# wreuven/h264-scroll-encoder

Measured on AMD Instinct MI355X. Metric: composed frames/sec (1280x720, 360x360 dyn) at 1/2/4/8 GPU; bit-exact vs CPU, higher is better.
Workload: dtype u8; 1 GPU; BASELINE config 3: 256 concurrent 1280x720 streams + 360x360 synthetic dynamic rect (4x4 int transform + quant + CAVLC), composer_write_scroll_frame semantics; resolution=1280x720, streams_per_gpu=256, parallelism=static stream shard x1, no RCCL

## Files before the change

### h264-scroll-encoder_amd/csrc/dyn_engine.h

```cpp
#ifndef SCROLL_DYN_ENGINE_H
#define SCROLL_DYN_ENGINE_H

#include <hip/hip_runtime.h>
#include "engine.h"

typedef struct {
    uint32_t *rows;
    uint16_t *meta;
    uint2 *body_lo, *body_hi;
    uint4 *body_w;
    uint4 *heads;
    unsigned long long *tcx;
    uint32_t *rowstage;
    uint32_t *gbits;
    uint32_t *spill;
    uint32_t *ctr;
    uint32_t ctr_frames;
    uint32_t epoch;
} DynScratch;
#define DYN_HEAD_VECS 16
#define DYN_CTR_LIST 4

typedef struct {
    hipStream_t side;
    hipEvent_t e0, e1;
} DynFork;
int dyn_launch_code(hipStream_t hs, int nframes, int S, DevStream *st, const NalDesc *nal,
                    int ld_nal, const PlanPending *pend, DynFrame *dfr, int ld_fr,
                    const DynGeom *g, const uint8_t *src, const uint8_t *refs, const DynScratch *x,
                    uint32_t epoch, int mbw, uint64_t *stamps, const DynFork *fk, hipEvent_t ev0 = nullptr,
                    hipEvent_t ev1 = nullptr);
int dyn_launch_static(hipStream_t hs, int nframes, int S, DevStream *st, const NalDesc *nal, int ld_nal,
                      const PlanPending *pend, DynFrame *dfr, int ld_fr, const DynGeom *g, const DynScratch *x);
int dyn_launch_pack(hipStream_t hs, int nframes, int S, DevStream *st, const NalDesc *nal,
                    int ld_nal, const PlanPending *pend, DynFrame *dfr, int ld_fr,
                    const DynGeom *g, const DynScratch *x, uint8_t *eps, uint64_t *stamps, const DynFork *fk);
int dyn_launch_emit(hipStream_t hs, int nframes, int S, const DevStream *st, const NalDesc *nal,
                    int ld_nal, const DynFrame *dfr, int ld_fr, const DynGeom *g,
                    const uint8_t *stage, const DynScratch *x, uint8_t *arena, uint64_t ld_arena,
                    uint64_t *stamps);
int dyn_launch_synth(hipStream_t hs, int nframes, int S, uint8_t *src, const DynGeom *g,
                     int stream_base, int t0);

void dyn_rowstage_geom(DynGeom *g, int mbw, int mbh);
size_t dyn_slot_bound(int mbw, int mbh, int rw, int rh);
uint32_t dyn_ep_cap(int rw, int rh, int debug);

#endif
```

### h264-scroll-encoder_amd/csrc/dyn_kernels.hip

```cpp
#include <hip/hip_runtime.h>

#include <stdint.h>
#include <mutex>

#include "dyn_device.h"
#include "dyn_engine.h"
#include "row_mfma.h"
#include "stage_util.h"

using namespace scroll;
using namespace scroll::dyn;
using namespace scroll::stage;

namespace {

__constant__ Tabs g_tabs = SCROLL_DYN_TABS;
constexpr Tabs k_tabs = SCROLL_DYN_TABS;
__constant__ PTabs g_ptabs = make_ptabs(k_tabs);
__device__ uint32_t g_tzrb[TZRB_N];
__constant__ LvTab g_lvt = make_lvt();

struct QpPair {
    QParams l, c;
};
// ... 452 lines not shown
    Regions rg;
    int a_end, mbw, nrefs;
    __device__ inline int sel(int row, int col) const
    {
        const bool curA = row < a_end, abvA = (row - 1) < a_end;
        return 3 * (row == 0 ? 0 : (curA ? 1 : (abvA ? 2 : 3))) + (col == 0 ? 0 : (col == mbw - 1 ? 2 : 1));
    }
    template <class S>
    __device__ inline void put_class(S &sk, int cls) const
    {
        const int ty = cls / 3, pos = cls - 3 * ty;
        const int x = pos == 0 ? 0 : (pos == 1 ? min(1, mbw - 1) : mbw - 1);
        const bool cur = ty == 0 ? 0 < a_end : ty == 1;
        const bool abv = ty == 1 || ty == 2;
        const int ref = cur ? rg.ra : rg.rb, mv4 = 4 * (cur ? rg.mva : rg.mvb);
        const int aref = abv ? rg.ra : rg.rb, amv4 = 4 * (abv ? rg.mva : rg.mvb);
        int px, py;
        predict(x, ty == 0 ? 0 : 1, mbw, ref, mv4, aref, amv4, px, py);
        put_mb_head(sk, ref, 0 - px, mv4 - py, nrefs);
    }
    template <class S>
    __device__ inline void put_slow(S &sk, int row, int col) const
    {
        const bool curA = row < a_end, abvA = (row - 1) < a_end;
        const int ref = curA ? rg.ra : rg.rb, mv4 = 4 * (curA ? rg.mva : rg.mvb);
        const int aref = abvA ? rg.ra : rg.rb, amv4 = 4 * (abvA ? rg.mva : rg.mvb);
        int px, py;
        predict(col, row, mbw, ref, mv4, aref, amv4, px, py);
        put_mb_head(sk, ref, 0 - px, mv4 - py, nrefs);
    }
};

__device__ inline HeadCtx head_ctx(const NalCtx &c)
{
    HeadCtx H;
    H.rg = regions(c);
    H.a_end = (c.h - c.off) / 16;
    H.mbw = c.w / 16;
    H.nrefs = 2 + c.nwp;
    return H;
}

__device__ inline uint32_t row_static_bits(const HeadCtx &H, const uint32_t *hlen, int row, const Rect &R)
{
    const int mbw = H.mbw;
    const bool in = row >= R.y0 && row < R.y0 + R.h;
    auto isdyn = [&](int col) { return in && col >= R.x0 && col < R.x0 + R.w; };
    const int base = H.sel(row, 0) - 0;
    uint32_t bits = isdyn(0) ? 0u : hlen[base] + 1u;
    if (mbw >= 2) {
        if (!isdyn(mbw - 1)) bits += hlen[base + 2] + 1u;
        int nmid = mbw - 2;
        if (in) nmid -= max(0, min(R.x0 + R.w, mbw - 1) - max(R.x0, 1));
        bits += (uint32_t)nmid * (hlen[base + 1] + 1u);
    }
    return bits;
}

__device__ inline void lb_store(unsigned long long *p, uint64_t v)
{
    __hip_atomic_store(p, v, __ATOMIC_RELAXED, __HIP_MEMORY_SCOPE_AGENT);
}

__host__ __device__ inline uint64_t rs_group_words(const DynGeom &g, int nA, int gi)
{
    if (gi < nA) return (uint64_t)gi * g.rs_static_words;
    if (gi < nA + g.h) return (uint64_t)nA * g.rs_static_words + (uint64_t)(gi - nA) * g.rs_row_words;
    return (uint64_t)(gi - g.h) * g.rs_static_words + (uint64_t)g.h * g.rs_row_words;
}

__host__ __device__ inline uint64_t rs_runs_words(const DynGeom &g, int nA, int gi)
{
    const bool row = gi >= nA && gi < nA + g.h;
    return rs_group_words(g, nA, gi) + (row ? g.rs_row_words - EPC_ROW : g.rs_static_words - EPC_STATIC);
}

constexpr uint32_t LO_LEN = 0x7ffu;

__device__ inline void piece_token(const uint16_t (*ct)[68], uint32_t mv, int nC, uint32_t &tv, uint32_t &tl)
{
    const int tc = tc_of(mv), t1 = (int)((mv >> 13) & 3u);
    if (nC >= 8) {
        tv = tc ? (uint32_t)(((tc - 1) << 2) | t1) : 3u;
        tl = 6;
    } else {
        const uint32_t e = ct[nC < 2 ? 0 : (nC < 4 ? 1 : 2)][4 * tc + t1];
        tv = e & 255u;
        tl = e >> 8;
    }
}

__device__ inline void wave_sync()
{
    __builtin_amdgcn_fence(__ATOMIC_RELEASE, "wavefront");
    __builtin_amdgcn_wave_barrier();
    __builtin_amdgcn_fence(__ATOMIC_ACQUIRE, "wavefront");
}

template <class S>
__device__ inline void ovf_code(S &sk, const PTabs &PT, const Tabs &TB, uint4 bd, const uint4 *bw, int pc, int nC)
{
    if (nC == -1) {
        const int dq[4] = {(int)(int16_t)(bd.x & 0xffffu), (int)(int16_t)(bd.x >> 16),
                           (int)(int16_t)(bd.y & 0xffffu), (int)(int16_t)(bd.y >> 16)};
        cavlc_dc4(sk, PT, dq);
    } else if (bw) {
        const uint4 hi = *bw;
        const uint32_t w8[8] = {bd.x, bd.y, bd.z, bd.w, hi.x, hi.y, hi.z, hi.w};
        int16_t l16[16];
#pragma unroll
        for (int i = 0; i < 8; ++i) {
            l16[2 * i] = (int16_t)(w8[i] & 0xffffu);
            l16[2 * i + 1] = (int16_t)(w8[i] >> 16);
        }
        cavlc_block(sk, TB, l16, pc < 16 ? 16 : 15, nC);
    } else {
        const int8_t *lvp = reinterpret_cast<const int8_t *>(&bd);
        cavlc_block(sk, TB, lvp, pc < 16 ? 16 : 15, nC);
    }
}

__device__ __attribute__((noinline)) uint32_t ovf_bits(const PTabs &PT, const Tabs &TB, uint4 bd, const uint4 *bw,
                                                       int pc, int nC)
{
    CountSink cn{0};
    ovf_code(cn, PT, TB, bd, bw, pc, nC);
    return cn.n;
}

__device__ __attribute__((noinline)) void ovf_put(uint32_t *buf, uint32_t lo, uint32_t n, uint32_t pos,
                                                  const PTabs &PT, const Tabs &TB, uint4 bd, const uint4 *bw, int pc,
                                                  int nC)
{
    WSink sk{LdsOrWin{buf, lo, n}, 0, 0, 0};
    sk.start(pos);
    ovf_code(sk, PT, TB, bd, bw, pc, nC);
    sk.finish();
}

__device__ inline uint4 body_msb(uint64_t hi, uint64_t lo, uint32_t n)
{
    const uint32_t k = 128u - n;
    uint64_t H, Lw;
    if (k >= 64u) {
        H = k >= 128u ? 0ull : lo << (k - 64u);
        Lw = 0ull;
    } else {
        H = k ? (hi << k) | (lo >> (64u - k)) : hi;
        Lw = lo << k;
    }
    return make_uint4((uint32_t)(H >> 32), (uint32_t)H, (uint32_t)(Lw >> 32), (uint32_t)Lw);
}

__global__ __launch_bounds__(256) void k_dyn_rows(const DevStream *__restrict__ st,
                                                  const NalDesc *__restrict__ nal, int ld_nal,
                                                  const PlanPending *__restrict__ pend,
                                                  DynFrame *__restrict__ dfr, int ld_fr, DynGeom g,
                                                  uint32_t *__restrict__ rows, uint32_t *__restrict__ ctr,
                                                  uint4 *__restrict__ heads)
{
    __shared__ int32_t wo[8], wl[8], wv[8];
    __shared__ int32_t gen;
    const int s = blockIdx.y, f = blockIdx.x, t = threadIdx.x;
    DynFrame *DF = dfr + (size_t)s * ld_fr + f;
    const int j = DF->nal;
    if (j < 0) return;
    if (t < 8) {
        wo[t] = pend[s].wo[t];
        wl[t] = pend[s].wl[t];
        wv[t] = pend[s].wv[t];
    }
    if (t == 0) gen = 0;
    __syncthreads();
    const DevStream *S = st + s;
    const NalDesc d = nal[(size_t)s * ld_nal + j];
    const NalCtx c = nal_ctx(S, d, wo, wl, wv);
    if (t < 12) {
        const HeadCtx H = head_ctx(c);
        CapSink hc{0, 0, 0};
        H.put_class(hc, t);
        uint4 *hv = heads + ((size_t)s * ld_fr + f) * DYN_HEAD_VECS;
        hv[t] = body_msb(hc.hi, hc.lo, min(hc.n, 128u));
        reinterpret_cast<uint32_t *>(hv + 12)[t] = hc.n | (hc.over() ? 0x80000000u : 0u);
    }
    const Regions rg = regions(c);
    const int w = c.w, h = c.h, a_end = (h - c.off) / 16;
    const uint32_t ysz = (uint32_t)w * (uint32_t)h, pic = ysz + ysz / 2;
    const WpTab T{wo, wv, h};
    uint32_t *rw = rows + ((size_t)s * ld_fr + f) * (size_t)(32 * g.h);
    bool my_gen = false;
    for (int i = t; i < 32 * g.h; i += 256) {
        uint32_t e;
        if (i < 16 * g.h) {
            const int Y = 16 * g.y0 + i, row = Y >> 4;
            const bool cA = row < a_end;
            int yo;
            const int b = luma_row(T, cA ? rg.ra : rg.rb, Y + (cA ? rg.mva : rg.mvb), yo);
            e = (uint32_t)b * pic + (uint32_t)yo * (uint32_t)w;
        } else {
            const int i2 = i - 16 * g.h, bot = i2 >= 8 * g.h;
            const int Y = 8 * g.y0 + (bot ? i2 - 8 * g.h : i2), row = Y >> 3;
            const bool cA = row < a_end;
            const int q = 4 * (cA ? rg.mva : rg.mvb), o = q >> 3, fr = q & 7;
            int yo;
            const int b = chroma_row(T, cA ? rg.ra : rg.rb, Y + o + bot, yo);
            if (b < 0) {
                e = ROW_GEN;
                if (!bot || fr) my_gen = true;
            } else {
                e = ((uint32_t)b * pic + ysz + (uint32_t)yo * (uint32_t)(w / 2)) | (uint32_t)fr << 28;
            }
        }
        rw[i] = e;
    }
    if (my_gen || S->dyn_qp < QP_MIN) gen = 1;
    __syncthreads();
    if (t == 0) {
        uint32_t e = 0u;
        if (gen) {
            const uint32_t k = atomicAdd(&ctr[1], 1u);
            if (k < g.gen_cap) {
                DF->rbsp_bytes = k;
                ctr[DYN_CTR_LIST + k] = (uint32_t)((size_t)s * ld_fr + f);
                e = DF_GENERAL;
            } else {
                e = DF_OVER;
            }
        }
        DF->err = e;
        DF->ep = 0u;
    }
}

constexpr int GW = 64;
#ifndef SCROLL_GBUF_WORDS
#define SCROLL_GBUF_WORDS 256
#endif
constexpr int GBUF_WORDS = SCROLL_GBUF_WORDS;

#ifndef SCROLL_STATIC_WORDS
#define SCROLL_STATIC_WORDS 1
#endif

struct StaticFixed {
    uint32_t ncand;
    uint32_t buf[GBUF_WORDS];
    uint64_t hhi[12], hlo[12];
    uint4 pat[12];
    uint32_t hlen[12];
    int32_t head_over;
    int32_t wo[8], wl[8], wv[8];
    uint32_t moff[DYN_STATIC_ROWS + 1];
};

__global__ __launch_bounds__(GW) void k_dyn_static(const DevStream *__restrict__ st,
                                                   const NalDesc *__restrict__ nal, int ld_nal,
                                                   const PlanPending *__restrict__ pend,
                                                   const DynFrame *__restrict__ dfr, int ld_fr, DynGeom g,
                                                   uint32_t *__restrict__ rowstage, uint32_t *__restrict__ gbits)
{
    __shared__ StaticFixed L;
    constexpr int SR = DYN_STATIC_ROWS;
    const Rect R{g.x0, g.y0, g.w, g.h};
    const int nA = max(1, (R.y0 + SR - 1) / SR);
    const int gi = (int)blockIdx.x >= nA ? (int)blockIdx.x + R.h : (int)blockIdx.x;
    const int ng = g.ngroups, f = blockIdx.y, s = blockIdx.z, t = threadIdx.x;
    const size_t nb = (size_t)s * ld_fr + f;
    const int j = dfr[nb].nal;
    if (j < 0) return;
    const bool first = gi == 0, last = gi == ng - 1;
    if (t < 8) {
        L.wo[t] = pend[s].wo[t];
        L.wl[t] = pend[s].wl[t];
        L.wv[t] = pend[s].wv[t];
    }
    if (t == 0) {
        L.head_over = 0;
        L.ncand = 0;
    }
    const DevStream *S = st + s;
    const NalDesc d = nal[(size_t)s * ld_nal + j];
    wave_sync();
    NalCtx c = nal_ctx(S, d, L.wo, L.wl, L.wv);
    c.qpd = S->dyn_qp - QP_DEFAULT;
    const HeadCtx H = head_ctx(c);
    const int mbw = H.mbw, mbh = c.h / 16;
    int ra, rb;
    if (gi < nA) {
        ra = gi * SR;
        rb = min(ra + SR, R.y0);
    } else {
        ra = R.y0 + R.h + (gi - nA - R.h) * SR;
        rb = min(ra + SR, mbh);
    }
    uint32_t F = 0;
    if (first) {
        CountSink hc{0};
        emit_slice_header(hc, c);
        F = hc.n;
    }
    if (t < 12) {
        CapSink hc{0, 0, 0};
        H.put_class(hc, t);
        L.hhi[t] = hc.hi;
        L.hlo[t] = hc.lo;
        L.hlen[t] = hc.n;
        if (hc.over()) L.head_over = 1;
        if (hc.n < 128u) {
            const uint64_t hi = (hc.hi << 1) | (hc.lo >> 63), lo = (hc.lo << 1) | 1u;
            L.pat[t] = body_msb(hi, lo, hc.n + 1u);
        } else {
            L.head_over = 1;
        }
    }
    wave_sync();
    const bool head_over = L.head_over;
    auto head_bits = [&](int r, int col) -> uint32_t {
        if (!head_over) return L.hlen[H.sel(r, col)];
        CountSink cn{0};
        H.put_slow(cn, r, col);
        return cn.n;
    };
    uint32_t len = 0;
    const int r = ra + t;
    if (r < rb) {
        if (!head_over) {
            len = row_static_bits(H, L.hlen, r, R);
        } else {
            for (int col = 0; col < mbw; ++col) len += head_bits(r, col) + 1u;
        }
    }
    const uint32_t incl = wave_incl_sum(len, t);
    if (r < rb) L.moff[r - ra] = F + incl - len;
    const uint32_t rows_end = F + __shfl(incl, GW - 1, GW);
    if (t == 0) L.moff[rb - ra] = rows_end;
    const uint32_t bits = rows_end + (last ? 1u : 0u);
    if (t == 0) gbits[nb * (size_t)ng + gi] = bits;
    wave_sync();

    uint32_t *out = rowstage + nb * g.rs_frame_words + rs_group_words(g, nA, gi);
    const uint32_t nw = min((bits + 31u) >> 5, g.rs_static_words - EPC_STATIC);
    const int ne = rb - ra;
    auto cnt_le = [&](uint32_t x) -> int {
        int lo = 0, hi = ne + 1;
        while (lo < hi) {
            const int mid = (lo + hi) >> 1;
            if (L.moff[mid] <= x) lo = mid + 1;
            else hi = mid;
        }
        return lo;
    };
    const uint32_t m_mbw = magic32((uint32_t)mbw);
    for (uint32_t p0 = 0; p0 < nw; p0 += GBUF_WORDS) {
        const uint32_t n = min((uint32_t)GBUF_WORDS, nw - p0);
        for (uint32_t i = (uint32_t)t; i < n; i += GW) L.buf[i] = 0u;
        wave_sync();
        const LdsOrWin win{L.buf, p0, n};
        if (!(SCROLL_STATIC_WORDS && !head_over) && first && t == 0 && p0 * 32u < F) {
            WSink hs{win, 0, 0, 0};
            hs.start(0);
            emit_slice_header(hs, c);
            hs.finish();
        }
        if (SCROLL_STATIC_WORDS && !head_over) {
            const uint32_t rbeg = L.moff[0], rend = L.moff[ne];
            for (uint32_t i = (uint32_t)t; i < n; i += GW) {
                const uint32_t W0 = 32u * (p0 + i), W1 = W0 + 32u;
                uint32_t acc = 0, b = max(W0, rbeg), R0 = 0, R1 = 0, L0 = 0, Lm = 1;
                int b3 = 0;
                float inv = 1.0f;
                while (b < W1 && b < rend) {
                    if (b >= R1 || b < R0) {
                        const int e = cnt_le(b) - 1;
                        R0 = L.moff[e];
                        R1 = L.moff[e + 1];
                        b3 = H.sel(ra + e, 0);
                        L0 = L.hlen[b3] + 1u;
                        Lm = L.hlen[b3 + 1] + 1u;
                        inv = 1.0f / (float)Lm;
                    }
                    const uint32_t o = b - R0;
                    uint32_t cl = (uint32_t)b3, off = o;
                    if (o >= L0) {
                        const uint32_t o2 = o - L0;
                        uint32_t q = (uint32_t)((float)o2 * inv);
                        if (q * Lm > o2) --q;
                        else if ((q + 1u) * Lm <= o2) ++q;
                        if (q < (uint32_t)(mbw - 2)) {
                            cl = (uint32_t)b3 + 1u;
                            off = o2 - q * Lm;
                        } else {
                            cl = (uint32_t)b3 + 2u;
                            off = o2 - (uint32_t)(mbw - 2) * Lm;
                        }
                    }
                    const uint32_t k = min(L.hlen[cl] + 1u - off, W1 - b);
                    const uint4 P = L.pat[cl];
                    const uint32_t wi = off >> 5, sh = off & 31u;
                    const uint32_t w0 = wi == 0 ? P.x : (wi == 1 ? P.y : (wi == 2 ? P.z : P.w));
                    const uint32_t w1 = wi == 0 ? P.y : (wi == 1 ? P.z : (wi == 2 ? P.w : 0u));
                    uint32_t v = sh ? __builtin_amdgcn_alignbit(w0, w1, 32u - sh) : w0;
                    v &= k >= 32u ? 0xffffffffu : ~(0xffffffffu >> k);
                    acc |= v >> (b - W0);
                    b += k;
                }
                L.buf[i] = acc;
            }
            wave_sync();
            if (first && t == 0 && p0 * 32u < F) {
                WSink hs{win, 0, 0, 0};
                hs.start(0);
                emit_slice_header(hs, c);
                hs.finish();
            }
            if (last && t == 0) {
                WSink sk{win, 0, 0, 0};
                sk.start(bits - 1u);
                sk.put(1, 1);
                sk.finish();
            }
            wave_sync();
            flush_window(L.buf, n, p0, p0 + n >= nw, out, &L.ncand,
                         rowstage + nb * g.rs_frame_words + rs_runs_words(g, nA, gi), EPC_STATIC - 1, t, GW);
            wave_sync();
            continue;
        }
        const int ea = max(cnt_le(32u * p0) - 1, 0), eb = min(cnt_le(32u * (p0 + n) - 1u), ne);
        const int nm = eb * mbw;
        for (int m = ea * mbw + t; m < nm; m += GW) {
            const int rr = (int)div_m((uint32_t)m, m_mbw), col = m - rr * mbw, rw = ra + rr;
            uint32_t off = L.moff[rr];
            WSink sk{win, 0, 0, 0};
            if (!head_over) {
                const int b3 = H.sel(rw, 0);
                off += col == 0 ? 0u : L.hlen[b3] + 1u + (uint32_t)(col - 1) * (L.hlen[b3 + 1] + 1u);
                if (off >= 32u * (p0 + n)) continue;
                const int cls = b3 + (col == 0 ? 0 : (col == mbw - 1 ? 2 : 1));
                if (off + L.hlen[cls] + 1u <= 32u * p0) continue;
                sk.start(off);
                sk.put_cap(CapSink{L.hhi[cls], L.hlo[cls], L.hlen[cls]});
            } else {
                for (int c2 = 0; c2 < col; ++c2) off += head_bits(rw, c2) + 1u;
                sk.start(off);
                H.put_slow(sk, rw, col);
            }
            sk.put(1, 1);
            sk.finish();
        }
        if (last && t == 0) {
            WSink sk{win, 0, 0, 0};
            sk.start(bits - 1u);
            sk.put(1, 1);
            sk.finish();
        }
        wave_sync();
        flush_window(L.buf, n, p0, p0 + n >= nw, out, &L.ncand,
                     rowstage + nb * g.rs_frame_words + rs_runs_words(g, nA, gi), EPC_STATIC - 1, t, GW);
        wave_sync();
    }
    if (t == 0) rowstage[nb * g.rs_frame_words + rs_runs_words(g, nA, gi)] = L.ncand;
}


__device__ inline CapSink cap_of_msb(uint64_t a, uint64_t b, uint32_t n)
{
    if (n == 0u) return CapSink{0, 0, 0};
    const uint32_t sh = 128u - n;
    if (sh >= 64u) return CapSink{0, a >> (sh - 64u), n};
    if (sh == 0u) return CapSink{a, b, n};
    return CapSink{a >> sh, (b >> sh) | (a << (64u - sh)), n};
}

__device__ inline void put_piece(uint32_t *buf, uint32_t p0, uint32_t n, uint32_t pos, uint32_t tv, uint32_t tl,
                                 uint4 b, uint32_t bl)
{
    const uint32_t tw = tv & low_mask((int)tl);
    const uint32_t c0 = __builtin_amdgcn_alignbit(tw, b.x, tl), c1 = __builtin_amdgcn_alignbit(b.x, b.y, tl);
    const uint32_t c2 = __builtin_amdgcn_alignbit(b.y, b.z, tl), c3 = __builtin_amdgcn_alignbit(b.z, b.w, tl);
    const uint32_t c4 = __builtin_amdgcn_alignbit(b.w, 0u, tl);
    const uint32_t sh = pos & 31u;
    const uint32_t o[6] = {c0 >> sh, __builtin_amdgcn_alignbit(c0, c1, sh), __builtin_amdgcn_alignbit(c1, c2, sh),
                           __builtin_amdgcn_alignbit(c2, c3, sh), __builtin_amdgcn_alignbit(c3, c4, sh),
                           __builtin_amdgcn_alignbit(c4, 0u, sh)};
    const uint32_t nw = (sh + tl + bl + 31u) >> 5, w0 = (pos >> 5) - p0;
#pragma unroll
    for (uint32_t j = 0; j < 6; ++j)
        if (j < nw && w0 + j < n && o[j]) atomicOr(&buf[w0 + j], o[j]);
}

constexpr uint32_t ROW_PAD = 4;

#ifndef SCROLL_LV_SWZ
#define SCROLL_LV_SWZ 0
#endif
__device__ inline uint32_t lv_key(int slot) { return ((uint32_t)slot >> 4) & 3u; }
__device__ inline uint4 lv_swz(uint4 v, uint32_t key)
{
    if (key & 1u) v = make_uint4(v.y, v.x, v.w, v.z);
    if (key & 2u) v = make_uint4(v.z, v.w, v.x, v.y);
    return v;
}
__device__ inline void put_piece1(uint32_t *buf, uint32_t pos, uint32_t tv, uint32_t tl, uint4 b, uint32_t bl)
{
    const uint32_t tw = tv & low_mask((int)tl);
    const uint32_t c0 = __builtin_amdgcn_alignbit(tw, b.x, tl), c1 = __builtin_amdgcn_alignbit(b.x, b.y, tl);
    const uint32_t c2 = __builtin_amdgcn_alignbit(b.y, b.z, tl), c3 = __builtin_amdgcn_alignbit(b.z, b.w, tl);
    const uint32_t c4 = __builtin_amdgcn_alignbit(b.w, 0u, tl);
    const uint32_t sh = pos & 31u, nw = (sh + tl + bl + 31u) >> 5;
    uint32_t *d = buf + (pos >> 5);
#ifndef SCROLL_PUT_FIRST
#define SCROLL_PUT_FIRST 1
#endif
    atomicOr(d, c0 >> sh);
    if (SCROLL_PUT_FIRST >= 2 || nw > 1u) atomicOr(d + 1, __builtin_amdgcn_alignbit(c0, c1, sh));
    if (SCROLL_PUT_FIRST >= 3 || nw > 2u) atomicOr(d + 2, __builtin_amdgcn_alignbit(c1, c2, sh));
    if (nw > 3u) {
        atomicOr(d + 3, __builtin_amdgcn_alignbit(c2, c3, sh));
        if (nw > 4u) {
            atomicOr(d + 4, __builtin_amdgcn_alignbit(c3, c4, sh));
            if (nw > 5u) atomicOr(d + 5, __builtin_amdgcn_alignbit(c4, 0u, sh));
        }
    }
}

constexpr int ROW_MAXT = 1024;
#ifndef SCROLL_ROW_WAVES
#define SCROLL_ROW_WAVES 8
#endif
#ifndef SCROLL_ROW_NP
#define SCROLL_ROW_NP 3
#endif
#ifndef SCROLL_ROW_NP_WIDE
#define SCROLL_ROW_NP_WIDE 4
#endif
#ifndef SCROLL_ROW_WIDE
#define SCROLL_ROW_WIDE 40
#endif
constexpr int ROW_NPMAX = 8;
#ifndef SCROLL_ROW_GB
#define SCROLL_ROW_GB 896
#endif
constexpr int ROW_GB = SCROLL_ROW_GB;

struct RowFixed {
    RowTabs ptabs;
    union {
        uint32_t buf[ROW_GB + 4];
        struct {
            uint32_t kc[2][SORT_KEYS];
            uint32_t kc_pad[32 - 2 * SORT_KEYS];
            uint32_t lvt[LVT_N];
        };
    };
    uint64_t hhi[12], hlo[12];
    uint32_t hlen[12];
    int32_t wo[8], wl[8], wv[8];
    int32_t head_over;
    uint32_t rt[32];
    uint32_t ncand;
    uint32_t spill;
    uint32_t pcd[NPC];
};

static_assert(2 * SORT_KEYS <= 32 && 32 + LVT_N <= ROW_GB, "the sort counts and the level table share the bit window");
static_assert(ROW_PAD == 4, "RowFixed::buf holds ROW_PAD spare words");
static_assert(offsetof(RowFixed, lvt) % 8 == 0, "the level table is copied in 8-byte words");

__host__ __device__ inline size_t row_lds_base(int w)
{
    return (size_t)16 * NPC * w + (size_t)4 * (w + 1) + (size_t)2 * (3 * NPC * w) + (size_t)10 * w + 16;
}
#ifndef SCROLL_ROW_GB_WIDE
#define SCROLL_ROW_GB_WIDE 1248
#endif
constexpr int ROW_GB_WIDE = SCROLL_ROW_GB_WIDE;
__host__ __device__ inline size_t row_wide_off(int w) { return (row_lds_base(w) + 15) & ~(size_t)15; }
__host__ __device__ inline bool row_wide_win(int w)
{
    return w > SCROLL_ROW_WIDE && row_wide_off(w) + 4 * (size_t)(ROW_GB_WIDE + ROW_PAD) + sizeof(RowFixed) <= 163840;
}
__host__ __device__ inline size_t row_lds_bytes(int w)
{
    return row_wide_win(w) ? row_wide_off(w) + 4 * (size_t)(ROW_GB_WIDE + ROW_PAD) : row_lds_base(w);
}

__host__ __device__ constexpr uint32_t pc_desc(int pc)
{
    if (pc == 16 || pc == 17) return 1u << 17;
    int da = 0, db = 0, e = 0;
    bool al = false, bt = false;
    if (pc < 16) {
        const int bx = pc & 3, by = pc >> 2;
        al = bx == 0;
        da = al ? 3 - NPC : -1;
        bt = by == 0;
        db = bt ? 0 : -4;
        e = bt ? pc : 0;
    } else {
        const int b = (pc - 18) & 3, bx = b & 1, by = b >> 1;
        al = bx == 0;
        da = al ? 1 - NPC : -1;
        bt = by == 0;
        db = bt ? 0 : -2;
        e = bt ? (pc < 22 ? pc - 14 : pc - 16) : 0;
    }
    return (uint32_t)(da + 32) | (al ? 1u : 0u) << 6 | (uint32_t)(db + 32) << 7 | (bt ? 1u : 0u) << 13 |
           (uint32_t)e << 14;
}

struct EpfLds {
    uint32_t *goff, *gb, *gw, *cw, *cbase, *lst, *cnt;
    uint32_t *ws;
};
// ... 2060 lines not shown
        S.fast = false;
        S.two = false;
        S.yv = false;
        S.lp = S.rem = 0u;
        if (c < wend && u0 >= 0 && u0 + 16 <= nebsp) {
            while ((int32_t)(sp[K] + K) < u0) K++;
            const uint32_t i0 = (uint32_t)u0 - K - kb, P = 8u * i0;
            while (gg + 1 < ng && goff[gg + 1] <= P) ++gg;
            const uint32_t lp = P - goff[gg], rem = gb[gg] - lp;
            const bool two = rem < 128u;
            if (!two || gg + 1 >= ng || gb[gg + 1] >= 128u - rem) {
                S.fast = true;
                S.two = two;
                S.lp = lp;
                S.rem = rem;
                S.yv = two && gg + 1 < ng;
                wo = 4u * (gw[gg] + (lp >> 5));
                yo = S.yv ? 4u * gw[gg + 1] : wo;
            }
        }
        S.K = K;
        const auto xa = __builtin_amdgcn_raw_buffer_load_b128(rr, wo, 0, 0);
        const uint32_t x4 = __builtin_amdgcn_raw_buffer_load_b32(rr, wo + 16u, 0, 0);
        const auto y = __builtin_amdgcn_raw_buffer_load_b128(rr, yo, 0, 0);
        S.x[0] = (uint32_t)xa[0]; S.x[1] = (uint32_t)xa[1]; S.x[2] = (uint32_t)xa[2]; S.x[3] = (uint32_t)xa[3];
        S.x[4] = x4;
        S.y[0] = (uint32_t)y[0]; S.y[1] = (uint32_t)y[1]; S.y[2] = (uint32_t)y[2]; S.y[3] = (uint32_t)y[3];
    };
    auto finish = [&](GSet &S) {
        if (S.fast) {
            const uint32_t yb[4] = {S.yv ? S.y[0] : 0u, S.yv ? S.y[1] : 0u, S.yv ? S.y[2] : 0u, S.yv ? S.y[3] : 0u};
            fast_chunk(S.c, S.u0, S.K, S.lp, S.rem, S.two, S.x, yb);
        } else {
            slow_chunk(S.c, S.K);
        }
    };
    for (uint32_t cb = cbeg; cb < cend; cb = wend) {
        uint32_t m = n;
        if (whole) {
            kb = 0;
            wend = cend;
        } else {
            __syncthreads();
            if (t == 0) {
                const int32_t ulo = 16 * (int32_t)cb - d0;
                uint32_t lo = 0, hi = n;
                while (lo < hi) {
                    const uint32_t mid = (lo + hi) >> 1;
                    if ((int32_t)(el[mid] + mid) < ulo) lo = mid + 1;
                    else hi = mid;
                }
                const uint32_t mm = min(n - lo, wcap);
                uint32_t ce = cend;
                if (lo + mm < n) ce = min(cend, max(cb + 1u, (uint32_t)((int32_t)(el[lo + mm] + lo + mm) + d0) >> 4));
                win[0] = lo;
                win[1] = mm;
                win[2] = ce;
            }
            __syncthreads();
            kb = win[0];
            m = win[1];
            wend = win[2];
        }
        for (uint32_t i = t; i < m; i += DT) (sorted ? sp : raw)[i] = el[kb + i] + kb;
        if (t == 0) sp[m] = 0x3fffffffu;
        __syncthreads();
        for (uint32_t i = t; i < (sorted ? 0u : m); i += DT) {
            const uint32_t v = raw[i];
            uint32_t r = 0;
            for (uint32_t k = 0; k < m; ++k) r += raw[k] < v ? 1u : 0u;
            sp[r] = v;
        }
        __syncthreads();
        T = goff[ng];
        ub = whole ? 0 : max(0, 16 * (int32_t)cb - d0);
        const uint32_t span = whole ? d.size : (uint32_t)(16 * (int32_t)wend - d0 - ub + 16);
        int lg = 0;
        while ((1u << lg) <= m) lg++;
        cs = 8;
        while ((span >> cs) >= (uint32_t)EPLIST_MAX) cs++;
        nblk = (int)(span >> cs) + 1;
        for (int bi = t; bi < nblk; bi += DT) {
            const uint32_t e0 = (uint32_t)ub + ((uint32_t)bi << cs);
            uint32_t K = 0;
            for (int b = lg - 1; b >= 0; --b) {
                const uint32_t k2 = K + (1u << b);
                K = k2 <= m && sp[k2 - 1] + (k2 - 1) < e0 ? k2 : K;
            }
            raw[bi] = K;
        }
        __syncthreads();
        if (stp && cb == cbeg) stp[1] = __builtin_amdgcn_s_memrealtime();
        GSet sa, sb;
        uint32_t c = cb + (uint32_t)t;
        if (c < wend) prep(c, sa);
        while (c < wend) {
            prep(c + DT, sb);
            finish(sa);
            c += DT;
            if (c >= wend) break;
            prep(c + DT, sa);
            finish(sb);
            c += DT;
        }
    }
    if (stamps) {
        __syncthreads();
        if (stp) stp[2] = __builtin_amdgcn_s_memrealtime();
    }
}

__device__ inline uint32_t mix32(uint32_t x)
{
    x ^= x >> 16;
    x *= 0x7feb352du;
    x ^= x >> 15;
    x *= 0x846ca68bu;
    x ^= x >> 16;
    return x;
}

__global__ __launch_bounds__(256) void k_dyn_synth(uint8_t *__restrict__ src, DynGeom g,
                                                   int stream_base, int t0)
{
    const uint32_t i = blockIdx.x * 256u + threadIdx.x;
    const int f = blockIdx.y, s = blockIdx.z;
    const uint32_t npx = 384u * (uint32_t)g.w * (uint32_t)g.h;
    if (i >= npx) return;
    const uint32_t tt = (uint32_t)(t0 + f);
    const uint32_t seed = (0x9E3779B9u * (uint32_t)(stream_base + s)) ^ (0x85EBCA6Bu * tt);
    const uint32_t hv = mix32(seed + i * 0x9E3779B9u);
    const uint32_t ly = 256u * (uint32_t)g.w * (uint32_t)g.h;
    int v;
    if (i < ly) {
        const int lw = 16 * g.w;
        const int y = (int)(i / (uint32_t)lw), x = (int)(i - (uint32_t)(y * lw));
        const int X = 16 * g.x0 + x, Y = 16 * g.y0 + y;
        v = 128 + ((X + 2 * Y + 3 * (int)tt) & 63) - 32 + (int)(hv >> 28) - 8;
    } else {
        const uint32_t r = (i - ly) % (64u * (uint32_t)g.w * (uint32_t)g.h);
        const int cw = 8 * g.w;
        const int y = (int)(r / (uint32_t)cw), x = (int)(r - (uint32_t)(y * cw));
        const int X = 8 * g.x0 + x, Y = 8 * g.y0 + y;
        v = 128 + ((X + Y + (int)tt) & 15) - 8 + (int)(hv >> 30);
    }
    src[(size_t)s * g.src_ld + (size_t)f * g.src_fr + i] = (uint8_t)clampi(v, 0, 255);
}

}

int dyn_launch_code(hipStream_t hs, int nframes, int S, DevStream *st, const NalDesc *nal,
                    int ld_nal, const PlanPending *pend, DynFrame *dfr, int ld_fr,
                    const DynGeom *g, const uint8_t *src, const uint8_t *refs, const DynScratch *x,
                    uint32_t epoch, int mbw, uint64_t *stamps, const DynFork *fk, hipEvent_t ev0, hipEvent_t ev1)
{
    if (nframes <= 0 || S <= 0) return 0;
    {
        static std::mutex mu;
        static uint64_t ready = 0;
        int dev = 0;
        if (hipGetDevice(&dev) != hipSuccess || dev >= 64) return -1;
        std::lock_guard<std::mutex> lk(mu);
        if (!(ready >> dev & 1u)) {
            hipLaunchKernelGGL(k_tzrb_init, dim3((TZRB_N + 255) / 256), dim3(256), 0, hs);
            if (hipGetLastError() != hipSuccess || hipStreamSynchronize(hs) != hipSuccess) return -1;
            ready |= 1ull << dev;
        }
    }
    hipLaunchKernelGGL(k_dyn_rows, dim3(nframes, S), dim3(256), 0, hs, st, nal, ld_nal, pend, dfr, ld_fr,
                       *g, x->rows, x->ctr, x->heads);
    if (hipGetLastError() != hipSuccess) return -1;
    hipStream_t hg = hs;
    if (fk) {
        if (hipEventRecord(fk->e0, hs) != hipSuccess || hipStreamWaitEvent(fk->side, fk->e0, 0) != hipSuccess)
            return -1;
        hg = fk->side;
    }
    const int nchunk = (24 * g->w * g->h + CODE_T - 1) / CODE_T;
    hipLaunchKernelGGL(k_dyn_code_general, dim3(nchunk, CODE_GEN_Y), dim3(CODE_T), 0, hg, st, dfr, ld_fr,
                       pend, nal, ld_nal, *g, x->rows, src, refs, x->meta, x->body_lo, x->body_hi, x->body_w,
                       x->ctr);
    if (hipGetLastError() != hipSuccess) return -1;
    if (row_lds_bytes(g->w) > 65536) {
        const int rl = (int)row_lds_bytes(g->w);
        if (hipFuncSetAttribute(reinterpret_cast<const void *>(&k_dyn_row<false>),
                                hipFuncAttributeMaxDynamicSharedMemorySize, rl) != hipSuccess ||
            hipFuncSetAttribute(reinterpret_cast<const void *>(&k_dyn_row<true>),
                                hipFuncAttributeMaxDynamicSharedMemorySize, rl) != hipSuccess)
            return -1;
    }
    if (ev0 && hipEventRecord(ev0, hs) != hipSuccess) return -1;
    hipLaunchKernelGGL(k_dyn_row<false>, dim3(g->h, nframes, S), dim3(row_threads(g->w)),
                       row_lds_bytes(g->w), hs, st, nal, ld_nal, pend, dfr, ld_fr, *g, x->rows, src, refs,
                       x->meta, x->body_lo, x->body_hi, x->body_w, x->tcx, epoch, x->rowstage, x->gbits, x->spill,
                       x->ctr, x->heads, stamps);
    if (hipGetLastError() != hipSuccess) return -1;
    if (ev1 && hipEventRecord(ev1, hs) != hipSuccess) return -1;
    hipLaunchKernelGGL(k_dyn_row<true>, dim3(g->h, std::min<uint32_t>(g->gen_cap, (uint32_t)(nframes * S)), 1),
                       dim3(row_threads(g->w)),
                       row_lds_bytes(g->w), hg, st, nal, ld_nal, pend, dfr, ld_fr, *g, x->rows, src, refs,
                       x->meta, x->body_lo, x->body_hi, x->body_w, x->tcx, epoch, x->rowstage, x->gbits, x->spill,
                       x->ctr, x->heads, stamps);
    if (hipGetLastError() != hipSuccess) return -1;
    if (fk) {
        if (dyn_launch_static(hg, nframes, S, st, nal, ld_nal, pend, dfr, ld_fr, g, x) ||
            hipEventRecord(fk->e1, hg) != hipSuccess)
            return -1;
    }
    return 0;
}

int dyn_launch_static(hipStream_t hs, int nframes, int S, DevStream *st, const NalDesc *nal, int ld_nal,
                      const PlanPending *pend, DynFrame *dfr, int ld_fr, const DynGeom *g, const DynScratch *x)
{
    if (nframes <= 0 || S <= 0) return 0;
    hipLaunchKernelGGL(k_dyn_static, dim3(g->ngroups - g->h, nframes, S), dim3(GW), 0, hs, st, nal, ld_nal,
                       pend, dfr, ld_fr, *g, x->rowstage, x->gbits);
    return hipGetLastError() == hipSuccess ? 0 : -1;
}

int dyn_launch_pack(hipStream_t hs, int nframes, int S, DevStream *st, const NalDesc *nal,
                    int ld_nal, const PlanPending *pend, DynFrame *dfr, int ld_fr,
                    const DynGeom *g, const DynScratch *x, uint8_t *eps, uint64_t *stamps, const DynFork *fk)
{
    if (nframes <= 0 || S <= 0) return 0;
    if (fk) {
        if (hipStreamWaitEvent(hs, fk->e1, 0) != hipSuccess) return -1;
    } else if (dyn_launch_static(hs, nframes, S, st, nal, ld_nal, pend, dfr, ld_fr, g, x)) {
        return -1;
    }
    if (g->ep_cap >= (uint32_t)EPF_BIG_LIST)
        hipLaunchKernelGGL((k_dyn_epfix<EPF_T, EPF_BIG_LIST>), dim3(nframes, S), dim3(EPF_T), gtab_bytes(g->ngroups, true),
                           hs, st, dfr, ld_fr, nframes, *g, x->rowstage, x->gbits, eps, stamps);
    else
        hipLaunchKernelGGL((k_dyn_epfix<EPF_T, EPF_LIST>), dim3(nframes, S), dim3(EPF_T), gtab_bytes(g->ngroups, true),
                           hs, st, dfr, ld_fr, nframes, *g, x->rowstage, x->gbits, eps, stamps);
    return hipGetLastError() == hipSuccess ? 0 : -1;
}

int dyn_launch_emit(hipStream_t hs, int nframes, int S, const DevStream *st, const NalDesc *nal,
                    int ld_nal, const DynFrame *dfr, int ld_fr, const DynGeom *g,
                    const uint8_t *stage, const DynScratch *x, uint8_t *arena, uint64_t ld_arena,
                    uint64_t *stamps)
{
    if (nframes <= 0 || S <= 0) return 0;
    const bool big = (int64_t)g->w * g->h > 1024;
    const uint32_t *rs = x ? x->rowstage : nullptr, *gbits = x ? x->gbits : nullptr;
    const dim3 grid(nframes, S, GATHER_Z);
    const size_t gl = x ? gtab_bytes(g->ngroups, false) : 0;
    if (x && !(g->debug & SCROLL_DEBUG_DYN_GATHER1))
        hipLaunchKernelGGL(k_dyn_gather, dim3(nframes, S, gather_z(*g, (int64_t)nframes * S)), dim3(DT), gl, hs, st, nal, ld_nal, dfr,
                           ld_fr, *g, stage, rs, gbits, arena, ld_arena, stamps);
    else if (x && big)
        hipLaunchKernelGGL((k_dyn_emit_gather<4, true>), grid, dim3(DT), gl, hs, st, nal, ld_nal, dfr, ld_fr, *g,
                           stage, rs, gbits, arena, ld_arena, stamps);
    else if (x)
        hipLaunchKernelGGL((k_dyn_emit_gather<1, true>), grid, dim3(DT), gl, hs, st, nal, ld_nal, dfr, ld_fr, *g,
                           stage, rs, gbits, arena, ld_arena, stamps);
    else if (big)
        hipLaunchKernelGGL((k_dyn_emit_gather<4, false>), grid, dim3(DT), 0, hs, st, nal, ld_nal, dfr, ld_fr,
                           *g, stage, rs, gbits, arena, ld_arena, stamps);
    else
        hipLaunchKernelGGL((k_dyn_emit_gather<1, false>), grid, dim3(DT), 0, hs, st, nal, ld_nal, dfr, ld_fr,
                           *g, stage, rs, gbits, arena, ld_arena, stamps);
    return hipGetLastError() == hipSuccess ? 0 : -1;
}

int dyn_launch_synth(hipStream_t hs, int nframes, int S, uint8_t *src, const DynGeom *g,
                     int stream_base, int t0)
{
    if (nframes <= 0 || S <= 0) return 0;
    const uint32_t npx = 384u * (uint32_t)g->w * (uint32_t)g->h;
    hipLaunchKernelGGL(k_dyn_synth, dim3((npx + 255) / 256, nframes, S), dim3(256), 0, hs, src, *g,
                       stream_base, t0);
    return hipGetLastError() == hipSuccess ? 0 : -1;
}

void dyn_rowstage_geom(DynGeom *g, int mbw, int mbh)
{
    const int SR = DYN_STATIC_ROWS;
    const int above = g->y0 < SR ? g->y0 : SR, below0 = mbh - g->y0 - g->h;
    const int below = below0 < SR ? below0 : SR;
    const int maxrows = above > below ? above : below;
    auto words = [](uint64_t bits) { return (uint32_t)((((bits + 31) / 32) + 63) & ~(uint64_t)63); };
    g->rs_static_words = words((uint64_t)HDR_MAX + (uint64_t)maxrows * mbw * (HEAD_MAX + 1) + 64) + EPC_STATIC;
    g->rs_spill_words = words((uint64_t)mbw * (HEAD_MAX + 1) + (uint64_t)g->w * MB_BITS_MAX + 64) + EPC_ROW;
    g->rs_row_words = words((uint64_t)mbw * (HEAD_MAX + 1) + (uint64_t)g->w * SCROLL_DYN_ROW_KBITS + 64) + EPC_ROW;
    if (g->rs_row_words > g->rs_spill_words) g->rs_row_words = g->rs_spill_words;
    g->rs_frame_words = (uint64_t)(g->ngroups - g->h) * g->rs_static_words + (uint64_t)g->h * g->rs_row_words;
}

uint32_t dyn_ep_cap(int rw, int rh, int debug)
{
    return (debug & SCROLL_DEBUG_DYN_EPWIN) || epf_big_rect((int64_t)rw * rh) ? (uint32_t)EPF_BIG_LIST
                                                                            : (uint32_t)EPLIST_MAX;
}

size_t dyn_slot_bound(int mbw, int mbh, int rw, int rh)
{
    const size_t bits = (size_t)HDR_MAX + (size_t)mbw * mbh * (HEAD_MAX + 1) +
                        (size_t)rw * rh * MB_BITS_MAX + 64;
    return ((bits / 8 + 32 + DYN_OVF_BYTES) + 255) & ~(size_t)255;
}

extern "C" int scroll_debug_row_occupancy(int w, int mbw, int extra_lds)
{
    int n = -1;
    (void)mbw;
    const size_t lds = (size_t)((long)row_lds_bytes(w) + extra_lds);
    if (hipOccupancyMaxActiveBlocksPerMultiprocessor(&n, reinterpret_cast<const void *>(&k_dyn_row<false>),
                                                     row_threads(w), lds) != hipSuccess)
        return -1;
    return n;
}
```

### h264-scroll-encoder_amd/csrc/scroll_kernels.hip

```cpp
#include <hip/hip_runtime.h>

#include <stdarg.h>
#include <stdint.h>
#include <stdio.h>
#include <stdlib.h>
#include <string.h>

#include <algorithm>
#include <mutex>
#include <vector>

#include "dyn_engine.h"
#include "hint_engine.h"
#include "splice_engine.h"
#include "hdyn_engine.h"
#include "ingest_engine.h"
#include "ipcm_engine.h"
#include "engine.h"
#include "scroll_device.h"

#include "dyn_device.h"

using namespace scroll;

// ... 661 lines not shown
                A[B0 + rel] = (uint8_t)tile_byte(Lo, no, cnt, jj, rel);
            }
        }
    }
    mark(4);
    if (stamps && lane == 0) {
        uint64_t hw = (uint32_t)__builtin_amdgcn_s_getreg((31 << 11) | 4);
        uint64_t xcc = (uint32_t)__builtin_amdgcn_s_getreg((15 << 11) | 20);
        stamp[7] = (__builtin_amdgcn_s_memrealtime() & 0xffffffffull) | (hw << 32);
        stamp[6] = (stamp[6] & 0x00ffffffffffffffull) | ((xcc & 0xff) << 56);
    }
    if (own && d.slow == 1) serial_write(my_ctx, A + d.out_off);
}

thread_local char g_err[512];

void set_err(const char *fmt, ...)
{
    va_list ap;
    va_start(ap, fmt);
    vsnprintf(g_err, sizeof(g_err), fmt, ap);
    va_end(ap);
}

#define HIPCHK(x)                                                                  \
    do {                                                                           \
        hipError_t e_ = (x);                                                       \
        if (e_ != hipSuccess) {                                                    \
            set_err("%s failed: %s", #x, hipGetErrorString(e_));                   \
            return SCROLL_ERR_HIP;                                                 \
        }                                                                          \
    } while (0)

int usable_devices(std::vector<int> *ids)
{
    int n = 0;
    if (hipGetDeviceCount(&n) != hipSuccess || n <= 0) {
        set_err("no HIP device visible (libh264scroll needs an MI355X / gfx950)");
        return 0;
    }
    int ok = 0;
    for (int i = 0; i < n; ++i) {
        hipDeviceProp_t p;
        if (hipGetDeviceProperties(&p, i) != hipSuccess) continue;
        if (strncmp(p.gcnArchName, "gfx950", 6) == 0) {
            ok++;
            if (ids) ids->push_back(i);
        }
    }
    if (!ok) set_err("no gfx950 device among %d HIP devices", n);
    return ok;
}

int check_cfg(const ComposerConfig *c)
{
    if (c->log2_max_frame_num < 1 || c->log2_max_frame_num > 16 ||
        (c->pic_order_cnt_type == 0 &&
         (c->log2_max_pic_order_cnt_lsb < 1 || c->log2_max_pic_order_cnt_lsb > 16)) ||
        c->num_waypoints < 0 || c->num_waypoints > MAX_WAYPOINTS || c->width < 0 ||
        c->height < 0) {
        set_err("unsupported ComposerConfig (log2 fields must be 1..16, num_waypoints 0..8)");
        return SCROLL_ERR_CONFIG;
    }
    return SCROLL_OK;
}

void cfg_to_dev(const ComposerConfig *c, DevStream *d)
{
    d->w = c->width;
    d->h = c->height;
    d->log2_mfn = c->log2_max_frame_num;
    d->poc_type = c->pic_order_cnt_type;
    d->log2_poc = c->log2_max_pic_order_cnt_lsb;
    d->deblock = c->deblocking_filter_control_present_flag;
    d->frame_num = c->frame_num;
    d->nwp = c->num_waypoints;
    for (int i = 0; i < 8; ++i) {
        d->wp_off[i] = c->waypoints[i].offset_px;
        d->wp_lt[i] = c->waypoints[i].long_term_idx;
        d->wp_valid[i] = c->waypoints[i].valid;
    }
}

void dev_to_cfg(const DevStream *d, ComposerConfig *c)
{
    c->frame_num = d->frame_num;
    c->num_waypoints = d->nwp;
    for (int i = 0; i < 8; ++i) {
        c->waypoints[i].offset_px = d->wp_off[i];
        c->waypoints[i].long_term_idx = d->wp_lt[i];
        c->waypoints[i].valid = d->wp_valid[i];
    }
}

}

constexpr int NEV = 7;
struct ScrollBatch {
    int device = 0;
    int mode = SCROLL_MODE_COMPOSER;
    int max_streams = 0, max_frames = 0, nstreams = 0;
    int debug = 0;
    size_t arena_bytes = 0, ld_arena = 0;
    int ld_nal = 0;
    DevStream *d_st = nullptr;
    DevStream *h_st = nullptr;
    int32_t *d_off = nullptr;
    NalDesc *d_nal = nullptr;
    uint8_t *d_arena = nullptr;
    hipStream_t own = nullptr;
    hipStream_t last = nullptr;
    hipEvent_t ev[NEV] = {};
    int timing = 0;
    int timed_pending = 0;
    float ms[6] = {0, 0, 0, 0, 0, 0};
    std::vector<hipEvent_t> ring;
    std::vector<uint8_t> ring_dyn;
    int ev_dyn = 0;
    int ring_used = 0;
    double acc_ms[6] = {0, 0, 0, 0, 0, 0};
    int acc_n = 0;
    int host_valid = 1;
    int last_plan_mode = SCROLL_PLAN_COMPOSER;
    int last_nframes = 0;
    std::vector<NalDesc> nal_cache;
    int nal_cache_valid = 0;
    uint64_t *d_dbg = nullptr;
    size_t dbg_slots = 0;
    PlanPending *d_pend = nullptr;
    int dyn_on = 0;
    int dyn_pw = 0, dyn_ph = 0;
    int dyn_refs = 0;
    DynGeom geo{};
    DynFrame *d_dfr = nullptr;
    uint8_t *d_src = nullptr, *d_refs = nullptr, *d_stage = nullptr;
    DynScratch dx{};
    int hint_on = 0;
    int hint_dirty = 0;
    int hint_max_mb = 0;
    std::vector<std::vector<ScrollHintRect>> h_hint;
    std::vector<int16_t> h_hint_mode;
    HintFrame *d_hf = nullptr;
    ScrollHintRect *d_pool = nullptr;
    size_t pool_cap = 0;
    struct SpliceHost {
        int x0 = 0, y0 = 0, w = 0, h = 0;
        std::vector<uint8_t> nal;
        const uint8_t *dnal = nullptr;
        size_t n = 0;
    };
    std::vector<SpliceHost> h_sp;
    std::vector<int32_t> h_dyn_pos;
    int fallback = 0;
    DynFork fork{};
    std::vector<int32_t> h_dyn_qp;
    int dyn_pos_custom = 0;
    int dyn_qp = 26;
    int hd_dirty = 0;
    uint32_t hd_mb_words = 0;
    size_t dyn_cap = 0;
    int sp_n = 0;
    int sp_dirty = 0;
    int sp_parse = 0;
    SpliceFrame *d_spf = nullptr;
    uint8_t *d_sp_nal = nullptr;
    uint32_t *d_sp_rbsp = nullptr;
    SpliceMbRec *d_sp_rec = nullptr;
    int32_t *d_sp_list = nullptr;
    SpliceUnit *d_sp_units = nullptr;
    int32_t *d_sp_lanes = nullptr;
    size_t sp_lanes_cap = 0, sp_nslots = 0;
    int sp_ymax = 1;
    size_t sp_nal_cap = 0, sp_rbsp_cap = 0, sp_rec_cap = 0, sp_list_cap = 0, sp_units_cap = 0;
    uint8_t *d_ing_in = nullptr;
    size_t ing_in_cap = 0;
    IngestFile *d_ing_files = nullptr;
    IngestScan *d_ing_scan = nullptr;
    IngestOut *d_ing_out = nullptr;
    int ing_cap = 0;
    void *d_ing_work = nullptr;
    size_t ing_work_bytes = 0;
    hipEvent_t ing_ev[2] = {};
    uint32_t *d_ipcm_cnt = nullptr;
    size_t ipcm_cap = 0;
    uint8_t *d_ipcm_stg = nullptr;
    size_t ipcm_stg_cap = 0;
    unsigned long long *d_ipcm_hw = nullptr;
    size_t ipcm_hw_cap = 0;
    uint32_t ipcm_epoch = 0;
    double ipcm_ms = 0.0;
    int ipcm_n = 0;
    uint32_t *ipcm_over = nullptr;
    uint32_t *d_ipcm_sticky = nullptr;
    size_t ipcm_over_stride = 0;
    std::vector<hipEvent_t> ipcm_ev;
    size_t ipcm_ev_used = 0;
    double ing_ms = 0.0;
    int ing_n = 0;
    int dyn_grow = 0;
    int32_t *d_upd = nullptr;
    size_t upd_cap = 0;
    uint64_t *d_out_tab = nullptr;
    size_t out_tab_cap = 0;
    hipEvent_t out_ev = nullptr;
};

static void event_ms(const hipEvent_t *e, bool dyn, bool lite, float out[6])
{
    auto el = [&](int a, int b) {
        float v = 0.0f;
        return hipEventElapsedTime(&v, e[a], e[b]) == hipSuccess ? v : 0.0f;
    };
    if (lite) {
        for (int k = 0; k < 6; ++k) out[k] = 0.0f;
        if (dyn) out[2] = out[4] = el(1, 6);
        else out[1] = el(1, 4);
        return;
    }
    if (dyn) {
        out[0] = el(0, 1) + el(2, 3);
        out[1] = el(3, 4);
        out[2] = el(1, 2);
        out[3] = el(4, 5);
        out[4] = el(1, 6);
        out[5] = el(6, 2);
    } else {
        out[0] = el(0, 1);
        out[1] = el(1, 4);
        out[2] = out[3] = out[4] = out[5] = 0.0f;
    }
}

static hipError_t timing_event(hipEvent_t *e)
{
    return hipEventCreateWithFlags(e, hipEventDisableSystemFence);
}

extern "C" {

const char *scroll_last_error(void) { return g_err; }

const char *scroll_version(void) { return "h264scroll-amd 0.1 (gfx950)"; }

int scroll_device_count(void) { return usable_devices(nullptr); }

int scroll_batch_create(ScrollBatch **out, const ScrollBatchDesc *desc)
{
    if (!out || !desc || desc->max_streams <= 0 || desc->max_frames <= 0 ||
        desc->arena_bytes == 0 ||
        (desc->mode != SCROLL_MODE_COMPOSER && desc->mode != SCROLL_MODE_EXPERIMENT)) {
        set_err("scroll_batch_create: bad descriptor");
        return SCROLL_ERR_ARG;
    }
    *out = nullptr;
    std::vector<int> ids;
    if (!usable_devices(&ids)) return SCROLL_ERR_NO_DEVICE;
    int n = 0;
    (void)hipGetDeviceCount(&n);
    if (desc->device < 0 || desc->device >= n) {
        set_err("scroll_batch_create: device %d out of range (%d visible)", desc->device, n);
        return SCROLL_ERR_ARG;
    }
    bool ok = false;
    for (int i : ids) ok |= (i == desc->device);
    if (!ok) {
        set_err("scroll_batch_create: device %d is not gfx950", desc->device);
        return SCROLL_ERR_NO_DEVICE;
    }
    HIPCHK(hipSetDevice(desc->device));
    ScrollBatch *b = new ScrollBatch();
    b->device = desc->device;
    b->mode = desc->mode;
    b->max_streams = desc->max_streams;
    b->max_frames = desc->max_frames;
    b->arena_bytes = desc->arena_bytes;
    b->ld_arena = (desc->arena_bytes + 128 + 255) & ~(size_t)255;
    b->ld_nal = 2 * desc->max_frames;
    size_t S = (size_t)desc->max_streams;
    hipError_t e = hipSuccess;
    if (e == hipSuccess) e = hipMalloc(&b->d_st, S * sizeof(DevStream));
    if (e == hipSuccess) e = hipHostMalloc(&b->h_st, S * sizeof(DevStream), hipHostMallocDefault);
    if (e == hipSuccess) e = hipMalloc(&b->d_off, S * (size_t)desc->max_frames * sizeof(int32_t));
    if (e == hipSuccess) e = hipMalloc(&b->d_nal, S * (size_t)b->ld_nal * sizeof(NalDesc));
    if (e == hipSuccess) e = hipMalloc(&b->d_arena, S * b->ld_arena);
    if (e == hipSuccess) e = hipMalloc(&b->d_pend, S * sizeof(PlanPending));
    if (e == hipSuccess) e = hipStreamCreateWithFlags(&b->own, hipStreamNonBlocking);
    for (int i = 0; i < NEV && e == hipSuccess; ++i) e = timing_event(&b->ev[i]);
    if (e == hipSuccess) e = hipMemset(b->d_st, 0, S * sizeof(DevStream));
    if (e == hipSuccess) e = hipMemset(b->d_off, 0, S * (size_t)desc->max_frames * sizeof(int32_t));
    if (e != hipSuccess) {
        set_err("scroll_batch_create: %s", hipGetErrorString(e));
        scroll_batch_destroy(b);
        return e == hipErrorOutOfMemory ? SCROLL_ERR_OOM : SCROLL_ERR_HIP;
    }
    memset(b->h_st, 0, S * sizeof(DevStream));
    b->last = b->own;
    *out = b;
    return SCROLL_OK;
}

void scroll_batch_destroy(ScrollBatch *b)
{
    if (!b) return;
    (void)hipSetDevice(b->device);
    if (b->own) (void)hipStreamSynchronize(b->own);
    for (int i = 0; i < NEV; ++i)
        if (b->ev[i]) (void)hipEventDestroy(b->ev[i]);
    for (hipEvent_t e : b->ring) (void)hipEventDestroy(e);
    if (b->fork.side) {
        (void)hipStreamSynchronize(b->fork.side);
        (void)hipStreamDestroy(b->fork.side);
        (void)hipEventDestroy(b->fork.e0);
        (void)hipEventDestroy(b->fork.e1);
    }
    if (b->own) (void)hipStreamDestroy(b->own);
    (void)hipFree(b->d_st);
    (void)hipHostFree(b->h_st);
    (void)hipFree(b->d_off);
    (void)hipFree(b->d_nal);
    (void)hipFree(b->d_arena);
    (void)hipFree(b->d_out_tab);
    (void)hipFree(b->d_upd);
    if (b->out_ev) (void)hipEventDestroy(b->out_ev);
    (void)hipFree(b->d_pend);
    (void)hipFree(b->d_dfr);
    (void)hipFree(b->d_src);
    (void)hipFree(b->d_refs);
    (void)hipFree(b->d_stage);
    (void)hipFree(b->d_hf);
    (void)hipFree(b->d_pool);
    (void)hipFree(b->d_spf);
    (void)hipFree(b->d_sp_nal);
    (void)hipFree(b->d_sp_rbsp);
    (void)hipFree(b->d_sp_rec);
    (void)hipFree(b->d_sp_list);
    (void)hipFree(b->d_sp_units);
    (void)hipFree(b->d_sp_lanes);
    (void)hipFree(b->d_ing_in);
    (void)hipFree(b->d_ipcm_cnt);
    (void)hipFree(b->d_ipcm_stg);
    (void)hipFree(b->d_ipcm_hw);
    (void)hipFree(b->d_ing_files);
    (void)hipFree(b->d_ing_scan);
    (void)hipFree(b->d_ing_out);
    (void)hipFree(b->d_ing_work);
    for (hipEvent_t e : b->ing_ev)
        if (e) (void)hipEventDestroy(e);
    for (hipEvent_t e : b->ipcm_ev)
        if (e) (void)hipEventDestroy(e);
    (void)hipFree(b->d_ipcm_sticky);
    if (b->d_dbg) (void)hipFree(b->d_dbg);
    delete b;
}

int scroll_batch_num_streams(const ScrollBatch *b) { return b ? b->nstreams : 0; }

int scroll_batch_set_debug(ScrollBatch *b, int flags)
{
    if (!b) return SCROLL_ERR_ARG;
    b->debug = flags;
    return SCROLL_OK;
}

static int dyn_grow_pools(ScrollBatch *b);

static int ipcm_async_check(ScrollBatch *b);

static int batch_host_sync(ScrollBatch *b)
{
    if (b->host_valid) return SCROLL_OK;
    HIPCHK(hipSetDevice(b->device));
    HIPCHK(hipStreamSynchronize(b->last));
    HIPCHK(hipMemcpy(b->h_st, b->d_st, (size_t)b->nstreams * sizeof(DevStream),
                     hipMemcpyDeviceToHost));
    b->host_valid = 1;
    return SCROLL_OK;
}

int scroll_batch_add_stream(ScrollBatch *b, const ComposerConfig *cfg)
{
    if (!b || !cfg) return SCROLL_ERR_ARG;
    if (b->nstreams >= b->max_streams) {
        set_err("scroll_batch_add_stream: batch full (%d streams)", b->max_streams);
        return SCROLL_ERR_ARG;
    }
    int rc = check_cfg(cfg);
    if (rc) return rc;
    if (b->dyn_on && (cfg->width != b->dyn_pw || cfg->height != b->dyn_ph)) {
        set_err("scroll_batch_add_stream: the dynamic rect needs %dx%d streams", b->dyn_pw,
                b->dyn_ph);
        return SCROLL_ERR_CONFIG;
    }
    if (b->hint_on && ((cfg->width / 16) * (cfg->height / 16) > b->hint_max_mb ||
                       cfg->width / 16 > HINT_MAX_MBW)) {
        set_err("scroll_batch_add_stream: hint staging slots hold %d MBs per picture, %d per row",
                b->hint_max_mb, HINT_MAX_MBW);
        return SCROLL_ERR_CONFIG;
    }
    rc = batch_host_sync(b);
    if (rc) return rc;
    int s = b->nstreams;
    DevStream *d = &b->h_st[s];
    if (b->dyn_qp != 26 && !cfg->deblocking_filter_control_present_flag) {
        set_err("scroll_batch_add_stream: a stream with the deblocking filter on (no "
                "deblocking_filter_control_present_flag) needs the rect at QP 26, the batch's is %d",
                b->dyn_qp);
        return SCROLL_ERR_CONFIG;
    }
    memset(d, 0, sizeof(*d));
    cfg_to_dev(cfg, d);
    d->dyn_qp = b->dyn_qp;
    d->out_pos = 0;
    d->out_cap = b->arena_bytes;
    HIPCHK(hipSetDevice(b->device));
    HIPCHK(hipMemcpy(b->d_st + s, d, sizeof(DevStream), hipMemcpyHostToDevice));
    b->nstreams++;
    return s;
}

int scroll_batch_get_config(ScrollBatch *b, int s, ComposerConfig *cfg)
{
    if (!b || !cfg || s < 0 || s >= b->nstreams) return SCROLL_ERR_ARG;
    int rc = batch_host_sync(b);
    if (rc) return rc;
    const DevStream *d = &b->h_st[s];
    composer_config_init(cfg, d->w, d->h);
    cfg->log2_max_frame_num = d->log2_mfn;
    cfg->pic_order_cnt_type = d->poc_type;
    cfg->log2_max_pic_order_cnt_lsb = d->log2_poc;
    cfg->deblocking_filter_control_present_flag = d->deblock;
    dev_to_cfg(d, cfg);
    return SCROLL_OK;
}

int scroll_batch_set_config(ScrollBatch *b, int s, const ComposerConfig *cfg)
{
    if (!b || !cfg || s < 0 || s >= b->nstreams) return SCROLL_ERR_ARG;
    int rc = check_cfg(cfg);
    if (rc) return rc;
    rc = batch_host_sync(b);
    if (rc) return rc;
    DevStream *d = &b->h_st[s];
    if (!cfg->deblocking_filter_control_present_flag) {
        bool bad = d->dyn_qp != 26;
        const size_t F = (size_t)b->max_frames, i0 = (size_t)s * F;
        for (size_t f = 0; !bad && f < F && i0 + f < b->h_dyn_qp.size(); ++f) {
            const int q = b->h_dyn_qp[i0 + f];
            bad = q >= 0 && q != 26;
        }
        if (bad) {
            set_err("scroll_batch_set_config: stream %d's rect QP is not 26: it cannot turn the deblocking "
                    "filter on (no deblocking_filter_control_present_flag)", s);
            return SCROLL_ERR_CONFIG;
        }
    }
    cfg_to_dev(cfg, d);
    HIPCHK(hipSetDevice(b->device));
    HIPCHK(hipMemcpy(b->d_st + s, d, sizeof(DevStream), hipMemcpyHostToDevice));
    return SCROLL_OK;
}

int scroll_batch_set_offsets(ScrollBatch *b, const int32_t *offsets, int nframes)
{
    if (!b || !offsets || nframes < 0 || nframes > b->max_frames) return SCROLL_ERR_ARG;
    if (nframes == 0 || b->nstreams == 0) return SCROLL_OK;
    HIPCHK(hipSetDevice(b->device));
    HIPCHK(hipMemcpy2D(b->d_off, (size_t)b->max_frames * sizeof(int32_t), offsets,
                       (size_t)nframes * sizeof(int32_t), (size_t)nframes * sizeof(int32_t),
                       (size_t)b->nstreams, hipMemcpyHostToDevice));
    return SCROLL_OK;
}

int32_t *scroll_batch_offsets_device(ScrollBatch *b) { return b ? b->d_off : nullptr; }

static void fold_ring(ScrollBatch *b)
{
    for (int i = 0; i + NEV <= b->ring_used; i += NEV) {
        float m[6];
        event_ms(&b->ring[i], (b->ring_dyn[i / NEV] & 1) != 0, (b->ring_dyn[i / NEV] & 2) != 0, m);
        for (int k = 0; k < 6; ++k) b->acc_ms[k] += m[k];
        b->acc_n++;
    }
    b->ring_used = 0;
}

static int ring_events(ScrollBatch *b, hipEvent_t **evs)
{
    if ((size_t)b->ring_used + NEV > b->ring.size()) {
        if (b->ring.size() >= (size_t)NEV * 256) {
            HIPCHK(hipStreamSynchronize(b->last));
            fold_ring(b);
        } else {
            for (int i = 0; i < NEV; ++i) {
                hipEvent_t e;
                HIPCHK(timing_event(&e));
                b->ring.push_back(e);
            }
            b->ring_dyn.push_back(0);
        }
    }
    *evs = &b->ring[b->ring_used];
    b->ring_used += NEV;
    return SCROLL_OK;
}

static int launch(ScrollBatch *b, int nframes, int plan_mode, int nal_max, hipStream_t hs,
                  int plan_flags = 0)
{
    int S = b->nstreams;
    if (S == 0) return SCROLL_OK;
    hipEvent_t *rev = nullptr;
    if (b->timing) {
        int rc = ring_events(b, &rev);
        if (rc) return rc;
    }
    const bool hint = b->hint_on && plan_mode != SCROLL_PLAN_EXPLICIT;
    const bool dyn = (b->dyn_on || hint) && plan_mode != SCROLL_PLAN_EXPLICIT;
    const bool lite = b->timing == 2;
    const bool lite_row = lite && dyn && !hint;
    auto mark = [&](int k) -> int {
        if (!b->timing || (!dyn && k != 0 && k != 1 && k != 4)) return SCROLL_OK;
        if (lite) {
            if ((k == 1 || k == (dyn ? 6 : 4)) && !lite_row) HIPCHK(hipEventRecord(rev[k], hs));
            return SCROLL_OK;
        }
        HIPCHK(hipEventRecord(b->ev[k], hs));
        HIPCHK(hipEventRecord(rev[k], hs));
        return SCROLL_OK;
    };
    if (b->timing) {
        b->ring_dyn[(b->ring_used - NEV) / NEV] = (uint8_t)((dyn ? 1 : 0) | (lite ? 2 : 0));
        if (!lite) b->ev_dyn = dyn ? 1 : 0;
    }
    const int ld_fr = b->max_frames;
    int rc = mark(0);
    if (rc) return rc;
    if (!dyn) {
        hipLaunchKernelGGL(k_plan, dim3(S), dim3(PLAN_THREADS), 0, hs, b->d_st, b->d_off,
                           b->max_frames, b->d_nal, b->ld_nal, nframes, plan_mode,
                           b->debug | plan_flags, b->d_pend, b->d_dfr, ld_fr);
        HIPCHK(hipGetLastError());
        if ((rc = mark(1)) || (rc = mark(2)) || (rc = mark(3))) return rc;
    } else {
        const bool dyn_rect = b->dyn_on && !hint;
        hipLaunchKernelGGL(k_plan, dim3(S), dim3(PLAN_THREADS), 0, hs, b->d_st, b->d_off,
                           b->max_frames, b->d_nal, b->ld_nal, nframes, plan_mode,
                           b->debug | plan_flags | PLAN_STATE | PLAN_DYN, b->d_pend, b->d_dfr,
                           ld_fr, nullptr, 0u, 0u, dyn_rect ? b->dx.ctr : nullptr);
        HIPCHK(hipGetLastError());
        if ((rc = mark(1))) return rc;
        uint64_t *stamps = nullptr;
        if (b->debug & SCROLL_DEBUG_DYN_STAMPS) {
            const size_t slots = (2 + (size_t)b->geo.ngroups) * (size_t)nframes * S;
            if (slots > b->dbg_slots) {
                if (b->d_dbg) (void)hipFree(b->d_dbg);
                HIPCHK(hipMalloc(&b->d_dbg, slots * 8 * sizeof(uint64_t)));
                b->dbg_slots = slots;
            }
            HIPCHK(hipMemsetAsync(b->d_dbg, 0, slots * 8 * sizeof(uint64_t), hs));
            stamps = b->d_dbg + 2 * (size_t)nframes * S * 8;
        }
        b->geo.debug = b->debug;
        if (hint) {
            if (b->sp_parse) {
                if (splice_launch_parse(hs, b->sp_n, b->sp_ymax, b->d_sp_list, b->d_spf, b->d_sp_units,
                                        b->d_sp_lanes, b->sp_nslots, b->d_st, ld_fr, b->d_sp_rbsp, b->d_sp_rec)) {
                    set_err("k_splice_parse launch: %s", hipGetErrorString(hipGetLastError()));
                    return SCROLL_ERR_HIP;
                }
                b->sp_parse = 0;
            }
            if (b->fallback && b->dyn_on &&
                hint_launch_fb(hs, nframes, S, b->d_st, b->d_nal, b->ld_nal, b->d_pend, b->d_dfr, ld_fr,
                               b->d_hf, b->d_pool)) {
                set_err("k_hint_fb launch: %s", hipGetErrorString(hipGetLastError()));
                return SCROLL_ERR_HIP;
            }
            if (hint_launch_stage(hs, nframes, S, b->d_st, b->d_nal, b->ld_nal, b->d_pend,
                                  b->d_dfr, ld_fr, b->d_hf, b->d_pool, b->d_stage,
                                  b->geo.slot_bytes)) {
                set_err("k_hint_stage launch: %s", hipGetErrorString(hipGetLastError()));
                return SCROLL_ERR_HIP;
            }
            const bool combined = b->dyn_on;
            if (combined &&
                hdyn_launch_code(hs, nframes, S, b->d_st, b->d_nal, b->ld_nal, b->d_pend, b->d_dfr, ld_fr,
                                 b->d_hf, b->d_pool, b->d_spf, &b->geo, b->d_src, b->d_refs,
                                 b->d_sp_rec, b->d_sp_rbsp, b->hd_mb_words)) {
                set_err("k_hdyn_code launch: %s", hipGetErrorString(hipGetLastError()));
                return SCROLL_ERR_HIP;
            }
            if ((b->sp_n > 0 || combined) &&
                splice_launch_stage(hs, nframes, S, b->d_st, b->d_nal, b->ld_nal, b->d_pend,
                                    b->d_dfr, ld_fr, b->d_hf, b->d_pool, b->d_spf, b->d_sp_rec,
                                    b->d_sp_rbsp, b->d_stage, b->geo.slot_bytes)) {
                set_err("k_splice_stage launch: %s", hipGetErrorString(hipGetLastError()));
                return SCROLL_ERR_HIP;
            }
            if ((rc = mark(6))) return rc;
        } else {
            b->dx.epoch = b->dx.epoch % 0xffffffu + 1u;
            const DynGeom &G = b->geo;
            const DynFork *fk = nullptr;
            static const bool fork_on = [] {
                const char *e = getenv("SCROLL_DYN_FORK");
                return e && e[0] == '1';
            }();
            if (fork_on) {
                if (!b->fork.side) {
                    HIPCHK(hipStreamCreateWithFlags(&b->fork.side, hipStreamNonBlocking));
                    HIPCHK(hipEventCreateWithFlags(&b->fork.e0, hipEventDisableTiming));
                    HIPCHK(hipEventCreateWithFlags(&b->fork.e1, hipEventDisableTiming));
                }
                fk = &b->fork;
            }
            if (dyn_launch_code(hs, nframes, S, b->d_st, b->d_nal, b->ld_nal, b->d_pend, b->d_dfr, ld_fr, &G,
                                b->d_src, b->d_refs, &b->dx, b->dx.epoch, b->dyn_pw / 16, stamps, fk,
                                lite_row ? rev[1] : nullptr, lite_row ? rev[6] : nullptr)) {
                set_err("k_dyn_code launch: %s", hipGetErrorString(hipGetLastError()));
                return SCROLL_ERR_HIP;
            }
            if ((rc = mark(6))) return rc;
            if (dyn_launch_pack(hs, nframes, S, b->d_st, b->d_nal, b->ld_nal, b->d_pend, b->d_dfr, ld_fr, &G,
                                &b->dx, b->d_stage, stamps ? b->d_dbg : nullptr, fk)) {
                set_err("k_dyn_static / k_dyn_epfix launch: %s", hipGetErrorString(hipGetLastError()));
                return SCROLL_ERR_HIP;
            }
        }
        if ((rc = mark(2))) return rc;
        hipLaunchKernelGGL(k_plan, dim3(S), dim3(PLAN_THREADS), 0, hs, b->d_st, b->d_off,
                           b->max_frames, b->d_nal, b->ld_nal, nframes, plan_mode,
                           b->debug | plan_flags | PLAN_SIZE | PLAN_DYN, b->d_pend, b->d_dfr,
                           ld_fr, (b->dyn_on && !b->hint_on) ? (const uint32_t *)b->dx.ctr : nullptr,
                           b->geo.rs_spill_cap, b->geo.gen_cap);
        HIPCHK(hipGetLastError());
        if ((rc = mark(3))) return rc;
    }
    int per_wg = EMIT_WAVES * TILE;
    int gx = (nal_max + per_wg - 1) / per_wg;
    if (gx > 0 && (b->debug & SCROLL_DEBUG_EMIT_STAMPS)) {
        size_t slots = (size_t)gx * S * EMIT_WAVES;
        if (slots > b->dbg_slots) {
            if (b->d_dbg) (void)hipFree(b->d_dbg);
            HIPCHK(hipMalloc(&b->d_dbg, slots * 8 * sizeof(uint64_t)));
            b->dbg_slots = slots;
        }
        HIPCHK(hipMemsetAsync(b->d_dbg, 0, slots * 8 * sizeof(uint64_t), hs));
    }
    if (gx > 0) {
        hipLaunchKernelGGL(k_emit, dim3(gx, S), dim3(EMIT_WAVES * 64), 0, hs, b->d_st, b->d_nal,
                           b->ld_nal, b->d_arena, (uint64_t)b->ld_arena, b->debug, b->d_dbg);
        HIPCHK(hipGetLastError());
    }
    if ((rc = mark(4))) return rc;
    if (dyn && dyn_launch_emit(hs, nframes, S, b->d_st, b->d_nal, b->ld_nal, b->d_dfr, ld_fr,
                               &b->geo, b->d_stage, hint ? nullptr : &b->dx, b->d_arena,
                               (uint64_t)b->ld_arena,
                               (b->debug & SCROLL_DEBUG_DYN_STAMPS) && b->d_dbg
                                   ? b->d_dbg + (size_t)nframes * S * 8 : nullptr)) {
        set_err("k_dyn_gather launch: %s", hipGetErrorString(hipGetLastError()));
        return SCROLL_ERR_HIP;
    }
    if ((rc = mark(5))) return rc;
    if (b->timing == 1) b->timed_pending = 1;
    b->host_valid = 0;
    b->nal_cache_valid = 0;
    b->last = hs;
    return SCROLL_OK;
}

static int hint_upload(ScrollBatch *b);
static int splice_upload(ScrollBatch *b);
static int hd_upload(ScrollBatch *b);
static int splice_frame_status(ScrollBatch *b, size_t i, int *status);
static const char *splice_msg(int e);

int scroll_batch_compose(ScrollBatch *b, int nframes, void *hip_stream)
{
    return scroll_batch_compose_ex(b, nframes, hip_stream, 0);
}

int scroll_batch_compose_ex(ScrollBatch *b, int nframes, void *hip_stream, int flags)
{
    if (!b || nframes < 0 || nframes > b->max_frames) {
        set_err("scroll_batch_compose: nframes %d out of range", nframes);
        return SCROLL_ERR_ARG;
    }
    if (b->dyn_on && !b->dyn_refs) {
        set_err("scroll_batch_compose: dynamic rect without reference pictures");
        return SCROLL_ERR_CONFIG;
    }
    HIPCHK(hipSetDevice(b->device));
    const bool combined = b->hint_on && b->dyn_on;
    if (b->dyn_pos_custom && !b->hint_on) {
        set_err("scroll_batch_compose: per-frame dynamic rect positions need UI hints "
                "(scroll_batch_set_hints)");
        return SCROLL_ERR_CONFIG;
    }
    if (b->hint_on && b->sp_dirty) {
        int rc = splice_upload(b);
        if (rc) return rc;
        if (combined) b->hd_dirty = 1;
    }
    if (combined && b->hd_dirty) {
        int rc = hd_upload(b);
        if (rc) return rc;
    }
    if (b->hint_on && b->hint_dirty) {
        int rc = hint_upload(b);
        if (rc) return rc;
    }
    hipStream_t hs = hip_stream ? (hipStream_t)hip_stream : b->own;
    int plan = b->mode == SCROLL_MODE_EXPERIMENT ? SCROLL_PLAN_EXPERIMENT : SCROLL_PLAN_COMPOSER;
    int nal_max = plan == SCROLL_PLAN_COMPOSER ? 2 * nframes : nframes;
    b->last_plan_mode = plan;
    b->last_nframes = nframes;
    return launch(b, nframes, plan, nal_max, hs,
                  (flags & SCROLL_COMPOSE_REWIND) ? PLAN_REWIND : 0);
}

int scroll_batch_sync(ScrollBatch *b)
{
    if (!b) return SCROLL_ERR_ARG;
    {
        int rc0 = batch_host_sync(b);
        if (rc0) return rc0;
        if ((rc0 = ipcm_async_check(b))) return rc0;
    }
    if (b->timed_pending) {
        event_ms(b->ev, b->ev_dyn != 0, false, b->ms);
        b->timed_pending = 0;
    }
    int rc = SCROLL_OK;
    for (int s = 0; s < b->nstreams; ++s) {
        if (!b->h_st[s].err) continue;
        if (rc == SCROLL_OK && (b->h_st[s].err & SCROLL_DEVERR_HANDOFF)) {
            set_err("stream %d: a dynamic-rect row waited past its bound for the row above's "
                    "TotalCoeffs (k_dyn_row hand-off); the stream committed nothing", s);
            rc = SCROLL_ERR_DEVICE;
        } else if (rc == SCROLL_OK && (b->h_st[s].err & SCROLL_DEVERR_SPLICE)) {
            int st = 0, ff = 0;
            for (; ff < b->max_frames && !st; ++ff)
                if (splice_frame_status(b, (size_t)s * b->max_frames + ff, &st)) break;
            if (st == HDYN_STATUS_OVERFLOW) {
                set_err("stream %d frame %d: a dynamic-rect MB under hints outgrew its %u-byte "
                        "region (raise slot_bytes of scroll_batch_set_dyn_rect)", s, ff - 1,
                        4u * b->hd_mb_words);
                rc = SCROLL_ERR_OVERFLOW;
            } else {
                set_err("stream %d frame %d: %s: %s", s, ff - 1,
                        b->dyn_on ? "dynamic rect under hints" : "spliced slice", splice_msg(st));
                rc = SCROLL_ERR_CONFIG;
            }
        } else if (rc == SCROLL_OK && (b->h_st[s].err & SCROLL_DEVERR_HINT)) {
            set_err("stream %d: a hint rect names a reference that is not valid in its frame "
                    "(ref 2 + i needs waypoint i)", s);
            rc = SCROLL_ERR_CONFIG;
        } else if (rc == SCROLL_OK && (b->h_st[s].err & SCROLL_DEVERR_DYN)) {
            uint32_t used[2] = {0, 0};
            if (b->dyn_on && !b->hint_on && b->dx.ctr)
                HIPCHK(hipMemcpy(used, b->dx.ctr, sizeof(used), hipMemcpyDeviceToHost));
            if (used[0] > b->geo.rs_spill_cap || used[1] > b->geo.gen_cap) {
                const int grc = dyn_grow_pools(b);
                set_err("stream %d: the dynamic rect's %s pool ran out (%u of %u); %s", s,
                        used[0] > b->geo.rs_spill_cap ? "row-stage spill" : "general-path record",
                        used[0] > b->geo.rs_spill_cap ? used[0] : used[1],
                        used[0] > b->geo.rs_spill_cap ? b->geo.rs_spill_cap : b->geo.gen_cap,
                        grc ? "growing it failed" : "grown: compose again");
            } else {
                set_err("stream %d: a staged NAL outgrew its staging slot (%llu bytes)", s,
                        (unsigned long long)b->geo.slot_bytes);
            }
            rc = SCROLL_ERR_OVERFLOW;
        } else if (rc == SCROLL_OK) {
            set_err("stream %d: output arena overflow (%llu bytes used, capacity %llu)", s,
                    (unsigned long long)b->h_st[s].out_pos,
                    (unsigned long long)b->h_st[s].out_cap);
            rc = SCROLL_ERR_OVERFLOW;
        }
        b->h_st[s].err = 0;
        HIPCHK(hipMemcpy(&b->d_st[s].err, &b->h_st[s].err, sizeof(int32_t),
                         hipMemcpyHostToDevice));
    }
    if (rc) return rc;
    return SCROLL_OK;
}

size_t scroll_batch_output_size(ScrollBatch *b, int s)
{
    if (!b || s < 0 || s >= b->nstreams || batch_host_sync(b)) return 0;
    return (size_t)b->h_st[s].out_pos;
}

int scroll_batch_copy_output(ScrollBatch *b, int s, size_t from, uint8_t *dst, size_t n)
{
    if (!b || s < 0 || s >= b->nstreams || (!dst && n)) return SCROLL_ERR_ARG;
    int rc = batch_host_sync(b);
    if (rc) return rc;
    if (from + n > b->h_st[s].out_pos) {
        set_err("scroll_batch_copy_output: range beyond stream output");
        return SCROLL_ERR_ARG;
    }
    if (n == 0) return SCROLL_OK;
    HIPCHK(hipSetDevice(b->device));
    HIPCHK(hipMemcpy(dst, b->d_arena + (size_t)s * b->ld_arena + from, n, hipMemcpyDeviceToHost));
    return SCROLL_OK;
}

namespace {
constexpr int OUT_Z = 8;
__global__ __launch_bounds__(1024) void k_out_table(DevStream *__restrict__ st, int S, uint64_t cap,
                                                    uint64_t *__restrict__ dtab, uint64_t *__restrict__ htab)
{
    __shared__ uint64_t s_w[16], s_carry;
    const int t = threadIdx.x, lane = t & 63, wave = t >> 6;
    if (t == 0) s_carry = 0;
    __syncthreads();
    for (int s0 = 0; s0 < S; s0 += 1024) {
        const int s = s0 + t;
        const uint64_t n = s < S ? st[s].undelivered : 0, a = (n + 15) & ~(uint64_t)15;
        const uint64_t inc = wave_incl_scan(a, lane);
        if (lane == 63) s_w[wave] = inc;
        __syncthreads();
        uint64_t before = s_carry;
        for (int w = 0; w < wave; ++w) before += s_w[w];
        if (s < S) {
            dtab[1 + 2 * (size_t)s] = htab[1 + 2 * (size_t)s] = before + inc - a;
            dtab[2 + 2 * (size_t)s] = htab[2 + 2 * (size_t)s] = n;
        }
        __syncthreads();
        if (t == 0)
            for (int w = 0; w < 16; ++w) s_carry += s_w[w];
        __syncthreads();
    }
    if (t == 0) {
        const uint64_t tot = s_carry <= cap ? s_carry : ~(uint64_t)0;
        dtab[0] = htab[0] = tot;
    }
    if (s_carry <= cap)
        for (int s = t; s < S; s += 1024) st[s].undelivered = 0;
}

__global__ __launch_bounds__(256) void k_out_copy(const DevStream *__restrict__ st, const uint8_t *__restrict__ arena,
                                                  uint64_t ld_arena, uint64_t arena_end,
                                                  const uint64_t *__restrict__ dtab, uint8_t *__restrict__ dst)
{
    const int s = blockIdx.y;
    if (dtab[0] == ~(uint64_t)0) return;
    const uint64_t n = dtab[2 + 2 * (size_t)s], o = dtab[1 + 2 * (size_t)s];
    const uint64_t from = (uint64_t)s * ld_arena + st[s].out_pos - n;
    uint4 *d = reinterpret_cast<uint4 *>(dst + o);
    const uint32_t q = (uint32_t)(from & 15u) >> 2, rb = (uint32_t)from & 3u;
    const uint64_t base = from & ~(uint64_t)15;
    const uint4 *a = reinterpret_cast<const uint4 *>(arena + base);
    const uint64_t nch = (n + 15) / 16;
    for (uint64_t j = (uint64_t)blockIdx.x * 256 + threadIdx.x; j < nch; j += (uint64_t)OUT_Z * 256) {
        const uint4 x = a[j];
        const uint4 y = (q | rb) && base + 16 * (j + 2) <= arena_end ? a[j + 1] : x;
        const uint32_t w0 = x.x, w1 = x.y, w2 = x.z, w3 = x.w, w4 = y.x, w5 = y.y, w6 = y.z, w7 = y.w;
        auto pick = [&](uint32_t i) -> uint32_t {
            const uint32_t lo = i & 1u ? (i & 2u ? w3 : w1) : (i & 2u ? w2 : w0);
            const uint32_t hi = i & 1u ? (i & 2u ? w7 : w5) : (i & 2u ? w6 : w4);
            return i & 4u ? hi : lo;
        };
        uint32_t o4[4];
#pragma unroll
        for (uint32_t k = 0; k < 4; ++k) {
            const uint32_t lo = pick(q + k), hi = pick(q + k + 1u);
            o4[k] = rb ? __builtin_amdgcn_alignbyte(hi, lo, rb) : lo;
        }
        d[j] = make_uint4(o4[0], o4[1], o4[2], o4[3]);
    }
}
}

int scroll_host_alloc(void **p, size_t n)
{
    if (!p) return SCROLL_ERR_ARG;
    *p = nullptr;
    hipError_t e = hipHostMalloc(p, n ? n : 1, hipHostMallocDefault);
    if (e != hipSuccess) {
        (void)hipGetLastError();
        set_err("scroll_host_alloc(%zu): %s", n, hipGetErrorString(e));
        return e == hipErrorOutOfMemory ? SCROLL_ERR_OOM : SCROLL_ERR_HIP;
    }
    return SCROLL_OK;
}

void scroll_host_free(void *p)
{
    if (p) (void)hipHostFree(p);
}

int scroll_batch_output_to_host_async(ScrollBatch *b, uint8_t *dst, size_t cap, uint64_t *table, void *hip_stream)
{
    if (!b || !dst || !table || (cap & 15) || (reinterpret_cast<uintptr_t>(dst) & 15)) {
        set_err("scroll_batch_output_to_host_async: bad arguments (dst / cap must be 16-byte aligned)");
        return SCROLL_ERR_ARG;
    }
    HIPCHK(hipSetDevice(b->device));
    hipStream_t hs = hip_stream ? (hipStream_t)hip_stream : (b->last ? b->last : b->own);
    if (b->last && hs != b->last) {
        if (!b->out_ev) HIPCHK(hipEventCreateWithFlags(&b->out_ev, hipEventDisableTiming));
        HIPCHK(hipEventRecord(b->out_ev, b->last));
        HIPCHK(hipStreamWaitEvent(hs, b->out_ev, 0));
    }
    const size_t S = (size_t)b->nstreams;
    if (b->out_tab_cap < 1 + 2 * S) {
        (void)hipFree(b->d_out_tab);
        b->d_out_tab = nullptr;
        b->out_tab_cap = 0;
        HIPCHK(hipMalloc(&b->d_out_tab, (1 + 2 * S) * sizeof(uint64_t)));
        b->out_tab_cap = 1 + 2 * S;
    }
    hipLaunchKernelGGL(k_out_table, dim3(1), dim3(1024), 0, hs, b->d_st, (int)S, (uint64_t)cap, b->d_out_tab,
                       table);
    HIPCHK(hipGetLastError());
    if (S) {
        hipLaunchKernelGGL(k_out_copy, dim3(OUT_Z, (unsigned)S), dim3(256), 0, hs, b->d_st, b->d_arena,
                           (uint64_t)b->ld_arena, (uint64_t)b->max_streams * b->ld_arena, b->d_out_tab, dst);
        HIPCHK(hipGetLastError());
    }
    b->last = hs;
    b->host_valid = 0;
    return SCROLL_OK;
}

const uint8_t *scroll_batch_output_device(ScrollBatch *b, int s)
{
    if (!b || s < 0 || s >= b->nstreams) return nullptr;
    return b->d_arena + (size_t)s * b->ld_arena;
}

int scroll_batch_reset_output(ScrollBatch *b)
{
    if (!b) return SCROLL_ERR_ARG;
    int rc = batch_host_sync(b);
    if (rc) return rc;
    for (int s = 0; s < b->nstreams; ++s) b->h_st[s].out_pos = b->h_st[s].undelivered = 0;
    HIPCHK(hipSetDevice(b->device));
    HIPCHK(hipMemcpy(b->d_st, b->h_st, (size_t)b->nstreams * sizeof(DevStream),
                     hipMemcpyHostToDevice));
    return SCROLL_OK;
}

static int load_nals(ScrollBatch *b)
{
    if (b->nal_cache_valid) return SCROLL_OK;
    int rc = batch_host_sync(b);
    if (rc) return rc;
    b->nal_cache.resize((size_t)b->nstreams * b->ld_nal);
    HIPCHK(hipMemcpy(b->nal_cache.data(), b->d_nal, b->nal_cache.size() * sizeof(NalDesc),
                     hipMemcpyDeviceToHost));
    b->nal_cache_valid = 1;
    return SCROLL_OK;
}

int scroll_batch_nal_count(ScrollBatch *b, int s)
{
    if (!b || s < 0 || s >= b->nstreams) return SCROLL_ERR_ARG;
    int rc = batch_host_sync(b);
    if (rc) return rc;
    return b->h_st[s].nnal;
}

int scroll_batch_nal_info(ScrollBatch *b, int s, int i, int *kind, int *offset_px,
                          uint32_t *size, int *slow)
{
    if (!b || s < 0 || s >= b->nstreams) return SCROLL_ERR_ARG;
    int rc = load_nals(b);
    if (rc) return rc;
    if (i < 0 || i >= b->h_st[s].nnal) return SCROLL_ERR_ARG;
    const NalDesc &d = b->nal_cache[(size_t)s * b->ld_nal + i];
    if (kind) *kind = d.kind;
    if (offset_px) *offset_px = d.off;
    if (size) *size = d.size;
    if (slow) *slow = d.slow;
    return SCROLL_OK;
}

int scroll_batch_kernel_stats(ScrollBatch *b, double *plan_ms, double *emit_ms, int *count)
{
    if (!b) return SCROLL_ERR_ARG;
    int rc = batch_host_sync(b);
    if (rc) return rc;
    HIPCHK(hipStreamSynchronize(b->last));
    fold_ring(b);
    if (plan_ms) *plan_ms = b->acc_ms[0];
    if (emit_ms) *emit_ms = b->acc_ms[1];
    if (count) *count = b->acc_n;
    for (int k = 0; k < 6; ++k) b->acc_ms[k] = 0;
    b->acc_n = 0;
    return SCROLL_OK;
}

int scroll_batch_kernel_stats_ex(ScrollBatch *b, double ms[6], int *count)
{
    if (!b || !ms) return SCROLL_ERR_ARG;
    int rc = batch_host_sync(b);
    if (rc) return rc;
    HIPCHK(hipStreamSynchronize(b->last));
    fold_ring(b);
    for (int k = 0; k < 6; ++k) {
        ms[k] = b->acc_ms[k];
        b->acc_ms[k] = 0;
    }
    if (count) *count = b->acc_n;
    b->acc_n = 0;
    return SCROLL_OK;
}

long long scroll_batch_debug_stamps(ScrollBatch *b, uint64_t *dst, long long max_slots)
{
    if (!b || batch_host_sync(b) || !b->d_dbg) return 0;
    long long n = (long long)b->dbg_slots < max_slots ? (long long)b->dbg_slots : max_slots;
    if (hipMemcpy(dst, b->d_dbg, (size_t)n * 8 * sizeof(uint64_t), hipMemcpyDeviceToHost) !=
        hipSuccess)
        return 0;
    return n;
}

unsigned long long scroll_batch_last_bytes(ScrollBatch *b)
{
    if (!b || batch_host_sync(b)) return 0;
    unsigned long long t = 0;
    for (int s = 0; s < b->nstreams; ++s) t += b->h_st[s].batch_bytes;
    return t;
}

long long scroll_batch_last_nals(ScrollBatch *b)
{
    if (!b || batch_host_sync(b)) return -1;
    long long t = 0;
    for (int s = 0; s < b->nstreams; ++s) t += b->h_st[s].nnal;
    return t;
}

static void dyn_release(ScrollBatch *b)
{
    if (!b->hint_on) {
        (void)hipFree(b->d_dfr);
        (void)hipFree(b->d_stage);
        b->d_dfr = nullptr;
        b->d_stage = nullptr;
    }
    (void)hipFree(b->d_src);
    (void)hipFree(b->d_refs);
    (void)hipFree(b->dx.rows);
    (void)hipFree(b->dx.meta);
    (void)hipFree(b->dx.body_lo);
    (void)hipFree(b->dx.body_hi);
    (void)hipFree(b->dx.body_w);
    (void)hipFree(b->dx.heads);
    (void)hipFree(b->dx.tcx);
    (void)hipFree(b->dx.rowstage);
    (void)hipFree(b->dx.ctr);
    (void)hipFree(b->dx.gbits);
    b->d_src = b->d_refs = nullptr;
    b->dx = DynScratch{};
    b->dyn_on = 0;
    b->dyn_refs = 0;
    b->h_dyn_pos.clear();
    b->h_dyn_qp.clear();
    b->dyn_pos_custom = 0;
    if (b->hint_on) {
        b->geo.x0 = b->geo.y0 = b->geo.w = b->geo.h = 0;
        b->sp_dirty = 1;
        b->hint_dirty = 1;
    }
}

static int hd_setup(ScrollBatch *b);
static int sp_grow(void **p, size_t *cap, size_t n, size_t size);

static size_t round256(size_t n) { return (n + 255) & ~(size_t)255; }

static size_t dyn_pair_bytes(const ScrollBatch *b)
{
    return round256((size_t)3 * b->dyn_pw * b->dyn_ph);
}

int scroll_batch_set_dyn_rect(ScrollBatch *b, int x0, int y0, int w, int h, size_t slot_bytes)
{
    if (!b || x0 < 0 || y0 < 0 || w < 0 || h < 0) return SCROLL_ERR_ARG;
    if (b->hint_on && b->sp_n > 0 && w > 0 && h > 0) {
        set_err("scroll_batch_set_dyn_rect: not combinable with spliced slices (clear them first)");
        return SCROLL_ERR_CONFIG;
    }
    int rc = batch_host_sync(b);
    if (rc) return rc;
    HIPCHK(hipSetDevice(b->device));
    dyn_release(b);
    if (w == 0 || h == 0) return SCROLL_OK;
    if (b->nstreams == 0) {
        set_err("scroll_batch_set_dyn_rect: add the streams first");
        return SCROLL_ERR_ARG;
    }
    const int pw = b->h_st[0].w, ph = b->h_st[0].h;
    for (int s = 1; s < b->nstreams; ++s)
        if (b->h_st[s].w != pw || b->h_st[s].h != ph) {
            set_err("scroll_batch_set_dyn_rect: streams of one batch must share the picture size");
            return SCROLL_ERR_CONFIG;
        }
    const int mbw = pw / 16, mbh = ph / 16;
    if ((pw & 15) || (ph & 15) || x0 + w > mbw || y0 + h > mbh || w > DYN_MAX_W || h > DYN_MAX_H ||
        mbw > DYN_MAX_MBW || mbh > DYN_MAX_MBH ||
        (size_t)3 * pw * ph >= ((size_t)1 << 28)) {
        set_err("scroll_batch_set_dyn_rect: rect (%d,%d %dx%d MBs) not supported in %dx%d", x0, y0,
                w, h, pw, ph);
        return SCROLL_ERR_CONFIG;
    }
    DynGeom g{};
    g.x0 = x0;
    g.y0 = y0;
    g.pw = pw;
    g.ph = ph;
    g.w = w;
    g.h = h;
    g.qp = b->dyn_qp;
    g.ql = scroll::dyn::qparams(g.qp);
    g.qc = scroll::dyn::qparams(scroll::dyn::qp_chroma(g.qp));
    {
        const int sr = DYN_STATIC_ROWS;
        const int na = (y0 + sr - 1) / sr, nbl = (mbh - y0 - h + sr - 1) / sr;
        g.ngroups = (na > 1 ? na : 1) + h + (nbl > 1 ? nbl : 1);
    }
    g.src_fr = (uint64_t)384 * w * h;
    g.src_ld = round256((size_t)b->max_frames * g.src_fr);
    g.ref_ld = 0;
    g.slot_bytes = slot_bytes ? round256(slot_bytes + DYN_OVF_BYTES) : dyn_slot_bound(mbw, mbh, w, h);
    g.ep_cap = dyn_ep_cap(w, h, b->debug);
    dyn_rowstage_geom(&g, mbw, mbh);
    b->dyn_pw = pw;
    b->dyn_ph = ph;
    const size_t S = (size_t)b->max_streams, F = (size_t)b->max_frames;
    hipError_t e = hipSuccess;
    if (!b->hint_on) {
        e = hipMalloc(&b->d_dfr, S * F * sizeof(DynFrame));
        if (e == hipSuccess) e = hipMalloc(&b->d_stage, S * F * (size_t)4 * g.ep_cap);
        if (e == hipSuccess) e = hipMemset(b->d_dfr, 0, S * F * sizeof(DynFrame));
    }
    if (e == hipSuccess) e = hipMalloc(&b->d_src, S * g.src_ld);
    if (e == hipSuccess) e = hipMalloc(&b->d_refs, S * dyn_pair_bytes(b));
    if (e == hipSuccess) e = hipMalloc(&b->dx.rows, S * F * 32 * h * sizeof(uint32_t));
    g.gen_cap = (uint32_t)std::min(S * F, std::max<size_t>(32, S * F / 64));
    g.rs_spill_cap = g.rs_row_words < g.rs_spill_words
                         ? (uint32_t)std::min(S * F * (size_t)h, std::max<size_t>(2048, S * F * (size_t)h / 32))
                         : 0u;
    g.rs_frames = (uint32_t)(S * F);
    if (b->dyn_grow) {
        g.gen_cap = (uint32_t)(S * F);
        if (g.rs_spill_cap) g.rs_spill_cap = (uint32_t)(S * F * (size_t)h);
    }
    const size_t nrec = (size_t)g.gen_cap * DYN_PIECES * w * h;
    if (e == hipSuccess) e = hipMalloc(&b->dx.meta, nrec * sizeof(uint16_t));
    if (e == hipSuccess) e = hipMalloc(&b->dx.body_lo, nrec * sizeof(uint2));
    if (e == hipSuccess) e = hipMalloc(&b->dx.body_hi, nrec * sizeof(uint2));
    if (e == hipSuccess) e = hipMalloc(&b->dx.body_w, nrec * sizeof(uint4));
    const size_t ng = (size_t)g.ngroups;
    if (e == hipSuccess) e = hipMalloc(&b->dx.heads, S * F * DYN_HEAD_VECS * sizeof(uint4));
    if (e == hipSuccess) e = hipMalloc(&b->dx.tcx, S * F * w * h * sizeof(unsigned long long));
    if (e == hipSuccess) e = hipMemset(b->dx.tcx, 0, S * F * w * h * sizeof(unsigned long long));
    const size_t rs_words = S * F * g.rs_frame_words + (size_t)g.rs_spill_cap * g.rs_spill_words;
// ... 215 lines not shown
            n++;
        }
    if (rbsp_bytes) *rbsp_bytes = r;
    if (ep_bytes) *ep_bytes = e;
    if (dyn_nals) *dyn_nals = n;
    return SCROLL_OK;
}

static void hint_release(ScrollBatch *b)
{
    (void)hipFree(b->d_dfr);
    (void)hipFree(b->d_stage);
    (void)hipFree(b->d_hf);
    (void)hipFree(b->d_pool);
    b->d_dfr = nullptr;
    b->d_stage = nullptr;
    b->d_hf = nullptr;
    b->d_pool = nullptr;
    b->pool_cap = 0;
    b->hint_on = 0;
    b->hint_dirty = 0;
    b->h_hint.clear();
    b->h_hint_mode.clear();
    (void)hipFree(b->d_spf);
    (void)hipFree(b->d_sp_nal);
    (void)hipFree(b->d_sp_rbsp);
    (void)hipFree(b->d_sp_rec);
    (void)hipFree(b->d_sp_list);
    (void)hipFree(b->d_sp_units);
    (void)hipFree(b->d_sp_lanes);
    b->d_spf = nullptr;
    b->d_sp_nal = nullptr;
    b->d_sp_rbsp = nullptr;
    b->d_sp_rec = nullptr;
    b->d_sp_list = nullptr;
    b->d_sp_units = nullptr;
    b->d_sp_lanes = nullptr;
    b->sp_nal_cap = b->sp_rbsp_cap = b->sp_rec_cap = b->sp_list_cap = b->sp_units_cap = b->sp_lanes_cap = 0;
    b->sp_nslots = 0;
    b->h_sp.clear();
    b->sp_n = 0;
    b->sp_dirty = 0;
    b->sp_parse = 0;
}

static int hint_upload(ScrollBatch *b)
{
    const size_t n = b->h_hint.size();
    std::vector<HintFrame> hf(n);
    std::vector<ScrollHintRect> pool;
    for (size_t i = 0; i < n; ++i) {
        hf[i].first = (int32_t)pool.size();
        hf[i].n = (int16_t)b->h_hint[i].size();
        hf[i].mode = b->h_hint_mode[i];
        if (i < b->h_sp.size() && b->h_sp[i].w > 0) hf[i].mode |= HINT_MODE_SPLICED;
        if (b->dyn_on && 2 * i < b->h_dyn_pos.size() && b->h_dyn_pos[2 * i] >= 0)
            hf[i].mode |= HINT_MODE_SPLICED;
        pool.insert(pool.end(), b->h_hint[i].begin(), b->h_hint[i].end());
    }
    if (pool.size() > b->pool_cap) {
        (void)hipFree(b->d_pool);
        b->d_pool = nullptr;
        b->pool_cap = 0;
        hipError_t e = hipMalloc(&b->d_pool, pool.size() * sizeof(ScrollHintRect));
        if (e != hipSuccess) {
            set_err("scroll_batch_compose: hint rects: %s", hipGetErrorString(e));
            return e == hipErrorOutOfMemory ? SCROLL_ERR_OOM : SCROLL_ERR_HIP;
        }
        b->pool_cap = pool.size();
    }
    HIPCHK(hipMemcpy(b->d_hf, hf.data(), n * sizeof(HintFrame), hipMemcpyHostToDevice));
    if (!pool.empty())
        HIPCHK(hipMemcpy(b->d_pool, pool.data(), pool.size() * sizeof(ScrollHintRect),
                         hipMemcpyHostToDevice));
    b->hint_dirty = 0;
    return SCROLL_OK;
}

static int hd_setup(ScrollBatch *b)
{
    const size_t S = (size_t)b->max_streams, F = (size_t)b->max_frames;
    const size_t nmb = (size_t)b->geo.w * b->geo.h;
    const size_t words = S * F * nmb * b->hd_mb_words + 2 + RWIN_SLACK_WORDS;
    int rc;
    if (!b->d_spf) {
        HIPCHK(hipMalloc(&b->d_spf, S * F * sizeof(SpliceFrame)));
        HIPCHK(hipMemset(b->d_spf, 0, S * F * sizeof(SpliceFrame)));
    }
    if ((rc = sp_grow((void **)&b->d_sp_rbsp, &b->sp_rbsp_cap, words, sizeof(uint32_t))) ||
        (rc = sp_grow((void **)&b->d_sp_rec, &b->sp_rec_cap, S * F * nmb, sizeof(SpliceMbRec))))
        return rc;
    const size_t slot = splice_slot_bound(b->dyn_pw / 16, b->dyn_ph / 16, b->geo.w, b->geo.h,
                                          nmb * 4 * b->hd_mb_words);
    if (slot > b->geo.slot_bytes) {
        void *ns = nullptr;
        hipError_t e = hipMalloc(&ns, S * F * slot);
        if (e != hipSuccess) {
            (void)hipGetLastError();
            set_err("dynamic rect under hints: staging (%zu bytes per frame): %s", slot,
                    hipGetErrorString(e));
            return e == hipErrorOutOfMemory ? SCROLL_ERR_OOM : SCROLL_ERR_HIP;
        }
        (void)hipFree(b->d_stage);
        b->d_stage = (uint8_t *)ns;
        b->geo.slot_bytes = slot;
    }
    b->hd_dirty = 1;
    b->hint_dirty = 1;
    return SCROLL_OK;
}

static int hd_upload(ScrollBatch *b)
{
    const size_t S = (size_t)b->max_streams, F = (size_t)b->max_frames;
    const size_t nmb = (size_t)b->geo.w * b->geo.h;
    std::vector<SpliceFrame> spf(S * F);
    for (size_t i = 0; i < S * F; ++i) {
        SpliceFrame &o = spf[i];
        o = SpliceFrame{};
        const bool dormant = b->h_dyn_pos[2 * i] < 0;
        if (dormant && !b->fallback) continue;
        o.x0 = dormant ? 0 : b->h_dyn_pos[2 * i];
        o.y0 = dormant ? 0 : b->h_dyn_pos[2 * i + 1];
        o.pad = dormant ? 1 : 0;
        o.w = b->geo.w;
        o.h = b->geo.h;
        o.rbsp_word = i * nmb * b->hd_mb_words;
        o.rec_first = (uint32_t)(i * nmb);
        const int fq = i < b->h_dyn_qp.size() ? b->h_dyn_qp[i] : -1;
        const size_t st = i / F;
        o.hd_qp = fq >= 0 ? fq : (st < (size_t)b->nstreams ? b->h_st[st].dyn_qp : b->dyn_qp);
    }
    HIPCHK(hipMemcpy(b->d_spf, spf.data(), S * F * sizeof(SpliceFrame), hipMemcpyHostToDevice));
    b->hd_dirty = 0;
    return SCROLL_OK;
}

static int set_stream_qp(ScrollBatch *b, int s, int qp, const char *who)
{
    if (!b || qp < SCROLL_DYN_QP_MIN || qp > SCROLL_DYN_QP_MAX || s >= b->nstreams) {
        set_err("%s: QP %d outside %d..%d or stream %d out of range", who, qp, SCROLL_DYN_QP_MIN,
                SCROLL_DYN_QP_MAX, s);
        return SCROLL_ERR_ARG;
    }
    const int s0 = s < 0 ? 0 : s, s1 = s < 0 ? b->nstreams : s + 1;
    for (int k = s0; k < s1; ++k)
        if (qp != 26 && !b->h_st[k].deblock) {
            set_err("%s: stream %d has the deblocking filter on (no "
                    "deblocking_filter_control_present_flag): its rect codes at QP 26", who, k);
            return SCROLL_ERR_CONFIG;
        }
    int rc = batch_host_sync(b);
    if (rc) return rc;
    HIPCHK(hipSetDevice(b->device));
    for (int k = s0; k < s1; ++k) {
        b->h_st[k].dyn_qp = qp;
        HIPCHK(hipMemcpy(&b->d_st[k].dyn_qp, &qp, sizeof(int32_t), hipMemcpyHostToDevice));
    }
    if (s < 0) b->dyn_qp = qp;
    b->hd_dirty = 1;
    return SCROLL_OK;
}

int scroll_batch_set_dyn_qp(ScrollBatch *b, int qp)
{
    return set_stream_qp(b, -1, qp, "scroll_batch_set_dyn_qp");
}

int scroll_batch_set_dyn_qp_stream(ScrollBatch *b, int s, int qp)
{
    if (!b || s < 0) {
        set_err("scroll_batch_set_dyn_qp_stream: bad stream");
        return SCROLL_ERR_ARG;
    }
    return set_stream_qp(b, s, qp, "scroll_batch_set_dyn_qp_stream");
}

int scroll_batch_set_dyn_qp_at(ScrollBatch *b, int s, int f, int qp)
{
    if (!b || !b->hint_on || !b->dyn_on || s < 0 || s >= b->nstreams || f < 0 || f >= b->max_frames ||
        qp < -1 || qp > SCROLL_DYN_QP_MAX) {
        set_err("scroll_batch_set_dyn_qp_at: needs UI hints and the dynamic rect; stream / frame / QP "
                "(-1, 0..%d) out of range", SCROLL_DYN_QP_MAX);
        return SCROLL_ERR_ARG;
    }
    if (qp >= 0 && qp != 26 && !b->h_st[s].deblock) {
        set_err("scroll_batch_set_dyn_qp_at: stream %d has the deblocking filter on: its rect codes at QP 26",
                s);
        return SCROLL_ERR_CONFIG;
    }
    int rc = batch_host_sync(b);
    if (rc) return rc;
    const size_t i = (size_t)s * b->max_frames + f;
    if (b->h_dyn_qp.size() < (size_t)b->max_streams * b->max_frames)
        b->h_dyn_qp.assign((size_t)b->max_streams * b->max_frames, -1);
    b->h_dyn_qp[i] = qp;
    b->hd_dirty = 1;
    return SCROLL_OK;
}

int scroll_batch_set_hints(ScrollBatch *b, int s, int f, const ScrollHintRect *rects, int n,
                           int mode)
{
    if (!b || s < 0 || s >= b->nstreams || f < 0 || f >= b->max_frames || n < 0 ||
        n > SCROLL_HINT_MAX_RECTS || (n > 0 && !rects) ||
        (mode != SCROLL_HINT_EXACT && mode != SCROLL_HINT_PSKIP && mode != SCROLL_HINT_SPEC)) {
        set_err("scroll_batch_set_hints: bad arguments");
        return SCROLL_ERR_ARG;
    }
    for (int i = 0; i < n; ++i) {
        const ScrollHintRect &r = rects[i];
        if (r.ref < 0 || r.ref >= 2 + 8 || r.mv_x < -SCROLL_HINT_MAX_MV ||
            r.mv_x > SCROLL_HINT_MAX_MV || r.mv_y < -SCROLL_HINT_MAX_MV ||
            r.mv_y > SCROLL_HINT_MAX_MV) {
            set_err("scroll_batch_set_hints: rect %d: ref %d / mv (%d, %d) out of range", i,
                    r.ref, r.mv_x, r.mv_y);
            return SCROLL_ERR_ARG;
        }
    }
    int rc = batch_host_sync(b);
    if (rc) return rc;
    HIPCHK(hipSetDevice(b->device));
    if (!b->hint_on) {
        int mb = 0;
        for (int k = 0; k < b->nstreams; ++k) {
            mb = std::max(mb, (b->h_st[k].w / 16) * (b->h_st[k].h / 16));
            if (b->h_st[k].w / 16 > HINT_MAX_MBW) {
                set_err("scroll_batch_set_hints: stream %d is wider than %d MBs", k, HINT_MAX_MBW);
                return SCROLL_ERR_CONFIG;
            }
        }
        const size_t slot = hint_slot_bound(1, mb);
        const size_t S = (size_t)b->max_streams, F = (size_t)b->max_frames;
        hipError_t e = hipSuccess;
        if (b->dyn_on) {
            void *ns = nullptr;
            e = hipMalloc(&ns, S * F * slot);
            if (e == hipSuccess) e = hipMalloc(&b->d_hf, S * F * sizeof(HintFrame));
            if (e != hipSuccess) {
                (void)hipFree(ns);
                (void)hipFree(b->d_hf);
                b->d_hf = nullptr;
                (void)hipGetLastError();
                set_err("scroll_batch_set_hints: %s", hipGetErrorString(e));
                return e == hipErrorOutOfMemory ? SCROLL_ERR_OOM : SCROLL_ERR_HIP;
            }
            (void)hipFree(b->d_stage);
            b->d_stage = (uint8_t *)ns;
        } else {
            e = hipMalloc(&b->d_dfr, S * F * sizeof(DynFrame));
            if (e == hipSuccess) e = hipMalloc(&b->d_stage, S * F * slot);
            if (e == hipSuccess) e = hipMalloc(&b->d_hf, S * F * sizeof(HintFrame));
            if (e == hipSuccess) e = hipMemset(b->d_dfr, 0, S * F * sizeof(DynFrame));
            if (e != hipSuccess) {
                set_err("scroll_batch_set_hints: %s", hipGetErrorString(e));
                hint_release(b);
                return e == hipErrorOutOfMemory ? SCROLL_ERR_OOM : SCROLL_ERR_HIP;
            }
            b->geo = DynGeom{};
        }
        b->geo.slot_bytes = slot;
        b->hint_max_mb = mb;
        b->h_hint.assign(S * F, {});
        b->h_hint_mode.assign(S * F, (int16_t)SCROLL_HINT_EXACT);
        b->hint_on = 1;
        if (b->dyn_on && (rc = hd_setup(b))) return rc;
    }
    const size_t i = (size_t)s * b->max_frames + f;
    b->h_hint[i].assign(rects, rects + n);
    b->h_hint_mode[i] = (int16_t)mode;
    b->hint_dirty = 1;
    return SCROLL_OK;
}

int scroll_batch_clear_hints(ScrollBatch *b)
{
    if (!b) return SCROLL_ERR_ARG;
    if (!b->hint_on) return SCROLL_OK;
    int rc = batch_host_sync(b);
    if (rc) return rc;
    HIPCHK(hipSetDevice(b->device));
    hint_release(b);
    if (b->dyn_on) {
        const size_t S = (size_t)b->max_streams, F = (size_t)b->max_frames;
        hipError_t e = hipMalloc(&b->d_dfr, S * F * sizeof(DynFrame));
        if (e == hipSuccess) e = hipMalloc(&b->d_stage, S * F * (size_t)4 * b->geo.ep_cap);
        if (e == hipSuccess) e = hipMemset(b->d_dfr, 0, S * F * sizeof(DynFrame));
        if (e != hipSuccess) {
            set_err("scroll_batch_clear_hints: %s", hipGetErrorString(e));
            dyn_release(b);
            return e == hipErrorOutOfMemory ? SCROLL_ERR_OOM : SCROLL_ERR_HIP;
        }
        b->geo.slot_bytes = b->dyn_cap;
        if (b->dyn_pos_custom) {
            for (size_t i = 0; i < S * F; ++i) {
                b->h_dyn_pos[2 * i] = b->geo.x0;
                b->h_dyn_pos[2 * i + 1] = b->geo.y0;
            }
            b->dyn_pos_custom = 0;
        }
    }
    return SCROLL_OK;
}

static int sp_grow(void **p, size_t *cap, size_t n, size_t size)
{
    if (n <= *cap) return SCROLL_OK;
    (void)hipFree(*p);
    *p = nullptr;
    *cap = 0;
    hipError_t e = hipMalloc(p, std::max<size_t>(n, 1) * size);
    if (e != hipSuccess) {
        set_err("splice: %s", hipGetErrorString(e));
        return e == hipErrorOutOfMemory ? SCROLL_ERR_OOM : SCROLL_ERR_HIP;
    }
    *cap = n;
    return SCROLL_OK;
}

static int splice_upload(ScrollBatch *b)
{
    const size_t S = (size_t)b->max_streams, F = (size_t)b->max_frames;
    std::vector<SpliceFrame> spf(S * F);
    for (SpliceFrame &o : spf) o.hd_qp = -1;
    std::vector<int32_t> list;
    std::vector<uint8_t> pool;
    size_t words = 0, recs = 0, nunits = 0, slot = b->geo.slot_bytes;
    int ymax = 1;
    std::vector<size_t> pool_off(b->h_sp.size(), 0);
    for (size_t i = 0; i < b->h_sp.size(); ++i) {
        const ScrollBatch::SpliceHost &h = b->h_sp[i];
        SpliceFrame &o = spf[i];
        o = SpliceFrame{};
        o.hd_qp = -1;
        if (h.w <= 0) continue;
        o.x0 = h.x0;
        o.y0 = h.y0;
        o.w = h.w;
        o.h = h.h;
        o.nal_len = (uint32_t)h.n;
        o.rbsp_word = words;
        o.rec_first = (uint32_t)recs;
        if (!h.dnal) {
            pool_off[i] = pool.size();
            pool.insert(pool.end(), h.nal.begin(), h.nal.end());
            pool.resize((pool.size() + 3) & ~(size_t)3);
        }
        words += (h.n + 3) / 4 + 2;
        recs += (size_t)h.w * h.h;
// ... 906 lines not shown
```

### h264-scroll-encoder_amd/h264scroll.py

```python
import ctypes
import os

HERE = os.path.dirname(os.path.abspath(__file__))
LIB_PATH = os.environ.get("H264SCROLL_LIB") or os.path.join(HERE, "lib", "libh264scroll.so")

SCROLL_OK = 0
SCROLL_ERR_NO_DEVICE = -1
SCROLL_ERR_ARG = -2
SCROLL_ERR_OOM = -3
SCROLL_ERR_OVERFLOW = -4
SCROLL_ERR_HIP = -5
SCROLL_ERR_CONFIG = -6
SCROLL_ERR_DEVICE = -7
SCROLL_MODE_COMPOSER = 0
SCROLL_MODE_EXPERIMENT = 1
SCROLL_DEBUG_FORCE_SERIAL = 1
SCROLL_DEBUG_EMIT_NOSTORE = 2
SCROLL_DEBUG_EMIT_ZEROS = 4
SCROLL_DEBUG_EMIT_BUILD = 8
SCROLL_DEBUG_EMIT_NOPURE = 16
SCROLL_DEBUG_EMIT_NOMIXED = 32
SCROLL_DEBUG_EMIT_STAMPS = 64
SCROLL_DEBUG_EMIT_NOBYTES = 128
SCROLL_DEBUG_DYN_STAMPS = 256
SCROLL_DEBUG_DYN_NOLOAD = 512
SCROLL_DEBUG_DYN_NOCAVLC = 1024
SCROLL_DEBUG_DYN_NOHEAD = 2048
SCROLL_DEBUG_DYN_NOWRITE = 4096
SCROLL_DEBUG_DYN_EPCAP4 = 8192
SCROLL_DEBUG_DYN_NOPUBLISH = 16384
SCROLL_DEBUG_DYN_GATHER1 = 32768
SCROLL_DEBUG_DYN_EPWIN = 65536
SCROLL_COMPOSE_REWIND = 1
MAX_WAYPOINTS = 8
MV_LIMIT_PX = 496


class WaypointInfo(ctypes.Structure):
    _fields_ = [("offset_px", ctypes.c_int), ("long_term_idx", ctypes.c_int),
                ("valid", ctypes.c_int)]


class ComposerConfig(ctypes.Structure):
    _fields_ = [("width", ctypes.c_int), ("height", ctypes.c_int),
                ("mb_width", ctypes.c_int), ("mb_height", ctypes.c_int),
                ("log2_max_frame_num", ctypes.c_int), ("pic_order_cnt_type", ctypes.c_int),
                ("log2_max_pic_order_cnt_lsb", ctypes.c_int),
                ("num_ref_idx_l0_default_minus1", ctypes.c_int),
                ("deblocking_filter_control_present_flag", ctypes.c_int),
                ("frame_num", ctypes.c_int), ("idr_pic_id", ctypes.c_int),
                ("waypoints", WaypointInfo * MAX_WAYPOINTS), ("num_waypoints", ctypes.c_int)]


class NALWriter(ctypes.Structure):
    _fields_ = [("output", ctypes.POINTER(ctypes.c_uint8)), ("output_capacity", ctypes.c_size_t),
                ("output_pos", ctypes.c_size_t), ("rbsp", ctypes.POINTER(ctypes.c_uint8)),
                ("rbsp_capacity", ctypes.c_size_t)]


class BitWriter(ctypes.Structure):
    _fields_ = [("buffer", ctypes.POINTER(ctypes.c_uint8)), ("capacity", ctypes.c_size_t),
                ("byte_pos", ctypes.c_size_t), ("bit_pos", ctypes.c_int),
                ("current_byte", ctypes.c_uint8)]


class BitReader(ctypes.Structure):
    _fields_ = [("buffer", ctypes.POINTER(ctypes.c_uint8)), ("size", ctypes.c_size_t),
                ("byte_pos", ctypes.c_size_t), ("bit_pos", ctypes.c_int)]


class NALUnit(ctypes.Structure):
    _fields_ = [("nal_ref_idc", ctypes.c_int), ("nal_unit_type", ctypes.c_int),
                ("data", ctypes.POINTER(ctypes.c_uint8)), ("size", ctypes.c_size_t),
                ("rbsp_size", ctypes.c_size_t)]


class NALParser(ctypes.Structure):
    _fields_ = [("data", ctypes.POINTER(ctypes.c_uint8)), ("size", ctypes.c_size_t),
                ("pos", ctypes.c_size_t)]


class Composer(ctypes.Structure):
    _fields_ = [("cfg", ComposerConfig), ("parse_cfg", ComposerConfig),
                ("ref_a_rbsp", ctypes.c_void_p), ("ref_a_size", ctypes.c_size_t),
                ("ref_b_rbsp", ctypes.c_void_p), ("ref_b_size", ctypes.c_size_t),
                ("orig_sps", ctypes.c_void_p), ("orig_sps_size", ctypes.c_size_t),
                ("orig_pps", ctypes.c_void_p), ("orig_pps_size", ctypes.c_size_t),
                ("nw", NALWriter), ("output_buffer", ctypes.c_void_p),
                ("output_capacity", ctypes.c_size_t), ("rbsp_temp", ctypes.c_void_p),
                ("rbsp_capacity", ctypes.c_size_t), ("frames_written", ctypes.c_int)]


class ScrollBatchDesc(ctypes.Structure):
    _fields_ = [("device", ctypes.c_int), ("max_streams", ctypes.c_int),
                ("max_frames", ctypes.c_int), ("arena_bytes", ctypes.c_size_t),
                ("mode", ctypes.c_int)]


class ScrollSpliceDesc(ctypes.Structure):
    _fields_ = [(n, ctypes.c_int32) for n in ("s", "f", "x0", "y0", "w", "h")] + [
        ("nal", ctypes.c_void_p), ("n", ctypes.c_uint64)]


class ScrollHintRect(ctypes.Structure):
    _fields_ = [(n, ctypes.c_int16) for n in ("x0", "y0", "x1", "y1", "ref", "reserved")] + [
        ("mv_x", ctypes.c_int32), ("mv_y", ctypes.c_int32)]


SCROLL_HINT_EXACT, SCROLL_HINT_PSKIP, SCROLL_HINT_SPEC, SCROLL_HINT_MAX_RECTS = 0, 1, 2, 64
(SCROLL_SPLICE_OK, SCROLL_SPLICE_ERR_NAL, SCROLL_SPLICE_ERR_HEADER, SCROLL_SPLICE_ERR_MBTYPE,
 SCROLL_SPLICE_ERR_SYNTAX, SCROLL_SPLICE_ERR_REF) = range(6)


def _load():
    if not os.path.exists(LIB_PATH):
        raise ImportError(f"{LIB_PATH} not built: run `make -C h264-scroll-encoder_amd` "
                          "(there is no fallback implementation)")
    lib = ctypes.CDLL(LIB_PATH)
    P = ctypes.POINTER
    u8p = P(ctypes.c_uint8)
    sig = {
        "scroll_last_error": (ctypes.c_char_p, []),
        "scroll_device_count": (ctypes.c_int, []),
        "scroll_version": (ctypes.c_char_p, []),
        "scroll_batch_create": (ctypes.c_int, [P(ctypes.c_void_p), P(ScrollBatchDesc)]),
        "scroll_batch_destroy": (None, [ctypes.c_void_p]),
        "scroll_batch_add_stream": (ctypes.c_int, [ctypes.c_void_p, P(ComposerConfig)]),
        "scroll_batch_num_streams": (ctypes.c_int, [ctypes.c_void_p]),
        "scroll_batch_set_debug": (ctypes.c_int, [ctypes.c_void_p, ctypes.c_int]),
        "scroll_batch_set_offsets": (ctypes.c_int, [ctypes.c_void_p, P(ctypes.c_int32),
                                                    ctypes.c_int]),
        "scroll_batch_offsets_device": (ctypes.c_void_p, [ctypes.c_void_p]),
        "scroll_batch_compose": (ctypes.c_int, [ctypes.c_void_p, ctypes.c_int, ctypes.c_void_p]),
        "scroll_batch_sync": (ctypes.c_int, [ctypes.c_void_p]),
        "scroll_batch_compose_ex": (ctypes.c_int, [ctypes.c_void_p, ctypes.c_int, ctypes.c_void_p,
                                                   ctypes.c_int]),
        "scroll_batch_kernel_stats": (ctypes.c_int, [ctypes.c_void_p, P(ctypes.c_double),
                                                     P(ctypes.c_double), P(ctypes.c_int)]),
        "scroll_batch_last_bytes": (ctypes.c_ulonglong, [ctypes.c_void_p]),
        "scroll_batch_debug_stamps": (ctypes.c_longlong, [ctypes.c_void_p, P(ctypes.c_uint64),
                                                          ctypes.c_longlong]),
        "scroll_batch_last_nals": (ctypes.c_longlong, [ctypes.c_void_p]),
        "scroll_batch_get_config": (ctypes.c_int, [ctypes.c_void_p, ctypes.c_int,
                                                   P(ComposerConfig)]),
        "scroll_batch_set_config": (ctypes.c_int, [ctypes.c_void_p, ctypes.c_int,
                                                   P(ComposerConfig)]),
        "scroll_batch_output_size": (ctypes.c_size_t, [ctypes.c_void_p, ctypes.c_int]),
        "scroll_batch_copy_output": (ctypes.c_int, [ctypes.c_void_p, ctypes.c_int,
                                                    ctypes.c_size_t, u8p, ctypes.c_size_t]),
        "scroll_batch_output_device": (ctypes.c_void_p, [ctypes.c_void_p, ctypes.c_int]),
        "scroll_host_alloc": (ctypes.c_int, [P(ctypes.c_void_p), ctypes.c_size_t]),
        "scroll_host_free": (None, [ctypes.c_void_p]),
        "scroll_batch_output_to_host_async": (ctypes.c_int, [ctypes.c_void_p, ctypes.c_void_p,
                                                             ctypes.c_size_t, ctypes.c_void_p,
                                                             ctypes.c_void_p]),
        "scroll_batch_reset_output": (ctypes.c_int, [ctypes.c_void_p]),
        "scroll_batch_nal_count": (ctypes.c_int, [ctypes.c_void_p, ctypes.c_int]),
        "scroll_batch_nal_info": (ctypes.c_int, [ctypes.c_void_p, ctypes.c_int, ctypes.c_int,
                                                 P(ctypes.c_int), P(ctypes.c_int),
                                                 P(ctypes.c_uint32), P(ctypes.c_int)]),
        "scroll_batch_enable_timing": (ctypes.c_int, [ctypes.c_void_p, ctypes.c_int]),
        "scroll_batch_kernel_ms": (ctypes.c_float, [ctypes.c_void_p, ctypes.c_int]),
        "scroll_batch_set_dyn_rect": (ctypes.c_int, [ctypes.c_void_p] + [ctypes.c_int] * 4 +
                                      [ctypes.c_size_t]),
        "scroll_batch_set_dyn_refs": (ctypes.c_int, [ctypes.c_void_p, ctypes.c_int, u8p, u8p]),
        "scroll_batch_set_dyn_qp": (ctypes.c_int, [ctypes.c_void_p, ctypes.c_int]),
        "scroll_batch_set_dyn_qp_stream": (ctypes.c_int, [ctypes.c_void_p, ctypes.c_int, ctypes.c_int]),
        "scroll_batch_set_dyn_qp_at": (ctypes.c_int, [ctypes.c_void_p, ctypes.c_int, ctypes.c_int,
                                                      ctypes.c_int]),
        "scroll_batch_set_dyn_source": (ctypes.c_int, [ctypes.c_void_p, u8p, ctypes.c_int]),
        "scroll_batch_set_dyn_rect_at": (ctypes.c_int, [ctypes.c_void_p] + [ctypes.c_int] * 4),
        "scroll_batch_set_fallback": (ctypes.c_int, [ctypes.c_void_p, ctypes.c_int]),
        "scroll_batch_fallback_frame": (ctypes.c_int, [ctypes.c_void_p, ctypes.c_int, ctypes.c_int,
                                                       ctypes.POINTER(ctypes.c_int)]),
        "scroll_batch_dyn_source_device": (ctypes.c_void_p, [ctypes.c_void_p, P(ctypes.c_size_t),
                                                             P(ctypes.c_size_t)]),
        "scroll_batch_dyn_source_synth": (ctypes.c_int, [ctypes.c_void_p, ctypes.c_int,
                                                         ctypes.c_int, ctypes.c_int]),
        "scroll_batch_dyn_frame_info": (ctypes.c_int, [ctypes.c_void_p, ctypes.c_int, ctypes.c_int,
                                                       P(ctypes.c_uint32), P(ctypes.c_uint32)]),
        "scroll_batch_dyn_totals": (ctypes.c_int, [ctypes.c_void_p, P(ctypes.c_ulonglong),
                                                   P(ctypes.c_ulonglong), P(ctypes.c_longlong)]),
        "scroll_batch_kernel_stats_ex": (ctypes.c_int, [ctypes.c_void_p, P(ctypes.c_double),
                                                        P(ctypes.c_int)]),
        "scroll_batch_set_hints": (ctypes.c_int, [ctypes.c_void_p, ctypes.c_int, ctypes.c_int,
                                                  P(ScrollHintRect), ctypes.c_int, ctypes.c_int]),
        "scroll_batch_clear_hints": (ctypes.c_int, [ctypes.c_void_p]),
        "scroll_batch_set_splice": (ctypes.c_int, [ctypes.c_void_p, ctypes.c_int, ctypes.c_int,
                                                   ctypes.c_int, ctypes.c_int, ctypes.c_int,
                                                   ctypes.c_int, ctypes.c_char_p, ctypes.c_size_t]),
        "scroll_batch_clear_splices": (ctypes.c_int, [ctypes.c_void_p]),
        "scroll_batch_set_splices_device": (ctypes.c_int, [ctypes.c_void_p, ctypes.c_int,
                                                           P(ScrollSpliceDesc)]),
        "scroll_batch_splice_status": (ctypes.c_int, [ctypes.c_void_p, ctypes.c_int, ctypes.c_int,
                                                      P(ctypes.c_int)]),
        "scroll_batch_splice_refusal": (ctypes.c_int, [ctypes.c_void_p, ctypes.c_int, ctypes.c_int,
                                                       P(ctypes.c_int), P(ctypes.c_int), P(ctypes.c_int),
                                                       P(ctypes.c_int)]),
        "scroll_batch_ingest": (ctypes.c_int, [ctypes.c_void_p, ctypes.c_int, P(u8p),
                                               P(ctypes.c_size_t), P(u8p), P(ctypes.c_size_t),
                                               P(ctypes.c_int)]),
        "scroll_batch_update_refs": (ctypes.c_int, [ctypes.c_void_p, ctypes.c_int, P(ctypes.c_int),
                                                    P(ctypes.c_int), P(u8p), P(ctypes.c_size_t),
                                                    P(ctypes.c_int)]),
        "scroll_batch_update_refs_device": (ctypes.c_int, [ctypes.c_void_p, ctypes.c_int, P(ctypes.c_int),
                                                           P(ctypes.c_int), ctypes.c_void_p,
                                                           P(ctypes.c_uint64), P(ctypes.c_int)]),
        "scroll_batch_ingest_stats": (ctypes.c_int, [ctypes.c_void_p, P(ctypes.c_double),
                                                     P(ctypes.c_int)]),
        "scroll_batch_ingest_device": (ctypes.c_int, [ctypes.c_void_p, ctypes.c_int,
                                                      ctypes.c_void_p, P(ctypes.c_uint64),
                                                      P(ctypes.c_int)]),
        "scroll_batch_ipcm_files_device": (ctypes.c_int, [ctypes.c_void_p, ctypes.c_int, ctypes.c_int,
                                                          ctypes.c_int, ctypes.c_void_p, ctypes.c_size_t,
                                                          ctypes.c_void_p, ctypes.c_size_t,
                                                          P(ctypes.c_uint64)]),
        "scroll_batch_ipcm_files_device_async": (ctypes.c_int, [ctypes.c_void_p, ctypes.c_int, ctypes.c_int,
                                                                ctypes.c_int, ctypes.c_void_p, ctypes.c_size_t,
                                                                ctypes.c_void_p, ctypes.c_size_t,
                                                                ctypes.c_void_p]),
        "scroll_batch_ipcm_stats": (ctypes.c_int, [ctypes.c_void_p, P(ctypes.c_double),
                                                   P(ctypes.c_int)]),
        "composer_batch_write_scroll_frames": (ctypes.c_int, [P(P(Composer)), P(ctypes.c_int),
                                                              ctypes.c_int, ctypes.c_int]),
        "composer_flush": (ctypes.c_int, [P(Composer)]),
        "composer_init": (ctypes.c_int, [P(Composer), ctypes.c_char_p, ctypes.c_char_p]),
        "composer_get_width": (ctypes.c_int, [P(Composer)]),
        "composer_get_height": (ctypes.c_int, [P(Composer)]),
        "composer_write_header": (None, [P(Composer)]),
        "composer_write_scroll_frame": (None, [P(Composer), ctypes.c_int]),
        "composer_get_output_size": (ctypes.c_size_t, [P(Composer)]),
        "composer_get_output": (u8p, [P(Composer)]),
        "composer_write_to_file": (ctypes.c_int, [P(Composer), ctypes.c_char_p]),
        "composer_finish": (None, [P(Composer)]),
        "composer_config_init": (None, [P(ComposerConfig), ctypes.c_int, ctypes.c_int]),
        "composer_config_set_sps_params": (None, [P(ComposerConfig), ctypes.c_int, ctypes.c_int,
                                                  ctypes.c_int]),
        "composer_config_set_pps_params": (None, [P(ComposerConfig), ctypes.c_int,
                                                  ctypes.c_int]),
        "h264_generate_sps": (ctypes.c_size_t, [u8p, ctypes.c_size_t, ctypes.c_int,
                                                ctypes.c_int]),
        "h264_generate_pps": (ctypes.c_size_t, [u8p, ctypes.c_size_t]),
        "h264_rewrite_idr_frame": (ctypes.c_size_t, [P(NALWriter), P(ComposerConfig),
                                                     P(ComposerConfig), u8p, ctypes.c_size_t]),
        "h264_rewrite_as_non_idr_i_frame": (ctypes.c_size_t, [P(NALWriter), P(ComposerConfig),
                                                              P(ComposerConfig), u8p,
                                                              ctypes.c_size_t, ctypes.c_int]),
        "h264_write_scroll_p_frame": (ctypes.c_size_t, [P(NALWriter), P(ComposerConfig),
                                                        ctypes.c_int]),
        "h264_needs_waypoint": (ctypes.c_int, [P(ComposerConfig), ctypes.c_int]),
        "h264_write_waypoint_p_frame": (ctypes.c_size_t, [P(NALWriter), P(ComposerConfig),
                                                          ctypes.c_int]),
        "nal_writer_init": (None, [P(NALWriter), u8p, ctypes.c_size_t, u8p, ctypes.c_size_t]),
        "nal_write_unit": (ctypes.c_size_t, [P(NALWriter), ctypes.c_int, ctypes.c_int, u8p,
                                             ctypes.c_size_t, ctypes.c_int]),
        "nal_writer_get_size": (ctypes.c_size_t, [P(NALWriter)]),
        "nal_writer_get_output": (u8p, [P(NALWriter)]),
        "rbsp_to_ebsp": (ctypes.c_size_t, [u8p, ctypes.c_size_t, u8p, ctypes.c_size_t]),
        "nal_parser_init": (None, [P(NALParser), u8p, ctypes.c_size_t]),
        "nal_parser_next": (ctypes.c_int, [P(NALParser), P(NALUnit)]),
        "ebsp_to_rbsp": (ctypes.c_size_t, [u8p, u8p, ctypes.c_size_t]),
        "parse_sps": (ctypes.c_int, [u8p, ctypes.c_size_t] + [P(ctypes.c_int)] * 5),
        "parse_pps": (ctypes.c_int, [u8p, ctypes.c_size_t] + [P(ctypes.c_int)] * 2),
        "bitwriter_init": (None, [P(BitWriter), u8p, ctypes.c_size_t]),
        "bitwriter_write_bits": (None, [P(BitWriter), ctypes.c_uint32, ctypes.c_int]),
        "bitwriter_write_bit": (None, [P(BitWriter), ctypes.c_int]),
        "bitwriter_write_ue": (None, [P(BitWriter), ctypes.c_uint32]),
        "bitwriter_write_se": (None, [P(BitWriter), ctypes.c_int32]),
        "bitwriter_write_trailing_bits": (None, [P(BitWriter)]),
        "bitwriter_flush": (None, [P(BitWriter)]),
        "bitwriter_get_size": (ctypes.c_size_t, [P(BitWriter)]),
        "bitwriter_get_bit_position": (ctypes.c_size_t, [P(BitWriter)]),
        "bitwriter_is_byte_aligned": (ctypes.c_int, [P(BitWriter)]),
        "bitreader_init": (None, [P(BitReader), u8p, ctypes.c_size_t]),
        "bitreader_read_bits": (ctypes.c_uint32, [P(BitReader), ctypes.c_int]),
        "bitreader_read_bit": (ctypes.c_int, [P(BitReader)]),
        "bitreader_read_ue": (ctypes.c_uint32, [P(BitReader)]),
        "bitreader_read_se": (ctypes.c_int32, [P(BitReader)]),
        "bitreader_get_bit_position": (ctypes.c_size_t, [P(BitReader)]),
        "bitreader_is_byte_aligned": (ctypes.c_int, [P(BitReader)]),
        "bitreader_get_remaining_bytes": (ctypes.c_size_t, [P(BitReader)]),
        "bitreader_get_pointer": (u8p, [P(BitReader)]),
    }
    variant = bool(os.environ.get("H264SCROLL_LIB"))
    for name, (res, args) in sig.items():
        try:
            f = getattr(lib, name)
        except AttributeError:
            if variant:
                continue
            raise
        f.restype = res
        f.argtypes = args
    return lib


lib = _load()


def last_error():
    return (lib.scroll_last_error() or b"").decode()


def device_count():
    return lib.scroll_device_count()


def u8buf(data_or_size):
    if isinstance(data_or_size, int):
        return (ctypes.c_uint8 * data_or_size)()
    b = (ctypes.c_uint8 * len(data_or_size)).from_buffer_copy(data_or_size)
    return b


class HostBuffer:

    def __init__(self, nbytes, nstreams):
        self.cap = (nbytes + 15) & ~15
        self.ns = nstreams
        self.p = ctypes.c_void_p()
        self.t = ctypes.c_void_p()
        if lib.scroll_host_alloc(ctypes.byref(self.p), self.cap) or \
                lib.scroll_host_alloc(ctypes.byref(self.t), 8 * (1 + 2 * nstreams)):
            raise RuntimeError("scroll_host_alloc: " + last_error())
        self.table = (ctypes.c_uint64 * (1 + 2 * nstreams)).from_address(self.t.value)
        self.data = (ctypes.c_uint8 * self.cap).from_address(self.p.value)

    def total(self):
        v = self.table[0]
        return None if v == (1 << 64) - 1 else v

    def stream(self, s):
        if self.total() is None:
            raise RuntimeError("the last delivery did not fit the host buffer: nothing was written")
        o, n = self.table[1 + 2 * s], self.table[2 + 2 * s]
        return ctypes.string_at(self.p.value + o, n)

    def close(self):
        if self.p:
            lib.scroll_host_free(self.p)
            lib.scroll_host_free(self.t)
            self.p = self.t = None

    def __del__(self):
        try:
            self.close()
        except Exception:
            pass


def make_config(w, h, frame_num=2, log2_mfn=4, poc_type=2, log2_poc=4, deblock=1,
                waypoints=()):
    c = ComposerConfig()
    lib.composer_config_init(ctypes.byref(c), w, h)
    lib.composer_config_set_sps_params(ctypes.byref(c), log2_mfn, poc_type, log2_poc)
    lib.composer_config_set_pps_params(ctypes.byref(c), 1, deblock)
    c.frame_num = frame_num
    for i, (off, lt, valid) in enumerate(waypoints):
        c.waypoints[i].offset_px, c.waypoints[i].long_term_idx, c.waypoints[i].valid = off, lt, valid
    c.num_waypoints = len(waypoints)
    return c


class Batch:

    def __init__(self, max_streams, max_frames, arena_bytes, device=0,
                 mode=SCROLL_MODE_COMPOSER):
        d = ScrollBatchDesc(device, max_streams, max_frames, arena_bytes, mode)
        h = ctypes.c_void_p()
        rc = lib.scroll_batch_create(ctypes.byref(h), ctypes.byref(d))
        if rc != SCROLL_OK:
            raise RuntimeError(f"scroll_batch_create failed ({rc}): {last_error()}")
        self.h = h
        self.max_frames = max_frames

    def close(self):
        if self.h:
            lib.scroll_batch_destroy(self.h)
            self.h = None

    def __del__(self):
        try:
            self.close()
        except Exception:
            pass

    def _chk(self, rc, what):
        if rc < 0:
            raise RuntimeError(f"{what} failed ({rc}): {last_error()}")
        return rc

    def add_stream(self, cfg):
        return self._chk(lib.scroll_batch_add_stream(self.h, ctypes.byref(cfg)), "add_stream")

    @property
    def num_streams(self):
        return lib.scroll_batch_num_streams(self.h)

    def set_debug(self, flags):
        self._chk(lib.scroll_batch_set_debug(self.h, flags), "set_debug")

    def set_offsets(self, offsets):
        import numpy as np
        a = np.ascontiguousarray(offsets, dtype=np.int32)
        self._chk(lib.scroll_batch_set_offsets(
            self.h, a.ctypes.data_as(ctypes.POINTER(ctypes.c_int32)), a.shape[1]), "set_offsets")

    def offsets_device_ptr(self):
        return lib.scroll_batch_offsets_device(self.h)

    def compose(self, nframes, stream=None, rewind=False):
        self._chk(lib.scroll_batch_compose_ex(self.h, nframes, stream,
                                              SCROLL_COMPOSE_REWIND if rewind else 0), "compose")

    def sync(self):
        return lib.scroll_batch_sync(self.h)

    def config(self, s):
        c = ComposerConfig()
        self._chk(lib.scroll_batch_get_config(self.h, s, ctypes.byref(c)), "get_config")
        return c

    def set_config(self, s, cfg):
        self._chk(lib.scroll_batch_set_config(self.h, s, ctypes.byref(cfg)), "set_config")

    def output_size(self, s):
        return lib.scroll_batch_output_size(self.h, s)

    def output(self, s, start=0, n=None):
        if n is None:
            n = self.output_size(s) - start
        b = u8buf(max(n, 1))
        self._chk(lib.scroll_batch_copy_output(self.h, s, start, b, n), "copy_output")
        return bytes(b[:n])

    def output_to_host_async(self, hb, stream=None):
        self._chk(lib.scroll_batch_output_to_host_async(self.h, hb.p, hb.cap, hb.t, stream),
                  "output_to_host_async")

    def output_device_ptr(self, s):
        return lib.scroll_batch_output_device(self.h, s)

    def reset_output(self):
        self._chk(lib.scroll_batch_reset_output(self.h), "reset_output")

    def nals(self, s):
        n = self._chk(lib.scroll_batch_nal_count(self.h, s), "nal_count")
        out = []
        k, o, sl = ctypes.c_int(), ctypes.c_int(), ctypes.c_int()
        sz = ctypes.c_uint32()
        for i in range(n):
            self._chk(lib.scroll_batch_nal_info(self.h, s, i, ctypes.byref(k), ctypes.byref(o),
                                                ctypes.byref(sz), ctypes.byref(sl)), "nal_info")
            out.append((k.value, o.value, sz.value, sl.value))
        return out

    def enable_timing(self, on=True, lite=False):
        self._chk(lib.scroll_batch_enable_timing(self.h, (2 if lite else 1) if on else 0), "enable_timing")

    def kernel_ms(self, which):
        return lib.scroll_batch_kernel_ms(self.h, which)

    def kernel_stats(self):
        a, e, n = ctypes.c_double(), ctypes.c_double(), ctypes.c_int()
        self._chk(lib.scroll_batch_kernel_stats(self.h, ctypes.byref(a), ctypes.byref(e),
                                                ctypes.byref(n)), "kernel_stats")
        return a.value, e.value, n.value

    def kernel_stats_ex(self):
        ms, n = (ctypes.c_double * 6)(), ctypes.c_int()
        self._chk(lib.scroll_batch_kernel_stats_ex(self.h, ms, ctypes.byref(n)), "kernel_stats_ex")
        return tuple(ms), n.value

    def ingest(self, refs):
        n = len(refs)
        bufs = [(u8buf(bytes(a) or b"\0"), u8buf(bytes(b) or b"\0")) for a, b in refs]
        u8p = ctypes.POINTER(ctypes.c_uint8)
        pa = (u8p * max(n, 1))(*[ctypes.cast(x[0], u8p) for x in bufs])
        pb = (u8p * max(n, 1))(*[ctypes.cast(x[1], u8p) for x in bufs])
        na = (ctypes.c_size_t * max(n, 1))(*[len(a) for a, _ in refs])
        nb = (ctypes.c_size_t * max(n, 1))(*[len(b) for _, b in refs])
        first = ctypes.c_int()
        self._chk(lib.scroll_batch_ingest(self.h, n, pa, na, pb, nb, ctypes.byref(first)), "ingest")
        return first.value

    def ingest_device(self, n, d_files, desc):
        arr = (ctypes.c_uint64 * max(1, len(desc)))(*desc)
        first = ctypes.c_int()
        self._chk(lib.scroll_batch_ingest_device(self.h, n, ctypes.c_void_p(d_files), arr,
                                                 ctypes.byref(first)), "ingest_device")
        return first.value

    def update_refs(self, streams, which, files, check=True):
        n = len(streams)
        st = (ctypes.c_int * n)(*streams)
        wh = (ctypes.c_int * n)(*which)
        bufs = [u8buf(f) for f in files]
        fp = (ctypes.POINTER(ctypes.c_uint8) * n)(*[ctypes.cast(x, ctypes.POINTER(ctypes.c_uint8)) for x in bufs])
        sz = (ctypes.c_size_t * n)(*[len(f) for f in files])
        stat = (ctypes.c_int * n)()
        rc = lib.scroll_batch_update_refs(self.h, n, st, wh, fp, sz, stat)
        if check:
            self._chk(rc, "update_refs")
        return rc, list(stat)

    def ingest_stats(self):
        ms, n = ctypes.c_double(), ctypes.c_int()
        self._chk(lib.scroll_batch_ingest_stats(self.h, ctypes.byref(ms), ctypes.byref(n)),
                  "ingest_stats")
        return ms.value, n.value

    def ipcm_files_device(self, n, w, h, d_pics, pic_stride, d_out, out_stride):
        sizes = (ctypes.c_uint64 * max(1, n))()
        self._chk(lib.scroll_batch_ipcm_files_device(self.h, n, w, h, ctypes.c_void_p(d_pics),
                                                     pic_stride, ctypes.c_void_p(d_out),
                                                     out_stride, sizes), "ipcm_files_device")
        return [int(sizes[i]) for i in range(n)]

    def ipcm_files_device_async(self, n, w, h, d_pics, pic_stride, d_out, out_stride, d_sizes):
        self._chk(lib.scroll_batch_ipcm_files_device_async(self.h, n, w, h, ctypes.c_void_p(d_pics), pic_stride,
                                                           ctypes.c_void_p(d_out), out_stride,
                                                           ctypes.c_void_p(d_sizes)), "ipcm_files_device_async")

    def ipcm_stats(self):
        ms, n = ctypes.c_double(), ctypes.c_int()
        self._chk(lib.scroll_batch_ipcm_stats(self.h, ctypes.byref(ms), ctypes.byref(n)),
                  "ipcm_stats")
        return ms.value, n.value

    def set_hints(self, s, f, rects, mode=SCROLL_HINT_EXACT):
        arr = (ScrollHintRect * max(1, len(rects)))()
        for i, (x0, y0, x1, y1, ref, mx, my) in enumerate(rects):
            arr[i] = ScrollHintRect(x0, y0, x1, y1, ref, 0, mx, my)
        self._chk(lib.scroll_batch_set_hints(self.h, s, f, arr, len(rects), mode), "set_hints")

    def clear_hints(self):
        self._chk(lib.scroll_batch_clear_hints(self.h), "clear_hints")

    def set_splice(self, s, f, x0, y0, w, h, nal):
        nal = bytes(nal)
        self._chk(lib.scroll_batch_set_splice(self.h, s, f, x0, y0, w, h, nal, len(nal)),
                  "set_splice")

    def set_splices_device(self, entries):
        arr = (ScrollSpliceDesc * max(1, len(entries)))()
        for i, e in enumerate(entries):
            arr[i] = ScrollSpliceDesc(*e)
        self._chk(lib.scroll_batch_set_splices_device(self.h, len(entries), arr),
                  "set_splices_device")

    def clear_splices(self):
        self._chk(lib.scroll_batch_clear_splices(self.h), "clear_splices")

    def splice_status(self, s, f):
# ... 83 lines not shown
```

### include/composer_batch.h

```cpp
#ifndef COMPOSER_BATCH_H
#define COMPOSER_BATCH_H

#include <stddef.h>
#include <stdint.h>
#include "composer.h"
#include "h264_writer.h"

#ifdef __cplusplus
extern "C" {
#endif

#define SCROLL_OK             0
#define SCROLL_ERR_NO_DEVICE (-1)
#define SCROLL_ERR_ARG       (-2)
#define SCROLL_ERR_OOM       (-3)
#define SCROLL_ERR_OVERFLOW  (-4)
#define SCROLL_ERR_HIP       (-5)
#define SCROLL_ERR_CONFIG    (-6)
#define SCROLL_ERR_DEVICE    (-7)

#define SCROLL_MODE_COMPOSER   0
#define SCROLL_MODE_EXPERIMENT 1

#define SCROLL_DEBUG_FORCE_SERIAL 1
#define SCROLL_DEBUG_EMIT_NOSTORE 2
#define SCROLL_DEBUG_EMIT_ZEROS   4
#define SCROLL_DEBUG_EMIT_BUILD   8
#define SCROLL_DEBUG_EMIT_NOPURE 16
#define SCROLL_DEBUG_EMIT_NOMIXED 32
#define SCROLL_DEBUG_EMIT_STAMPS 64
#define SCROLL_DEBUG_EMIT_NOBYTES 128
#define SCROLL_DEBUG_DYN_STAMPS 256
#define SCROLL_DEBUG_DYN_NOLOAD  512
#define SCROLL_DEBUG_DYN_NOCAVLC 1024
#define SCROLL_DEBUG_DYN_NOHEAD  2048
#define SCROLL_DEBUG_DYN_NOWRITE 4096
#define SCROLL_DEBUG_DYN_EPCAP4 8192
#define SCROLL_DEBUG_DYN_NOPUBLISH 16384
#define SCROLL_DEBUG_DYN_GATHER1 32768
#define SCROLL_DEBUG_DYN_EPWIN 65536

typedef struct ScrollBatch ScrollBatch;

typedef struct {
    int device;
    int max_streams;
    int max_frames;
    size_t arena_bytes;
    int mode;
} ScrollBatchDesc;

const char *scroll_last_error(void);
int scroll_device_count(void);
const char *scroll_version(void);

int scroll_batch_create(ScrollBatch **out, const ScrollBatchDesc *desc);
void scroll_batch_destroy(ScrollBatch *b);
int scroll_batch_add_stream(ScrollBatch *b, const ComposerConfig *cfg);
int scroll_batch_num_streams(const ScrollBatch *b);
int scroll_batch_set_debug(ScrollBatch *b, int flags);

int scroll_batch_set_offsets(ScrollBatch *b, const int32_t *offsets, int nframes);
int32_t *scroll_batch_offsets_device(ScrollBatch *b);

int scroll_batch_compose(ScrollBatch *b, int nframes, void *hip_stream);
#define SCROLL_COMPOSE_REWIND 1
int scroll_batch_compose_ex(ScrollBatch *b, int nframes, void *hip_stream, int flags);
int scroll_batch_sync(ScrollBatch *b);

int scroll_batch_get_config(ScrollBatch *b, int s, ComposerConfig *cfg);
int scroll_batch_set_config(ScrollBatch *b, int s, const ComposerConfig *cfg);
size_t scroll_batch_output_size(ScrollBatch *b, int s);
int scroll_batch_copy_output(ScrollBatch *b, int s, size_t from, uint8_t *dst, size_t n);
const uint8_t *scroll_batch_output_device(ScrollBatch *b, int s);
int scroll_host_alloc(void **p, size_t n);
void scroll_host_free(void *p);
int scroll_batch_output_to_host_async(ScrollBatch *b, uint8_t *dst, size_t cap, uint64_t *table,
                                      void *hip_stream);
int scroll_batch_reset_output(ScrollBatch *b);

int scroll_batch_nal_count(ScrollBatch *b, int s);
int scroll_batch_nal_info(ScrollBatch *b, int s, int i, int *kind, int *offset_px,
                          uint32_t *size, int *slow);

int scroll_batch_enable_timing(ScrollBatch *b, int on);
float scroll_batch_kernel_ms(ScrollBatch *b, int which);
int scroll_batch_kernel_stats(ScrollBatch *b, double *plan_ms, double *emit_ms, int *count);
long long scroll_batch_debug_stamps(ScrollBatch *b, uint64_t *dst, long long max_slots);
unsigned long long scroll_batch_last_bytes(ScrollBatch *b);
long long scroll_batch_last_nals(ScrollBatch *b);

int scroll_batch_set_dyn_rect(ScrollBatch *b, int x0, int y0, int w, int h, size_t slot_bytes);
int scroll_batch_set_dyn_refs(ScrollBatch *b, int s, const uint8_t *ref_a, const uint8_t *ref_b);
#define SCROLL_DYN_QP_MIN 0
#define SCROLL_DYN_QP_MAX 51
int scroll_batch_set_dyn_qp(ScrollBatch *b, int qp);
int scroll_batch_set_dyn_qp_stream(ScrollBatch *b, int s, int qp);
int scroll_batch_set_dyn_qp_at(ScrollBatch *b, int s, int f, int qp);
int scroll_batch_set_dyn_source(ScrollBatch *b, const uint8_t *src, int nframes);
int scroll_batch_set_dyn_rect_at(ScrollBatch *b, int s, int f, int x0, int y0);
int scroll_batch_set_fallback(ScrollBatch *b, int on);
int scroll_batch_fallback_frame(ScrollBatch *b, int s, int f, int *fell_back);
uint8_t *scroll_batch_dyn_source_device(ScrollBatch *b, size_t *stream_stride,
                                        size_t *frame_stride);
int scroll_batch_dyn_source_synth(ScrollBatch *b, int nframes, int stream_base, int t0);
int scroll_batch_dyn_frame_info(ScrollBatch *b, int s, int f, uint32_t *rbsp_bytes,
                                uint32_t *ep_bytes);
int scroll_batch_dyn_totals(ScrollBatch *b, unsigned long long *rbsp_bytes,
                            unsigned long long *ep_bytes, long long *dyn_nals);
int scroll_batch_kernel_stats_ex(ScrollBatch *b, double ms[6], int *count);

#define SCROLL_HINT_EXACT 0
#define SCROLL_HINT_PSKIP 1
#define SCROLL_HINT_SPEC 2
#define SCROLL_HINT_MAX_RECTS 64
#define SCROLL_HINT_MAX_MV 8192
typedef struct ScrollHintRect {
    int16_t x0, y0, x1, y1;
    int16_t ref;
    int16_t reserved;
    int32_t mv_x, mv_y;
} ScrollHintRect;
int scroll_batch_set_hints(ScrollBatch *b, int s, int f, const ScrollHintRect *rects, int n,
                           int mode);
int scroll_batch_clear_hints(ScrollBatch *b);

#define SCROLL_SPLICE_MAX_BYTES   ((uint64_t)1 << 29)
#define SCROLL_SPLICE_OK          0
#define SCROLL_SPLICE_ERR_NAL     1
#define SCROLL_SPLICE_ERR_HEADER  2
#define SCROLL_SPLICE_ERR_MBTYPE  3
#define SCROLL_SPLICE_ERR_SYNTAX  4
#define SCROLL_SPLICE_ERR_REF     5
int scroll_batch_set_splice(ScrollBatch *b, int s, int f, int x0, int y0, int w, int h,
                            const uint8_t *nal, size_t n);
typedef struct ScrollSpliceDesc {
    int32_t s, f;
    int32_t x0, y0, w, h;
    const uint8_t *nal;
    uint64_t n;
} ScrollSpliceDesc;
int scroll_batch_set_splices_device(ScrollBatch *b, int n, const ScrollSpliceDesc *d);
int scroll_batch_clear_splices(ScrollBatch *b);
int scroll_batch_splice_status(ScrollBatch *b, int s, int f, int *status);
int scroll_batch_splice_refusal(ScrollBatch *b, int s, int f, int *status, int *mb_x, int *mb_y, int *mb_type);

int scroll_batch_ingest(ScrollBatch *b, int n, const uint8_t *const *ref_a, const size_t *na,
                        const uint8_t *const *ref_b, const size_t *nb, int *first);
int scroll_batch_ingest_device(ScrollBatch *b, int n, const uint8_t *d_files,
                               const uint64_t *desc, int *first);

int scroll_batch_update_refs(ScrollBatch *b, int n, const int *streams, const int *which,
                             const uint8_t *const *files, const size_t *sizes, int *status);
int scroll_batch_update_refs_device(ScrollBatch *b, int n, const int *streams, const int *which,
                                    const uint8_t *d_files, const uint64_t *desc, int *status);
int scroll_batch_ingest_stats(ScrollBatch *b, double *ms, int *count);

int scroll_batch_ipcm_files_device(ScrollBatch *b, int n, int w, int h, const uint8_t *d_pics,
                                   size_t pic_stride, uint8_t *d_out, size_t out_stride,
                                   uint64_t *sizes);
int scroll_batch_ipcm_files_device_async(ScrollBatch *b, int n, int w, int h, const uint8_t *d_pics,
                                         size_t pic_stride, uint8_t *d_out, size_t out_stride,
                                         uint64_t *d_sizes);
int scroll_batch_ipcm_stats(ScrollBatch *b, double *ms, int *count);

int composer_batch_write_scroll_frames(Composer *const *cs, const int *offsets, int n,
                                       int flags);
int composer_flush(Composer *c);

#ifdef __cplusplus
}
#endif
#endif
```

Measured before the change: 2.799 million frames/s.

## Fuse static-row bitstream packing into row-table kernel and skip general path when impossible

Merges the separate k_dyn_static kernel into k_dyn_rows so each frame block computes head classes once and then packs the static row groups with per-wave shared buffers. It removes the side-stream fork option and adds a host-side gen_possible flag that skips general-path launches when no low-QP or generated-row case can occur. If an unexpected general frame appears, the flag triggers a retry via the overflow path. This cuts kernel launches and repeated header setup, at the cost of a larger fused kernel with more shared memory and lower occupancy.

```diff
diff --git a/h264-scroll-encoder_amd/csrc/dyn_engine.h b/h264-scroll-encoder_amd/csrc/dyn_engine.h
--- a/h264-scroll-encoder_amd/csrc/dyn_engine.h
+++ b/h264-scroll-encoder_amd/csrc/dyn_engine.h
@@ -21,20 +21,13 @@
 #define DYN_HEAD_VECS 16
 #define DYN_CTR_LIST 4
 
-typedef struct {
-    hipStream_t side;
-    hipEvent_t e0, e1;
-} DynFork;
 int dyn_launch_code(hipStream_t hs, int nframes, int S, DevStream *st, const NalDesc *nal,
                     int ld_nal, const PlanPending *pend, DynFrame *dfr, int ld_fr,
                     const DynGeom *g, const uint8_t *src, const uint8_t *refs, const DynScratch *x,
-                    uint32_t epoch, int mbw, uint64_t *stamps, const DynFork *fk, hipEvent_t ev0 = nullptr,
+                    uint32_t epoch, int mbw, uint64_t *stamps, bool general, hipEvent_t ev0 = nullptr,
                     hipEvent_t ev1 = nullptr);
-int dyn_launch_static(hipStream_t hs, int nframes, int S, DevStream *st, const NalDesc *nal, int ld_nal,
-                      const PlanPending *pend, DynFrame *dfr, int ld_fr, const DynGeom *g, const DynScratch *x);
-int dyn_launch_pack(hipStream_t hs, int nframes, int S, DevStream *st, const NalDesc *nal,
-                    int ld_nal, const PlanPending *pend, DynFrame *dfr, int ld_fr,
-                    const DynGeom *g, const DynScratch *x, uint8_t *eps, uint64_t *stamps, const DynFork *fk);
+int dyn_launch_pack(hipStream_t hs, int nframes, int S, DevStream *st, DynFrame *dfr, int ld_fr,
+                    const DynGeom *g, const DynScratch *x, uint8_t *eps, uint64_t *stamps);
 int dyn_launch_emit(hipStream_t hs, int nframes, int S, const DevStream *st, const NalDesc *nal,
                     int ld_nal, const DynFrame *dfr, int ld_fr, const DynGeom *g,
                     const uint8_t *stage, const DynScratch *x, uint8_t *arena, uint64_t ld_arena,
diff --git a/h264-scroll-encoder_amd/csrc/dyn_kernels.hip b/h264-scroll-encoder_amd/csrc/dyn_kernels.hip
--- a/h264-scroll-encoder_amd/csrc/dyn_kernels.hip
+++ b/h264-scroll-encoder_amd/csrc/dyn_kernels.hip
@@ -628,44 +628,268 @@
     return make_uint4((uint32_t)(H >> 32), (uint32_t)H, (uint32_t)(Lw >> 32), (uint32_t)Lw);
 }
 
-__global__ __launch_bounds__(256) void k_dyn_rows(const DevStream *__restrict__ st,
-                                                  const NalDesc *__restrict__ nal, int ld_nal,
-                                                  const PlanPending *__restrict__ pend,
-                                                  DynFrame *__restrict__ dfr, int ld_fr, DynGeom g,
-                                                  uint32_t *__restrict__ rows, uint32_t *__restrict__ ctr,
-                                                  uint4 *__restrict__ heads)
-{
-    __shared__ int32_t wo[8], wl[8], wv[8];
+constexpr int GW = 64;
+#ifndef SCROLL_GBUF_WORDS
+#define SCROLL_GBUF_WORDS 256
+#endif
+constexpr int GBUF_WORDS = SCROLL_GBUF_WORDS;
+
+#ifndef SCROLL_STATIC_WORDS
+#define SCROLL_STATIC_WORDS 1
+#endif
+
+struct StaticHeads {
+    uint4 pat[12];
+    uint64_t hhi[12], hlo[12];
+    uint32_t hlen[12];
+    int32_t head_over;
+    int32_t wo[8], wl[8], wv[8];
+};
+struct StaticWave {
+    uint32_t ncand;
+    uint32_t buf[GBUF_WORDS];
+    uint32_t moff[DYN_STATIC_ROWS + 1];
+};
+
+__device__ inline void static_class(StaticHeads &C, const HeadCtx &H, int t, uint4 &bits, uint32_t &len)
+{
+    CapSink hc{0, 0, 0};
+    H.put_class(hc, t);
+    C.hhi[t] = hc.hi;
+    C.hlo[t] = hc.lo;
+    C.hlen[t] = hc.n;
+    if (hc.over()) C.head_over = 1;
+    if (hc.n < 128u) {
+        const uint64_t hi = (hc.hi << 1) | (hc.lo >> 63), lo = (hc.lo << 1) | 1u;
+        C.pat[t] = body_msb(hi, lo, hc.n + 1u);
+    } else {
+        C.head_over = 1;
+    }
+    bits = body_msb(hc.hi, hc.lo, min(hc.n, 128u));
+    len = hc.n | (hc.over() ? 0x80000000u : 0u);
+}
+
+__device__ inline void static_group(const StaticHeads &C, StaticWave &L, const HeadCtx &H, const NalCtx &c,
+                                    const DynGeom &g, int gi, size_t nb, int t,
+                                    uint32_t *__restrict__ rowstage, uint32_t *__restrict__ gbits)
+{
+    constexpr int SR = DYN_STATIC_ROWS;
+    const Rect R{g.x0, g.y0, g.w, g.h};
+    const int nA = max(1, (R.y0 + SR - 1) / SR);
+    const int ng = g.ngroups;
+    const bool first = gi == 0, last = gi == ng - 1;
+    if (t == 0) L.ncand = 0;
+    const int mbw = H.mbw, mbh = c.h / 16;
+    int ra, rb;
+    if (gi < nA) {
+        ra = gi * SR;
+        rb = min(ra + SR, R.y0);
+    } else {
+        ra = R.y0 + R.h + (gi - nA - R.h) * SR;
+        rb = min(ra + SR, mbh);
+    }
+    uint32_t F = 0;
+    if (first) {
+        CountSink hc{0};
+        emit_slice_header(hc, c);
+        F = hc.n;
+    }
+    const bool head_over = C.head_over;
+    auto head_bits = [&](int r, int col) -> uint32_t {
+        if (!head_over) return C.hlen[H.sel(r, col)];
+        CountSink cn{0};
+        H.put_slow(cn, r, col);
+        return cn.n;
+    };
+    uint32_t len = 0;
+    const int r = ra + t;
+    if (r < rb) {
+        if (!head_over) {
+            len = row_static_bits(H, C.hlen, r, R);
+        } else {
+            for (int col = 0; col < mbw; ++col) len += head_bits(r, col) + 1u;
+        }
+    }
+    const uint32_t incl = wave_incl_sum(len, t);
+    if (r < rb) L.moff[r - ra] = F + incl - len;
+    const uint32_t rows_end = F + __shfl(incl, GW - 1, GW);
+    if (t == 0) L.moff[rb - ra] = rows_end;
+    const uint32_t bits = rows_end + (last ? 1u : 0u);
+    if (t == 0) gbits[nb * (size_t)ng + gi] = bits;
+    wave_sync();
+
+    uint32_t *out = rowstage + nb * g.rs_frame_words + rs_group_words(g, nA, gi);
+    const uint32_t nw = min((bits + 31u) >> 5, g.rs_static_words - EPC_STATIC);
+    const int ne = rb - ra;
+    auto cnt_le = [&](uint32_t x) -> int {
+        int lo = 0, hi = ne + 1;
+        while (lo < hi) {
+            const int mid = (lo + hi) >> 1;
+            if (L.moff[mid] <= x) lo = mid + 1;
+            else hi = mid;
+        }
+        return lo;
+    };
+    const uint32_t m_mbw = magic32((uint32_t)mbw);
+    for (uint32_t p0 = 0; p0 < nw; p0 += GBUF_WORDS) {
+        const uint32_t n = min((uint32_t)GBUF_WORDS, nw - p0);
+        for (uint32_t i = (uint32_t)t; i < n; i += GW) L.buf[i] = 0u;
+        wave_sync();
+        const LdsOrWin win{L.buf, p0, n};
+        if (!(SCROLL_STATIC_WORDS && !head_over) && first && t == 0 && p0 * 32u < F) {
+            WSink hs{win, 0, 0, 0};
+            hs.start(0);
+            emit_slice_header(hs, c);
+            hs.finish();
+        }
+        if (SCROLL_STATIC_WORDS && !head_over) {
+            const uint32_t rbeg = L.moff[0], rend = L.moff[ne];
+            for (uint32_t i = (uint32_t)t; i < n; i += GW) {
+                const uint32_t W0 = 32u * (p0 + i), W1 = W0 + 32u;
+                uint32_t acc = 0, b = max(W0, rbeg), R0 = 0, R1 = 0, L0 = 0, Lm = 1;
+                int b3 = 0;
+                float inv = 1.0f;
+                while (b < W1 && b < rend) {
+                    if (b >= R1 || b < R0) {
+                        const int e = cnt_le(b) - 1;
+                        R0 = L.moff[e];
+                        R1 = L.moff[e + 1];
+                        b3 = H.sel(ra + e, 0);
+                        L0 = C.hlen[b3] + 1u;
+                        Lm = C.hlen[b3 + 1] + 1u;
+                        inv = 1.0f / (float)Lm;
+                    }
+                    const uint32_t o = b - R0;
+                    uint32_t cl = (uint32_t)b3, off = o;
+                    if (o >= L0) {
+                        const uint32_t o2 = o - L0;
+                        uint32_t q = (uint32_t)((float)o2 * inv);
+                        if (q * Lm > o2) --q;
+                        else if ((q + 1u) * Lm <= o2) ++q;
+                        if (q < (uint32_t)(mbw - 2)) {
+                            cl = (uint32_t)b3 + 1u;
+                            off = o2 - q * Lm;
+                        } else {
+                            cl = (uint32_t)b3 + 2u;
+                            off = o2 - (uint32_t)(mbw - 2) * Lm;
+                        }
+                    }
+                    const uint32_t k = min(C.hlen[cl] + 1u - off, W1 - b);
+                    const uint4 P = C.pat[cl];
+                    const uint32_t wi = off >> 5, sh = off & 31u;
+                    const uint32_t w0 = wi == 0 ? P.x : (wi == 1 ? P.y : (wi == 2 ? P.z : P.w));
+                    const uint32_t w1 = wi == 0 ? P.y : (wi == 1 ? P.z : (wi == 2 ? P.w : 0u));
+                    uint32_t v = sh ? __builtin_amdgcn_alignbit(w0, w1, 32u - sh) : w0;
+                    v &= k >= 32u ? 0xffffffffu : ~(0xffffffffu >> k);
+                    acc |= v >> (b - W0);
+                    b += k;
+                }
+                L.buf[i] = acc;
+            }
+            wave_sync();
+            if (first && t == 0 && p0 * 32u < F) {
+                WSink hs{win, 0, 0, 0};
+                hs.start(0);
+                emit_slice_header(hs, c);
+                hs.finish();
+            }
+            if (last && t == 0) {
+                WSink sk{win, 0, 0, 0};
+                sk.start(bits - 1u);
+                sk.put(1, 1);
+                sk.finish();
+            }
+            wave_sync();
+            flush_window(L.buf, n, p0, p0 + n >= nw, out, &L.ncand,
+                         rowstage + nb * g.rs_frame_words + rs_runs_words(g, nA, gi), EPC_STATIC - 1, t, GW);
+            wave_sync();
+            continue;
+        }
+        const int ea = max(cnt_le(32u * p0) - 1, 0), eb = min(cnt_le(32u * (p0 + n) - 1u), ne);
+        const int nm = eb * mbw;
+        for (int m = ea * mbw + t; m < nm; m += GW) {
+            const int rr = (int)div_m((uint32_t)m, m_mbw), col = m - rr * mbw, rw = ra + rr;
+            uint32_t off = L.moff[rr];
+            WSink sk{win, 0, 0, 0};
+            if (!head_over) {
+                const int b3 = H.sel(rw, 0);
+                off += col == 0 ? 0u : C.hlen[b3] + 1u + (uint32_t)(col - 1) * (C.hlen[b3 + 1] + 1u);
+                if (off >= 32u * (p0 + n)) continue;
+                const int cls = b3 + (col == 0 ? 0 : (col == mbw - 1 ? 2 : 1));
+                if (off + C.hlen[cls] + 1u <= 32u * p0) continue;
+                sk.start(off);
+                sk.put_cap(CapSink{C.hhi[cls], C.hlo[cls], C.hlen[cls]});
+            } else {
+                for (int c2 = 0; c2 < col; ++c2) off += head_bits(rw, c2) + 1u;
+                sk.start(off);
+                H.put_slow(sk, rw, col);
+            }
+            sk.put(1, 1);
+            sk.finish();
+        }
+        if (last && t == 0) {
+            WSink sk{win, 0, 0, 0};
+            sk.start(bits - 1u);
+            sk.put(1, 1);
+            sk.finish();
+        }
+        wave_sync();
+        flush_window(L.buf, n, p0, p0 + n >= nw, out, &L.ncand,
+                     rowstage + nb * g.rs_frame_words + rs_runs_words(g, nA, gi), EPC_STATIC - 1, t, GW);
+        wave_sync();
+    }
+    if (t == 0) rowstage[nb * g.rs_frame_words + rs_runs_words(g, nA, gi)] = L.ncand;
+    wave_sync();
+}
+
+constexpr int ROWS_MAXW = 4;
+__global__ __launch_bounds__(64 * ROWS_MAXW) __attribute__((amdgpu_waves_per_eu(8))) void k_dyn_rows(const DevStream *__restrict__ st,
+                                                              const NalDesc *__restrict__ nal, int ld_nal,
+                                                              const PlanPending *__restrict__ pend,
+                                                              DynFrame *__restrict__ dfr, int ld_fr, DynGeom g,
+                                                              uint32_t *__restrict__ rows, uint32_t *__restrict__ ctr,
+                                                              uint4 *__restrict__ heads,
+                                                              uint32_t *__restrict__ rowstage,
+                                                              uint32_t *__restrict__ gbits)
+{
+    __shared__ StaticHeads C;
+    __shared__ StaticWave LW[ROWS_MAXW];
     __shared__ int32_t gen;
-    const int s = blockIdx.y, f = blockIdx.x, t = threadIdx.x;
-    DynFrame *DF = dfr + (size_t)s * ld_fr + f;
+    const int s = blockIdx.y, f = blockIdx.x, t = threadIdx.x, nt = (int)blockDim.x;
+    const size_t nb = (size_t)s * ld_fr + f;
+    DynFrame *DF = dfr + nb;
     const int j = DF->nal;
     if (j < 0) return;
     if (t < 8) {
-        wo[t] = pend[s].wo[t];
-        wl[t] = pend[s].wl[t];
-        wv[t] = pend[s].wv[t];
-    }
-    if (t == 0) gen = 0;
+        C.wo[t] = pend[s].wo[t];
+        C.wl[t] = pend[s].wl[t];
+        C.wv[t] = pend[s].wv[t];
+    }
+    if (t == 0) {
+        gen = 0;
+        C.head_over = 0;
+    }
     __syncthreads();
     const DevStream *S = st + s;
     const NalDesc d = nal[(size_t)s * ld_nal + j];
-    const NalCtx c = nal_ctx(S, d, wo, wl, wv);
+    NalCtx c = nal_ctx(S, d, C.wo, C.wl, C.wv);
+    c.qpd = S->dyn_qp - QP_DEFAULT;
+    const HeadCtx H = head_ctx(c);
     if (t < 12) {
-        const HeadCtx H = head_ctx(c);
-        CapSink hc{0, 0, 0};
-        H.put_class(hc, t);
-        uint4 *hv = heads + ((size_t)s * ld_fr + f) * DYN_HEAD_VECS;
-        hv[t] = body_msb(hc.hi, hc.lo, min(hc.n, 128u));
-        reinterpret_cast<uint32_t *>(hv + 12)[t] = hc.n | (hc.over() ? 0x80000000u : 0u);
-    }
-    const Regions rg = regions(c);
-    const int w = c.w, h = c.h, a_end = (h - c.off) / 16;
+        uint4 hb;
+        uint32_t hl;
+        static_class(C, H, t, hb, hl);
+        uint4 *hv = heads + nb * DYN_HEAD_VECS;
+        hv[t] = hb;
+        reinterpret_cast<uint32_t *>(hv + 12)[t] = hl;
+    }
+    const Regions rg = H.rg;
+    const int w = c.w, h = c.h, a_end = H.a_end;
     const uint32_t ysz = (uint32_t)w * (uint32_t)h, pic = ysz + ysz / 2;
-    const WpTab T{wo, wv, h};
-    uint32_t *rw = rows + ((size_t)s * ld_fr + f) * (size_t)(32 * g.h);
+    const WpTab T{C.wo, C.wv, h};
+    uint32_t *rw = rows + nb * (size_t)(32 * g.h);
     bool my_gen = false;
-    for (int i = t; i < 32 * g.h; i += 256) {
+    for (int i = t; i < 32 * g.h; i += nt) {
         uint32_t e;
         if (i < 16 * g.h) {
             const int Y = 16 * g.y0 + i, row = Y >> 4;
@@ -697,7 +921,7 @@
             const uint32_t k = atomicAdd(&ctr[1], 1u);
             if (k < g.gen_cap) {
                 DF->rbsp_bytes = k;
-                ctr[DYN_CTR_LIST + k] = (uint32_t)((size_t)s * ld_fr + f);
+                ctr[DYN_CTR_LIST + k] = (uint32_t)nb;
                 e = DF_GENERAL;
             } else {
                 e = DF_OVER;
@@ -706,235 +930,15 @@
         DF->err = e;
         DF->ep = 0u;
     }
-}
-
-constexpr int GW = 64;
-#ifndef SCROLL_GBUF_WORDS
-#define SCROLL_GBUF_WORDS 256
-#endif
-constexpr int GBUF_WORDS = SCROLL_GBUF_WORDS;
-
-#ifndef SCROLL_STATIC_WORDS
-#define SCROLL_STATIC_WORDS 1
-#endif
-
-struct StaticFixed {
-    uint32_t ncand;
-    uint32_t buf[GBUF_WORDS];
-    uint64_t hhi[12], hlo[12];
-    uint4 pat[12];
-    uint32_t hlen[12];
-    int32_t head_over;
-    int32_t wo[8], wl[8], wv[8];
-    uint32_t moff[DYN_STATIC_ROWS + 1];
-};
-
-__global__ __launch_bounds__(GW) void k_dyn_static(const DevStream *__restrict__ st,
-                                                   const NalDesc *__restrict__ nal, int ld_nal,
-                                                   const PlanPending *__restrict__ pend,
-                                                   const DynFrame *__restrict__ dfr, int ld_fr, DynGeom g,
-                                                   uint32_t *__restrict__ rowstage, uint32_t *__restrict__ gbits)
-{
-    __shared__ StaticFixed L;
-    constexpr int SR = DYN_STATIC_ROWS;
-    const Rect R{g.x0, g.y0, g.w, g.h};
-    const int nA = max(1, (R.y0 + SR - 1) / SR);
-    const int gi = (int)blockIdx.x >= nA ? (int)blockIdx.x + R.h : (int)blockIdx.x;
-    const int ng = g.ngroups, f = blockIdx.y, s = blockIdx.z, t = threadIdx.x;
-    const size_t nb = (size_t)s * ld_fr + f;
-    const int j = dfr[nb].nal;
-    if (j < 0) return;
-    const bool first = gi == 0, last = gi == ng - 1;
-    if (t < 8) {
-        L.wo[t] = pend[s].wo[t];
-        L.wl[t] = pend[s].wl[t];
-        L.wv[t] = pend[s].wv[t];
-    }
-    if (t == 0) {
-        L.head_over = 0;
-        L.ncand = 0;
-    }
-    const DevStream *S = st + s;
-    const NalDesc d = nal[(size_t)s * ld_nal + j];
-    wave_sync();
-    NalCtx c = nal_ctx(S, d, L.wo, L.wl, L.wv);
-    c.qpd = S->dyn_qp - QP_DEFAULT;
-    const HeadCtx H = head_ctx(c);
-    const int mbw = H.mbw, mbh = c.h / 16;
-    int ra, rb;
-    if (gi < nA) {
-        ra = gi * SR;
-        rb = min(ra + SR, R.y0);
-    } else {
-        ra = R.y0 + R.h + (gi - nA - R.h) * SR;
-        rb = min(ra + SR, mbh);
-    }
-    uint32_t F = 0;
-    if (first) {
-        CountSink hc{0};
-        emit_slice_header(hc, c);
-        F = hc.n;
-    }
-    if (t < 12) {
-        CapSink hc{0, 0, 0};
-        H.put_class(hc, t);
-        L.hhi[t] = hc.hi;
-        L.hlo[t] = hc.lo;
-        L.hlen[t] = hc.n;
-        if (hc.over()) L.head_over = 1;
-        if (hc.n < 128u) {
-            const uint64_t hi = (hc.hi << 1) | (hc.lo >> 63), lo = (hc.lo << 1) | 1u;
-            L.pat[t] = body_msb(hi, lo, hc.n + 1u);
-        } else {
-            L.head_over = 1;
-        }
-    }
-    wave_sync();
-    const bool head_over = L.head_over;
-    auto head_bits = [&](int r, int col) -> uint32_t {
-        if (!head_over) return L.hlen[H.sel(r, col)];
-        CountSink cn{0};
-        H.put_slow(cn, r, col);
-        return cn.n;
-    };
-    uint32_t len = 0;
-    const int r = ra + t;
-    if (r < rb) {
-        if (!head_over) {
-            len = row_static_bits(H, L.hlen, r, R);
-        } else {
-            for (int col = 0; col < mbw; ++col) len += head_bits(r, col) + 1u;
-        }
-    }
-    const uint32_t incl = wave_incl_sum(len, t);
-    if (r < rb) L.moff[r - ra] = F + incl - len;
-    const uint32_t rows_end = F + __shfl(incl, GW - 1, GW);
-    if (t == 0) L.moff[rb - ra] = rows_end;
-    const uint32_t bits = rows_end + (last ? 1u : 0u);
-    if (t == 0) gbits[nb * (size_t)ng + gi] = bits;
-    wave_sync();
-
-    uint32_t *out = rowstage + nb * g.rs_frame_words + rs_group_words(g, nA, gi);
-    const uint32_t nw = min((bits + 31u) >> 5, g.rs_static_words - EPC_STATIC);
-    const int ne = rb - ra;
-    auto cnt_le = [&](uint32_t x) -> int {
-        int lo = 0, hi = ne + 1;
-        while (lo < hi) {
-            const int mid = (lo + hi) >> 1;
-            if (L.moff[mid] <= x) lo = mid + 1;
-            else hi = mid;
-        }
-        return lo;
-    };
-    const uint32_t m_mbw = magic32((uint32_t)mbw);
-    for (uint32_t p0 = 0; p0 < nw; p0 += GBUF_WORDS) {
-        const uint32_t n = min((uint32_t)GBUF_WORDS, nw - p0);
-        for (uint32_t i = (uint32_t)t; i < n; i += GW) L.buf[i] = 0u;
-        wave_sync();
-        const LdsOrWin win{L.buf, p0, n};
-        if (!(SCROLL_STATIC_WORDS && !head_over) && first && t == 0 && p0 * 32u < F) {
-            WSink hs{win, 0, 0, 0};
-            hs.start(0);
-            emit_slice_header(hs, c);
-            hs.finish();
-        }
-        if (SCROLL_STATIC_WORDS && !head_over) {
-            const uint32_t rbeg = L.moff[0], rend = L.moff[ne];
-            for (uint32_t i = (uint32_t)t; i < n; i += GW) {
-                const uint32_t W0 = 32u * (p0 + i), W1 = W0 + 32u;
-                uint32_t acc = 0, b = max(W0, rbeg), R0 = 0, R1 = 0, L0 = 0, Lm = 1;
-                int b3 = 0;
-                float inv = 1.0f;
-                while (b < W1 && b < rend) {
-                    if (b >= R1 || b < R0) {
-                        const int e = cnt_le(b) - 1;
-                        R0 = L.moff[e];
-                        R1 = L.moff[e + 1];
-                        b3 = H.sel(ra + e, 0);
-                        L0 = L.hlen[b3] + 1u;
-                        Lm = L.hlen[b3 + 1] + 1u;
-                        inv = 1.0f / (float)Lm;
-                    }
-                    const uint32_t o = b - R0;
-                    uint32_t cl = (uint32_t)b3, off = o;
-                    if (o >= L0) {
-                        const uint32_t o2 = o - L0;
-                        uint32_t q = (uint32_t)((float)o2 * inv);
-                        if (q * Lm > o2) --q;
-                        else if ((q + 1u) * Lm <= o2) ++q;
-                        if (q < (uint32_t)(mbw - 2)) {
-                            cl = (uint32_t)b3 + 1u;
-                            off = o2 - q * Lm;
-                        } else {
-                            cl = (uint32_t)b3 + 2u;
-                            off = o2 - (uint32_t)(mbw - 2) * Lm;
-                        }
-                    }
-                    const uint32_t k = min(L.hlen[cl] + 1u - off, W1 - b);
-                    const uint4 P = L.pat[cl];
-                    const uint32_t wi = off >> 5, sh = off & 31u;
-                    const uint32_t w0 = wi == 0 ? P.x : (wi == 1 ? P.y : (wi == 2 ? P.z : P.w));
-                    const uint32_t w1 = wi == 0 ? P.y : (wi == 1 ? P.z : (wi == 2 ? P.w : 0u));
-                    uint32_t v = sh ? __builtin_amdgcn_alignbit(w0, w1, 32u - sh) : w0;
-                    v &= k >= 32u ? 0xffffffffu : ~(0xffffffffu >> k);
-                    acc |= v >> (b - W0);
-                    b += k;
-                }
-                L.buf[i] = acc;
-            }
-            wave_sync();
-            if (first && t == 0 && p0 * 32u < F) {
-                WSink hs{win, 0, 0, 0};
-                hs.start(0);
-                emit_slice_header(hs, c);
-                hs.finish();
-            }
-            if (last && t == 0) {
-                WSink sk{win, 0, 0, 0};
-                sk.start(bits - 1u);
-                sk.put(1, 1);
-                sk.finish();
-            }
-            wave_sync();
-            flush_window(L.buf, n, p0, p0 + n >= nw, out, &L.ncand,
-                         rowstage + nb * g.rs_frame_words + rs_runs_words(g, nA, gi), EPC_STATIC - 1, t, GW);
-            wave_sync();
-            continue;
-        }
-        const int ea = max(cnt_le(32u * p0) - 1, 0), eb = min(cnt_le(32u * (p0 + n) - 1u), ne);
-        const int nm = eb * mbw;
-        for (int m = ea * mbw + t; m < nm; m += GW) {
-            const int rr = (int)div_m((uint32_t)m, m_mbw), col = m - rr * mbw, rw = ra + rr;
-            uint32_t off = L.moff[rr];
-            WSink sk{win, 0, 0, 0};
-            if (!head_over) {
-                const int b3 = H.sel(rw, 0);
-                off += col == 0 ? 0u : L.hlen[b3] + 1u + (uint32_t)(col - 1) * (L.hlen[b3 + 1] + 1u);
-                if (off >= 32u * (p0 + n)) continue;
-                const int cls = b3 + (col == 0 ? 0 : (col == mbw - 1 ? 2 : 1));
-                if (off + L.hlen[cls] + 1u <= 32u * p0) continue;
-                sk.start(off);
-                sk.put_cap(CapSink{L.hhi[cls], L.hlo[cls], L.hlen[cls]});
-            } else {
-                for (int c2 = 0; c2 < col; ++c2) off += head_bits(rw, c2) + 1u;
-                sk.start(off);
-                H.put_slow(sk, rw, col);
-            }
-            sk.put(1, 1);
-            sk.finish();
-        }
-        if (last && t == 0) {
-            WSink sk{win, 0, 0, 0};
-            sk.start(bits - 1u);
-            sk.put(1, 1);
-            sk.finish();
-        }
-        wave_sync();
-        flush_window(L.buf, n, p0, p0 + n >= nw, out, &L.ncand,
-                     rowstage + nb * g.rs_frame_words + rs_runs_words(g, nA, gi), EPC_STATIC - 1, t, GW);
-        wave_sync();
-    }
-    if (t == 0) rowstage[nb * g.rs_frame_words + rs_runs_words(g, nA, gi)] = L.ncand;
+    const int wave = t >> 6, nwv = nt >> 6, nstat = g.ngroups - g.h;
+    const int nA = max(1, (g.y0 + DYN_STATIC_ROWS - 1) / DYN_STATIC_ROWS);
+    for (int k = wave; k < nstat; k += nwv)
+        static_group(C, LW[wave], H, c, g, k >= nA ? k + g.h : k, nb, t & 63, rowstage, gbits);
+}
+
+inline int rows_threads(const DynGeom &g)
+{
+    return 64 * std::min(ROWS_MAXW, std::max(2, g.ngroups - g.h));
 }
 
 
@@ -3301,7 +3305,7 @@
 int dyn_launch_code(hipStream_t hs, int nframes, int S, DevStream *st, const NalDesc *nal,
                     int ld_nal, const PlanPending *pend, DynFrame *dfr, int ld_fr,
                     const DynGeom *g, const uint8_t *src, const uint8_t *refs, const DynScratch *x,
-                    uint32_t epoch, int mbw, uint64_t *stamps, const DynFork *fk, hipEvent_t ev0, hipEvent_t ev1)
+                    uint32_t epoch, int mbw, uint64_t *stamps, bool general, hipEvent_t ev0, hipEvent_t ev1)
 {
     if (nframes <= 0 || S <= 0) return 0;
     {
@@ -3316,20 +3320,21 @@
             ready |= 1ull << dev;
         }
     }
-    hipLaunchKernelGGL(k_dyn_rows, dim3(nframes, S), dim3(256), 0, hs, st, nal, ld_nal, pend, dfr, ld_fr,
-                       *g, x->rows, x->ctr, x->heads);
+    int nl = 0;
+    DynGeom gr = *g;
+    if (!general) gr.gen_cap = 0;
+    hipLaunchKernelGGL(k_dyn_rows, dim3(nframes, S), dim3(rows_threads(*g)), 0, hs, st, nal, ld_nal, pend, dfr,
+                       ld_fr, gr, x->rows, x->ctr, x->heads, x->rowstage, x->gbits);
     if (hipGetLastError() != hipSuccess) return -1;
-    hipStream_t hg = hs;
-    if (fk) {
-        if (hipEventRecord(fk->e0, hs) != hipSuccess || hipStreamWaitEvent(fk->side, fk->e0, 0) != hipSuccess)
-            return -1;
-        hg = fk->side;
-    }
-    const int nchunk = (24 * g->w * g->h + CODE_T - 1) / CODE_T;
-    hipLaunchKernelGGL(k_dyn_code_general, dim3(nchunk, CODE_GEN_Y), dim3(CODE_T), 0, hg, st, dfr, ld_fr,
-                       pend, nal, ld_nal, *g, x->rows, src, refs, x->meta, x->body_lo, x->body_hi, x->body_w,
-                       x->ctr);
-    if (hipGetLastError() != hipSuccess) return -1;
+    ++nl;
+    if (general) {
+        const int nchunk = (24 * g->w * g->h + CODE_T - 1) / CODE_T;
+        hipLaunchKernelGGL(k_dyn_code_general, dim3(nchunk, CODE_GEN_Y), dim3(CODE_T), 0, hs, st, dfr, ld_fr,
+                           pend, nal, ld_nal, *g, x->rows, src, refs, x->meta, x->body_lo, x->body_hi, x->body_w,
+                           x->ctr);
+        if (hipGetLastError() != hipSuccess) return -1;
+        ++nl;
+    }
     if (row_lds_bytes(g->w) > 65536) {
         const int rl = (int)row_lds_bytes(g->w);
         if (hipFuncSetAttribute(reinterpret_cast<const void *>(&k_dyn_row<false>),
@@ -3344,47 +3349,31 @@
                        x->meta, x->body_lo, x->body_hi, x->body_w, x->tcx, epoch, x->rowstage, x->gbits, x->spill,
                        x->ctr, x->heads, stamps);
     if (hipGetLastError() != hipSuccess) return -1;
+    ++nl;
     if (ev1 && hipEventRecord(ev1, hs) != hipSuccess) return -1;
-    hipLaunchKernelGGL(k_dyn_row<true>, dim3(g->h, std::min<uint32_t>(g->gen_cap, (uint32_t)(nframes * S)), 1),
-                       dim3(row_threads(g->w)),
-                       row_lds_bytes(g->w), hg, st, nal, ld_nal, pend, dfr, ld_fr, *g, x->rows, src, refs,
-                       x->meta, x->body_lo, x->body_hi, x->body_w, x->tcx, epoch, x->rowstage, x->gbits, x->spill,
-                       x->ctr, x->heads, stamps);
-    if (hipGetLastError() != hipSuccess) return -1;
-    if (fk) {
-        if (dyn_launch_static(hg, nframes, S, st, nal, ld_nal, pend, dfr, ld_fr, g, x) ||
-            hipEventRecord(fk->e1, hg) != hipSuccess)
-            return -1;
-    }
-    return 0;
-}
-
-int dyn_launch_static(hipStream_t hs, int nframes, int S, DevStream *st, const NalDesc *nal, int ld_nal,
-                      const PlanPending *pend, DynFrame *dfr, int ld_fr, const DynGeom *g, const DynScratch *x)
+    if (general) {
+        hipLaunchKernelGGL(k_dyn_row<true>, dim3(g->h, std::min<uint32_t>(g->gen_cap, (uint32_t)(nframes * S)), 1),
+                           dim3(row_threads(g->w)),
+                           row_lds_bytes(g->w), hs, st, nal, ld_nal, pend, dfr, ld_fr, *g, x->rows, src, refs,
+                           x->meta, x->body_lo, x->body_hi, x->body_w, x->tcx, epoch, x->rowstage, x->gbits,
+                           x->spill, x->ctr, x->heads, stamps);
+        if (hipGetLastError() != hipSuccess) return -1;
+        ++nl;
+    }
+    return nl;
+}
+
+int dyn_launch_pack(hipStream_t hs, int nframes, int S, DevStream *st, DynFrame *dfr, int ld_fr,
+                    const DynGeom *g, const DynScratch *x, uint8_t *eps, uint64_t *stamps)
 {
     if (nframes <= 0 || S <= 0) return 0;
-    hipLaunchKernelGGL(k_dyn_static, dim3(g->ngroups - g->h, nframes, S), dim3(GW), 0, hs, st, nal, ld_nal,
-                       pend, dfr, ld_fr, *g, x->rowstage, x->gbits);
-    return hipGetLastError() == hipSuccess ? 0 : -1;
-}
-
-int dyn_launch_pack(hipStream_t hs, int nframes, int S, DevStream *st, const NalDesc *nal,
-                    int ld_nal, const PlanPending *pend, DynFrame *dfr, int ld_fr,
-                    const DynGeom *g, const DynScratch *x, uint8_t *eps, uint64_t *stamps, const DynFork *fk)
-{
-    if (nframes <= 0 || S <= 0) return 0;
-    if (fk) {
-        if (hipStreamWaitEvent(hs, fk->e1, 0) != hipSuccess) return -1;
-    } else if (dyn_launch_static(hs, nframes, S, st, nal, ld_nal, pend, dfr, ld_fr, g, x)) {
-        return -1;
-    }
     if (g->ep_cap >= (uint32_t)EPF_BIG_LIST)
         hipLaunchKernelGGL((k_dyn_epfix<EPF_T, EPF_BIG_LIST>), dim3(nframes, S), dim3(EPF_T), gtab_bytes(g->ngroups, true),
                            hs, st, dfr, ld_fr, nframes, *g, x->rowstage, x->gbits, eps, stamps);
     else
         hipLaunchKernelGGL((k_dyn_epfix<EPF_T, EPF_LIST>), dim3(nframes, S), dim3(EPF_T), gtab_bytes(g->ngroups, true),
                            hs, st, dfr, ld_fr, nframes, *g, x->rowstage, x->gbits, eps, stamps);
-    return hipGetLastError() == hipSuccess ? 0 : -1;
+    return hipGetLastError() == hipSuccess ? 1 : -1;
 }
 
 int dyn_launch_emit(hipStream_t hs, int nframes, int S, const DevStream *st, const NalDesc *nal,
diff --git a/h264-scroll-encoder_amd/csrc/scroll_kernels.hip b/h264-scroll-encoder_amd/csrc/scroll_kernels.hip
--- a/h264-scroll-encoder_amd/csrc/scroll_kernels.hip
+++ b/h264-scroll-encoder_amd/csrc/scroll_kernels.hip
@@ -837,7 +837,9 @@
     std::vector<SpliceHost> h_sp;
     std::vector<int32_t> h_dyn_pos;
     int fallback = 0;
-    DynFork fork{};
+    int gen_possible = 0;
+    uint32_t last_gen_cap = 0;
+    int launches = 0;
     std::vector<int32_t> h_dyn_qp;
     int dyn_pos_custom = 0;
     int dyn_qp = 26;
@@ -992,12 +994,6 @@
     for (int i = 0; i < NEV; ++i)
         if (b->ev[i]) (void)hipEventDestroy(b->ev[i]);
     for (hipEvent_t e : b->ring) (void)hipEventDestroy(e);
-    if (b->fork.side) {
-        (void)hipStreamSynchronize(b->fork.side);
-        (void)hipStreamDestroy(b->fork.side);
-        (void)hipEventDestroy(b->fork.e0);
-        (void)hipEventDestroy(b->fork.e1);
-    }
     if (b->own) (void)hipStreamDestroy(b->own);
     (void)hipFree(b->d_st);
     (void)hipHostFree(b->h_st);
@@ -1094,6 +1090,7 @@
     }
     memset(d, 0, sizeof(*d));
     cfg_to_dev(cfg, d);
+    if (d->nwp > 0) b->gen_possible = 1;
     d->dyn_qp = b->dyn_qp;
     d->out_pos = 0;
     d->out_cap = b->arena_bytes;
@@ -1140,6 +1137,7 @@
         }
     }
     cfg_to_dev(cfg, d);
+    if (d->nwp > 0) b->gen_possible = 1;
     HIPCHK(hipSetDevice(b->device));
     HIPCHK(hipMemcpy(b->d_st + s, d, sizeof(DevStream), hipMemcpyHostToDevice));
     return SCROLL_OK;
@@ -1220,11 +1218,13 @@
     const int ld_fr = b->max_frames;
     int rc = mark(0);
     if (rc) return rc;
+    b->launches = 0;
     if (!dyn) {
         hipLaunchKernelGGL(k_plan, dim3(S), dim3(PLAN_THREADS), 0, hs, b->d_st, b->d_off,
                            b->max_frames, b->d_nal, b->ld_nal, nframes, plan_mode,
                            b->debug | plan_flags, b->d_pend, b->d_dfr, ld_fr);
         HIPCHK(hipGetLastError());
+        b->launches++;
         if ((rc = mark(1)) || (rc = mark(2)) || (rc = mark(3))) return rc;
     } else {
         const bool dyn_rect = b->dyn_on && !hint;
@@ -1233,6 +1233,8 @@
                            b->debug | plan_flags | PLAN_STATE | PLAN_DYN, b->d_pend, b->d_dfr,
                            ld_fr, nullptr, 0u, 0u, dyn_rect ? b->dx.ctr : nullptr);
         HIPCHK(hipGetLastError());
+        b->launches++;
+        uint32_t gen_cap = b->geo.gen_cap;
         if ((rc = mark(1))) return rc;
         uint64_t *stamps = nullptr;
         if (b->debug & SCROLL_DEBUG_DYN_STAMPS) {
@@ -1254,6 +1256,7 @@
                     return SCROLL_ERR_HIP;
                 }
                 b->sp_parse = 0;
+                b->launches += 5;
             }
             if (b->fallback && b->dyn_on &&
                 hint_launch_fb(hs, nframes, S, b->d_st, b->d_nal, b->ld_nal, b->d_pend, b->d_dfr, ld_fr,
@@ -1261,6 +1264,8 @@
                 set_err("k_hint_fb launch: %s", hipGetErrorString(hipGetLastError()));
                 return SCROLL_ERR_HIP;
             }
+            b->launches += (b->fallback && b->dyn_on ? 1 : 0) + 1 + (b->dyn_on ? 2 : 0) +
+                           (b->sp_n > 0 || b->dyn_on ? 1 : 0);
             if (hint_launch_stage(hs, nframes, S, b->d_st, b->d_nal, b->ld_nal, b->d_pend,
                                   b->d_dfr, ld_fr, b->d_hf, b->d_pool, b->d_stage,
                                   b->geo.slot_bytes)) {
@@ -1286,39 +1291,34 @@
         } else {
             b->dx.epoch = b->dx.epoch % 0xffffffu + 1u;
             const DynGeom &G = b->geo;
-            const DynFork *fk = nullptr;
-            static const bool fork_on = [] {
-                const char *e = getenv("SCROLL_DYN_FORK");
-                return e && e[0] == '1';
-            }();
-            if (fork_on) {
-                if (!b->fork.side) {
-                    HIPCHK(hipStreamCreateWithFlags(&b->fork.side, hipStreamNonBlocking));
-                    HIPCHK(hipEventCreateWithFlags(&b->fork.e0, hipEventDisableTiming));
-                    HIPCHK(hipEventCreateWithFlags(&b->fork.e1, hipEventDisableTiming));
-                }
-                fk = &b->fork;
-            }
-            if (dyn_launch_code(hs, nframes, S, b->d_st, b->d_nal, b->ld_nal, b->d_pend, b->d_dfr, ld_fr, &G,
-                                b->d_src, b->d_refs, &b->dx, b->dx.epoch, b->dyn_pw / 16, stamps, fk,
-                                lite_row ? rev[1] : nullptr, lite_row ? rev[6] : nullptr)) {
+            const bool general = b->gen_possible && !(b->debug & SCROLL_DEBUG_DYN_NOGEN);
+            gen_cap = general ? G.gen_cap : 0u;
+            int n = dyn_launch_code(hs, nframes, S, b->d_st, b->d_nal, b->ld_nal, b->d_pend, b->d_dfr, ld_fr, &G,
+                                    b->d_src, b->d_refs, &b->dx, b->dx.epoch, b->dyn_pw / 16, stamps, general,
+                                    lite_row ? rev[1] : nullptr, lite_row ? rev[6] : nullptr);
+            if (n < 0) {
                 set_err("k_dyn_code launch: %s", hipGetErrorString(hipGetLastError()));
                 return SCROLL_ERR_HIP;
             }
+            b->launches += n;
             if ((rc = mark(6))) return rc;
-            if (dyn_launch_pack(hs, nframes, S, b->d_st, b->d_nal, b->ld_nal, b->d_pend, b->d_dfr, ld_fr, &G,
-                                &b->dx, b->d_stage, stamps ? b->d_dbg : nullptr, fk)) {
-                set_err("k_dyn_static / k_dyn_epfix launch: %s", hipGetErrorString(hipGetLastError()));
+            n = dyn_launch_pack(hs, nframes, S, b->d_st, b->d_dfr, ld_fr, &G, &b->dx, b->d_stage,
+                                stamps ? b->d_dbg : nullptr);
+            if (n < 0) {
+                set_err("k_dyn_epfix launch: %s", hipGetErrorString(hipGetLastError()));
                 return SCROLL_ERR_HIP;
             }
+            b->launches += n;
         }
         if ((rc = mark(2))) return rc;
+        b->last_gen_cap = gen_cap;
         hipLaunchKernelGGL(k_plan, dim3(S), dim3(PLAN_THREADS), 0, hs, b->d_st, b->d_off,
                            b->max_frames, b->d_nal, b->ld_nal, nframes, plan_mode,
                            b->debug | plan_flags | PLAN_SIZE | PLAN_DYN, b->d_pend, b->d_dfr,
                            ld_fr, (b->dyn_on && !b->hint_on) ? (const uint32_t *)b->dx.ctr : nullptr,
-                           b->geo.rs_spill_cap, b->geo.gen_cap);
+                           b->geo.rs_spill_cap, gen_cap);
         HIPCHK(hipGetLastError());
+        b->launches++;
         if ((rc = mark(3))) return rc;
     }
     int per_wg = EMIT_WAVES * TILE;
@@ -1336,6 +1336,7 @@
         hipLaunchKernelGGL(k_emit, dim3(gx, S), dim3(EMIT_WAVES * 64), 0, hs, b->d_st, b->d_nal,
                            b->ld_nal, b->d_arena, (uint64_t)b->ld_arena, b->debug, b->d_dbg);
         HIPCHK(hipGetLastError());
+        b->launches++;
     }
     if ((rc = mark(4))) return rc;
     if (dyn && dyn_launch_emit(hs, nframes, S, b->d_st, b->d_nal, b->ld_nal, b->d_dfr, ld_fr,
@@ -1346,6 +1347,7 @@
         set_err("k_dyn_gather launch: %s", hipGetErrorString(hipGetLastError()));
         return SCROLL_ERR_HIP;
     }
+    if (dyn && nframes > 0) b->launches++;
     if ((rc = mark(5))) return rc;
     if (b->timing == 1) b->timed_pending = 1;
     b->host_valid = 0;
@@ -1445,12 +1447,15 @@
             uint32_t used[2] = {0, 0};
             if (b->dyn_on && !b->hint_on && b->dx.ctr)
                 HIPCHK(hipMemcpy(used, b->dx.ctr, sizeof(used), hipMemcpyDeviceToHost));
-            if (used[0] > b->geo.rs_spill_cap || used[1] > b->geo.gen_cap) {
-                const int grc = dyn_grow_pools(b);
+            if (used[0] > b->geo.rs_spill_cap || used[1] > b->last_gen_cap) {
+                const bool skipped = b->dyn_on && !b->hint_on && used[1] > b->last_gen_cap &&
+                                     b->last_gen_cap < b->geo.gen_cap;
+                if (skipped) b->gen_possible = 1;
+                const int grc = used[0] > b->geo.rs_spill_cap || used[1] > b->geo.gen_cap ? dyn_grow_pools(b) : 0;
                 set_err("stream %d: the dynamic rect's %s pool ran out (%u of %u); %s", s,
                         used[0] > b->geo.rs_spill_cap ? "row-stage spill" : "general-path record",
                         used[0] > b->geo.rs_spill_cap ? used[0] : used[1],
-                        used[0] > b->geo.rs_spill_cap ? b->geo.rs_spill_cap : b->geo.gen_cap,
+                        used[0] > b->geo.rs_spill_cap ? b->geo.rs_spill_cap : b->last_gen_cap,
                         grc ? "growing it failed" : "grown: compose again");
             } else {
                 set_err("stream %d: a staged NAL outgrew its staging slot (%llu bytes)", s,
@@ -1694,6 +1699,8 @@
     b->acc_n = 0;
     return SCROLL_OK;
 }
+
+int scroll_batch_debug_launches(const ScrollBatch *b) { return b ? b->launches : 0; }
 
 long long scroll_batch_debug_stamps(ScrollBatch *b, uint64_t *dst, long long max_slots)
 {
@@ -2215,6 +2222,7 @@
         }
     int rc = batch_host_sync(b);
     if (rc) return rc;
+    if (qp < scroll::dyn::QP_MIN) b->gen_possible = 1;
     HIPCHK(hipSetDevice(b->device));
     for (int k = s0; k < s1; ++k) {
         b->h_st[k].dyn_qp = qp;
@@ -2258,6 +2266,7 @@
     if (b->h_dyn_qp.size() < (size_t)b->max_streams * b->max_frames)
         b->h_dyn_qp.assign((size_t)b->max_streams * b->max_frames, -1);
     b->h_dyn_qp[i] = qp;
+    if (qp >= 0 && qp < scroll::dyn::QP_MIN) b->gen_possible = 1;
     b->hd_dirty = 1;
     return SCROLL_OK;
 }
diff --git a/h264-scroll-encoder_amd/h264scroll.py b/h264-scroll-encoder_amd/h264scroll.py
--- a/h264-scroll-encoder_amd/h264scroll.py
+++ b/h264-scroll-encoder_amd/h264scroll.py
@@ -31,6 +31,7 @@
 SCROLL_DEBUG_DYN_NOPUBLISH = 16384
 SCROLL_DEBUG_DYN_GATHER1 = 32768
 SCROLL_DEBUG_DYN_EPWIN = 65536
+SCROLL_DEBUG_DYN_NOGEN = 131072
 SCROLL_COMPOSE_REWIND = 1
 MAX_WAYPOINTS = 8
 MV_LIMIT_PX = 496
@@ -140,6 +141,7 @@
         "scroll_batch_last_bytes": (ctypes.c_ulonglong, [ctypes.c_void_p]),
         "scroll_batch_debug_stamps": (ctypes.c_longlong, [ctypes.c_void_p, P(ctypes.c_uint64),
                                                           ctypes.c_longlong]),
+        "scroll_batch_debug_launches": (ctypes.c_int, [ctypes.c_void_p]),
         "scroll_batch_last_nals": (ctypes.c_longlong, [ctypes.c_void_p]),
         "scroll_batch_get_config": (ctypes.c_int, [ctypes.c_void_p, ctypes.c_int,
                                                    P(ComposerConfig)]),
@@ -400,6 +402,9 @@
     def set_debug(self, flags):
         self._chk(lib.scroll_batch_set_debug(self.h, flags), "set_debug")
 
+    def debug_launches(self):
+        return lib.scroll_batch_debug_launches(self.h)
+
     def set_offsets(self, offsets):
         import numpy as np
         a = np.ascontiguousarray(offsets, dtype=np.int32)
diff --git a/include/composer_batch.h b/include/composer_batch.h
--- a/include/composer_batch.h
+++ b/include/composer_batch.h
@@ -39,6 +39,7 @@
 #define SCROLL_DEBUG_DYN_NOPUBLISH 16384
 #define SCROLL_DEBUG_DYN_GATHER1 32768
 #define SCROLL_DEBUG_DYN_EPWIN 65536
+#define SCROLL_DEBUG_DYN_NOGEN 131072
 
 typedef struct ScrollBatch ScrollBatch;
 
@@ -87,6 +88,7 @@
 float scroll_batch_kernel_ms(ScrollBatch *b, int which);
 int scroll_batch_kernel_stats(ScrollBatch *b, double *plan_ms, double *emit_ms, int *count);
 long long scroll_batch_debug_stamps(ScrollBatch *b, uint64_t *dst, long long max_slots);
+int scroll_batch_debug_launches(const ScrollBatch *b);
 unsigned long long scroll_batch_last_bytes(ScrollBatch *b);
 long long scroll_batch_last_nals(ScrollBatch *b);
 
```

Result: no change. 2.825 million frames/s (median of 6 runs) (+0.9%).
